# ha7ilm/csdr

Measured on AMD Instinct MI355X. Metric: complex MS/s in->out, WFM demod chain @2.4 MS/s x N streams, higher is better.
Workload: dtype f32

## Files before the change

### csdr_amd/__init__.py

```python
import ctypes as C
import os
import sys
import subprocess
import numpy as np

HERE = os.path.dirname(os.path.abspath(__file__))
LIB_PATH = os.environ.get("CSDR_AMD_LIB") or os.path.join(HERE, "libcsdr_amd.so")
ROOT = os.path.dirname(HERE)

c64 = np.complex64
f32 = np.float32

SHIFT = {"addition": 0, "math": 1, "table": 2, "unroll": 3, "addfast": 4}
WINDOWS = {"BOXCAR": 0, "BLACKMAN": 1, "HAMMING": 2}


class CsdrAmdError(RuntimeError):
    pass


def build(verbose=False):
    r = subprocess.run(["make", "-C", os.path.join(HERE, "csrc"), "-j8"], capture_output=True, text=True)
    if r.returncode != 0:
        raise CsdrAmdError("libcsdr_amd build failed:\n" + r.stdout[-4000:] + r.stderr[-4000:])
# ... 151 lines not shown
    L.csdr_amd_costas_params.argtypes = [fl, fl, i, vp]
    L.csdr_amd_pll_params_p.argtypes = [fl, vp]
    L.csdr_amd_pll_params_pi.argtypes = [fl, fl, fl, fl, vp]
    L.csdr_amd_carrier_create.restype = vp; L.csdr_amd_carrier_create.argtypes = [vp, vp, i]
    L.csdr_amd_carrier_process.argtypes = [vp, vp, ll, sz, vp, vp, vp, vp, sz]
    L.csdr_amd_carrier_reset.argtypes = [vp]
    L.csdr_amd_carrier_reset_channel.argtypes = [vp, i]
    L.csdr_amd_carrier_get_channel.argtypes = [vp, i, vp]
    L.csdr_amd_carrier_set_channel.argtypes = [vp, i, vp]
    L.csdr_amd_carrier_set_lanes.argtypes = [vp, i]
    L.csdr_amd_carrier_lanes.argtypes = [vp]
    L.csdr_amd_carrier_force_generic.argtypes = [vp, i]
    L.csdr_amd_carrier_kernel_name.restype = C.c_char_p; L.csdr_amd_carrier_kernel_name.argtypes = [vp]
    L.csdr_amd_carrier_destroy.argtypes = [vp]; L.csdr_amd_carrier_destroy.restype = None
    L.csdr_amd_debug_carrier_walk.restype = ll; L.csdr_amd_debug_carrier_walk.argtypes = [vp, vp, ll, vp, i, vp, vp, vp, vp, vp]
    L.csdr_amd_amssb_params_default.argtypes = [vp, i]
    L.csdr_amd_amssb_create_cf32.restype = vp; L.csdr_amd_amssb_create_cf32.argtypes = [vp, vp, i, vp, i, i, sz]
    L.csdr_amd_amssb_create.restype = vp; L.csdr_amd_amssb_create.argtypes = [vp, vp, i, fl, i, vp, i, vp, i, i, sz]
    L.csdr_amd_amssb_create_rates.restype = vp; L.csdr_amd_amssb_create_rates.argtypes = [vp, vp, i, vp, i, vp, i, vp, i, i, sz]
    L.csdr_amd_amssb_process.restype = ll; L.csdr_amd_amssb_process.argtypes = [vp, vp, sz, ll, vp, vp, sz]
    L.csdr_amd_amssb_max_out.restype = ll; L.csdr_amd_amssb_max_out.argtypes = [vp, ll]
    L.csdr_amd_amssb_set_rate.argtypes = [vp, i, fl]
    L.csdr_amd_amssb_get_rate.restype = fl; L.csdr_amd_amssb_get_rate.argtypes = [vp, i]
    L.csdr_amd_amssb_front_end.restype = vp; L.csdr_amd_amssb_front_end.argtypes = [vp]
    if hasattr(L, "csdr_amd_amssb_set_passband"):
        L.csdr_amd_amssb_set_passband.argtypes = [vp, i, fl, fl, i]
        L.csdr_amd_amssb_set_channel_taps.argtypes = [vp, i, vp, i]
        L.csdr_amd_amssb_get_passband.argtypes = [vp, i, vp, vp]
    L.csdr_amd_amssb_reset.argtypes = [vp]
    L.csdr_amd_amssb_reset_channel.argtypes = [vp, i]
    L.csdr_amd_amssb_get_channel.argtypes = [vp, i, vp]
    L.csdr_amd_amssb_set_channel.argtypes = [vp, i, vp]
    L.csdr_amd_amssb_set_lanes.argtypes = [vp, i]
    L.csdr_amd_amssb_lanes.argtypes = [vp]
    L.csdr_amd_amssb_force_generic.argtypes = [vp, i]
    L.csdr_amd_amssb_kernel_name.restype = C.c_char_p; L.csdr_amd_amssb_kernel_name.argtypes = [vp]
    L.csdr_amd_amssb_destroy.argtypes = [vp]; L.csdr_amd_amssb_destroy.restype = None
    L.csdr_amd_debug_amssb_walk.restype = ll; L.csdr_amd_debug_amssb_walk.argtypes = [vp, vp, i, vp, vp, vp]
    L.csdr_amd_fmmod_fc.argtypes = [vp, vp, vp, i, sz, sz, sz, vp]
    L.csdr_amd_dsb_fc.argtypes = [vp, vp, vp, sz, fl]
    L.csdr_amd_add_dcoffset_cc.argtypes = [vp, vp, vp, sz]
    L.csdr_amd_fixed_amplitude_cc.argtypes = [vp, vp, vp, sz, fl]
    L.csdr_amd_convert_f_samplerf.argtypes = [vp, vp, vp, sz, C.c_uint]
    L.csdr_amd_debug_fmmod_walk.restype = ll; L.csdr_amd_debug_fmmod_walk.argtypes = [vp, ll, vp, i, vp, vp, vp]
    L.csdr_amd_txbank_create.restype = vp; L.csdr_amd_txbank_create.argtypes = [vp, i, i, fl, fl, i, vp, i, vp, i, sz]
    L.csdr_amd_txbank_process.argtypes = [vp, vp, sz, ll, vp, sz, C.POINTER(ll)]
    L.csdr_amd_txbank_set_rate.argtypes = [vp, i, fl]
    L.csdr_amd_txbank_get_rate.restype = fl; L.csdr_amd_txbank_get_rate.argtypes = [vp, i]
    L.csdr_amd_txbank_reset.argtypes = [vp]
    L.csdr_amd_txbank_max_out.restype = ll; L.csdr_amd_txbank_max_out.argtypes = [vp, ll]
    L.csdr_amd_txbank_force_generic.argtypes = [vp, i]
    L.csdr_amd_txbank_kernel_name.restype = C.c_char_p; L.csdr_amd_txbank_kernel_name.argtypes = [vp]
    L.csdr_amd_txbank_destroy.argtypes = [vp]; L.csdr_amd_txbank_destroy.restype = None
    L.csdr_amd_rational_resampler_get_lowpass_f.restype = None; L.csdr_amd_rational_resampler_get_lowpass_f.argtypes = [vp, i, i, i, i]
    L.csdr_amd_debug_resampler_schedule.argtypes = [i, i, i, i, i, vp]
    L.csdr_amd_logaveragepower_cf.argtypes = [vp, vp, vp, i, i, i, fl]
    L.csdr_amd_fft_exchange_sides_ff.argtypes = [vp, vp, vp, i, i]
    L.csdr_amd_accumulate_power_cf.argtypes = [vp, vp, vp, sz]
    L.csdr_amd_log_ff.argtypes = [vp, vp, vp, sz, fl]
    L.csdr_amd_timer_start.argtypes = [vp]
    L.csdr_amd_timer_stop_ms.argtypes = [vp, C.POINTER(fl)]
    L.csdr_amd_firdes_filter_len.argtypes = [fl]
    L.csdr_amd_firdes_lowpass_f.argtypes = [vp, i, fl, i]
    L.csdr_amd_firdes_bandpass_c.argtypes = [vp, i, fl, fl, i]
    L.csdr_amd_nfm_deemph_taps.argtypes = [i, C.POINTER(vp)]
    L.csdr_amd_shift_addition_init.argtypes = [fl, vp]
    for nm in ("u8_f", "s8_f", "s16_f", "f_u8", "f_s8", "f_s16"):
        getattr(L, "csdr_amd_convert_" + nm).argtypes = [vp, vp, vp, sz]
    L.csdr_amd_convert_f_s24.argtypes = [vp, vp, vp, sz, i]
    L.csdr_amd_convert_s24_f.argtypes = [vp, vp, vp, sz, i]
    L.csdr_amd_rotator_generate.argtypes = [vp, i, fl, C.POINTER(fl), vp, sz, i, i]
    L.csdr_amd_mix_cc.argtypes = [vp, vp, vp, vp, i, sz, sz, sz]
    L.csdr_amd_mix_fc.argtypes = [vp, vp, vp, vp, i, sz, sz, sz]
    L.csdr_amd_shift_cc.argtypes = [vp, i, fl, C.POINTER(fl), vp, vp, i, sz, sz, sz, i, i]
    L.csdr_amd_decimating_shift_addition_cc.argtypes = [vp, vp, vp, i, i, sz, sz, vp, i, vp]
    L.csdr_amd_fir_decimate_cc.argtypes = [vp, vp, vp, i, i, sz, sz, i, vp, i]
    L.csdr_amd_fir_last_kernel.restype = C.c_char_p; L.csdr_amd_fir_last_kernel.argtypes = []
    L.csdr_amd_fir_last_instance.restype = C.c_char_p; L.csdr_amd_fir_last_instance.argtypes = []
    L.csdr_amd_audio_last_path.restype = C.c_char_p; L.csdr_amd_audio_last_path.argtypes = []
    L.csdr_amd_fir_ff_last_instance.restype = C.c_char_p; L.csdr_amd_fir_ff_last_instance.argtypes = []
    L.csdr_amd_fir_ff.argtypes = [vp, vp, vp, i, i, sz, sz, vp, i]
    L.csdr_amd_fmdemod_quadri_cf.argtypes = [vp, vp, vp, i, sz, sz, sz, vp]
    L.csdr_amd_limit_ff.argtypes = [vp, vp, vp, sz, fl]
    L.csdr_amd_gain_ff.argtypes = [vp, vp, vp, sz, fl]
    L.csdr_amd_deemphasis_wfm_ff.argtypes = [vp, vp, vp, i, sz, sz, sz, fl, i, vp]
    L.csdr_amd_fastagc_ff.argtypes = [vp, vp, vp, i, i, i, sz, sz, fl, vp]
    L.csdr_amd_fracdec_create.restype = vp; L.csdr_amd_fracdec_create.argtypes = [fl, i, vp, i]
    L.csdr_amd_fracdec_destroy.argtypes = [vp]
    L.csdr_amd_fractional_decimator_ff.argtypes = [vp, vp, vp, vp, i, i, sz, sz, C.POINTER(i)]
    L.csdr_amd_fracdec_set_cli_bufsize.restype = None; L.csdr_amd_fracdec_set_cli_bufsize.argtypes = [vp, i]
    L.csdr_amd_fracdec_set_where.restype = None; L.csdr_amd_fracdec_set_where.argtypes = [vp, fl]
    L.csdr_amd_fracdec_get_where.restype = fl; L.csdr_amd_fracdec_get_where.argtypes = [vp]
    L.csdr_amd_fftfilt_create.restype = vp; L.csdr_amd_fftfilt_create.argtypes = [vp, i, vp, i, i, i]
    L.csdr_amd_fftfilt_set_taps.argtypes = [vp, vp, i]
    if hasattr(L, "csdr_amd_fftfilt_create_per_stream"):
        L.csdr_amd_fftfilt_create_per_stream.restype = vp; L.csdr_amd_fftfilt_create_per_stream.argtypes = [vp, i, vp, i, i, i]
        L.csdr_amd_fftfilt_set_stream_taps.argtypes = [vp, i, vp, i]
        L.csdr_amd_fftfilt_per_stream.argtypes = [vp]
    L.csdr_amd_fftfilt_destroy.argtypes = [vp]
    L.csdr_amd_fftfilt_input_size.argtypes = [vp]
    L.csdr_amd_fftfilt_reset.argtypes = [vp]
    L.csdr_amd_fftfilt_kernel_name.restype = C.c_char_p; L.csdr_amd_fftfilt_kernel_name.argtypes = [vp]
    L.csdr_amd_fftfilt_window.argtypes = [vp]
    L.csdr_amd_fftfilt_process.argtypes = [vp, vp, vp, i, sz, sz]
    L.csdr_amd_fft_c2c.argtypes = [vp, vp, vp, i, i]
    L.csdr_amd_fastddc_init.argtypes = [vp, fl, i, fl]
    L.csdr_amd_fastddc_fwd_create.restype = vp; L.csdr_amd_fastddc_fwd_create.argtypes = [vp, vp, i]
    L.csdr_amd_fastddc_fwd_destroy.argtypes = [vp]
    L.csdr_amd_fastddc_fwd_process.argtypes = [vp, vp, vp, i]
    L.csdr_amd_fastddc_inv_create.restype = vp; L.csdr_amd_fastddc_inv_create.argtypes = [vp, fl, i, vp, i, i, i]
    L.csdr_amd_fastddc_inv_destroy.argtypes = [vp]
    L.csdr_amd_fastddc_inv_geometry.argtypes = [vp, i, vp]
    L.csdr_amd_fastddc_inv_max_output.argtypes = [vp, i]
    L.csdr_amd_fastddc_inv_process.argtypes = [vp, vp, i, vp, sz, vp]
    L.csdr_amd_fastddc_bank_create.restype = vp; L.csdr_amd_fastddc_bank_create.argtypes = [vp, fl, i, vp, i, i, i]
    L.csdr_amd_fastddc_bank_destroy.argtypes = [vp]; L.csdr_amd_fastddc_bank_destroy.restype = None
    L.csdr_amd_fastddc_bank_set_rate.argtypes = [vp, i, fl]
    L.csdr_amd_fastddc_bank_input_size.argtypes = [vp]
    L.csdr_amd_fastddc_bank_max_output.argtypes = [vp, i]
    L.csdr_amd_fastddc_bank_process.argtypes = [vp, vp, i, vp, sz, vp]
    L.csdr_amd_fastddc_bank_inverse.restype = vp; L.csdr_amd_fastddc_bank_inverse.argtypes = [vp]
    L.csdr_amd_fastddc_bank_submit.argtypes = [vp, vp, i]
    L.csdr_amd_fastddc_bank_collect.argtypes = [vp, vp, sz, vp]
    L.csdr_amd_comm_unique_id.argtypes = [vp]
    L.csdr_amd_comm_create.restype = vp; L.csdr_amd_comm_create.argtypes = [vp, vp, i, i]
    L.csdr_amd_comm_destroy.argtypes = [vp]; L.csdr_amd_comm_destroy.restype = None
    L.csdr_amd_comm_rank.argtypes = [vp]; L.csdr_amd_comm_world.argtypes = [vp]
    L.csdr_amd_comm_broadcast.argtypes = [vp, vp, sz, i]
    L.csdr_amd_comm_dup.restype = vp; L.csdr_amd_comm_dup.argtypes = [vp]
    L.csdr_amd_comm_selftest.argtypes = [vp, sz, C.c_char_p, sz]
    L.csdr_amd_fastddc_bank_create_sharded.restype = vp; L.csdr_amd_fastddc_bank_create_sharded.argtypes = [vp, fl, i, vp, i, i, i, vp]
    L.csdr_amd_fastddc_bank_channel_slice.argtypes = [vp, C.POINTER(i), C.POINTER(i)]
    L.csdr_amd_fastddc_bank_create_sharded_by.restype = vp; L.csdr_amd_fastddc_bank_create_sharded_by.argtypes = [vp, fl, i, vp, i, i, i, vp, i]
    L.csdr_amd_fastddc_bank_shard_mode.argtypes = [vp]
    L.csdr_amd_fastddc_bank_default_shard_mode.argtypes = [i]
    L.csdr_amd_fastddc_bank_local_blocks.argtypes = [vp, i, C.POINTER(i), C.POINTER(i)]
    L.csdr_amd_fastddc_bank_overlap.argtypes = [vp]
    L.csdr_amd_fastddc_bank_submit_local.argtypes = [vp, vp, i]
    if hasattr(L, "csdr_amd_fastddc_bank_process_s16"):
        for nm in ("s16", "u8"):
            getattr(L, "csdr_amd_fastddc_bank_process_" + nm).argtypes = [vp, vp, i, vp, sz, vp]
            getattr(L, "csdr_amd_fastddc_bank_submit_" + nm).argtypes = [vp, vp, i]
            getattr(L, "csdr_amd_fastddc_bank_submit_local_" + nm).argtypes = [vp, vp, i]
    L.csdr_amd_fastddc_bank_finish.argtypes = [vp, vp]
    L.csdr_amd_fastddc_bank_set_rate_global.argtypes = [vp, i, fl]
    L.csdr_amd_loopback_create.restype = vp; L.csdr_amd_loopback_create.argtypes = [i]
    L.csdr_amd_loopback_destroy.argtypes = [vp]; L.csdr_amd_loopback_destroy.restype = None
    L.csdr_amd_loopback_abort.argtypes = [vp]; L.csdr_amd_loopback_abort.restype = None
    L.csdr_amd_comm_create_loopback.restype = vp; L.csdr_amd_comm_create_loopback.argtypes = [vp, vp, i]
    L.csdr_amd_comm_create_null.restype = vp; L.csdr_amd_comm_create_null.argtypes = [vp, i, i]
    L.csdr_amd_comm_create_ipc.restype = vp; L.csdr_amd_comm_create_ipc.argtypes = [vp, C.c_char_p, i, i]
    L.csdr_amd_fastddc_inv_kernel_name.restype = C.c_char_p; L.csdr_amd_fastddc_inv_kernel_name.argtypes = [vp]
    L.csdr_amd_fastddc_inv_kernels.restype = C.c_char_p; L.csdr_amd_fastddc_inv_kernels.argtypes = [vp]
    L.csdr_amd_fastddc_inv_set_profiling.argtypes = [vp, i]
    L.csdr_amd_fastddc_inv_kernel_time.argtypes = [vp, C.POINTER(C.c_double), C.POINTER(C.c_long)]
    L.csdr_amd_fastddc_inv_stage_time.argtypes = [vp, i, C.POINTER(C.c_double), C.POINTER(C.c_long)]
    L.csdr_amd_wfm_create.restype = vp; L.csdr_amd_wfm_create.argtypes = [vp, i, fl, i, vp, i, i, fl, i, sz]
    L.csdr_amd_wfm_destroy.argtypes = [vp]
    L.csdr_amd_wfm_reset.argtypes = [vp]
    L.csdr_amd_wfm_process.restype = C.c_long; L.csdr_amd_wfm_process.argtypes = [vp, vp, sz, sz, vp, vp, sz]
    L.csdr_amd_wfm_kernel_name.restype = C.c_char_p; L.csdr_amd_wfm_kernel_name.argtypes = [vp]
    ll = C.c_longlong; db = C.c_double
    L.csdr_amd_wfm_ring_create.restype = vp; L.csdr_amd_wfm_ring_create.argtypes = [vp, i, fl, i, vp, i, i, fl, i, sz, i]
    L.csdr_amd_wfm_ring_destroy.argtypes = [vp]; L.csdr_amd_wfm_ring_destroy.restype = None
    L.csdr_amd_wfm_ring_reset.argtypes = [vp]
    L.csdr_amd_wfm_ring_acquire.argtypes = [vp, ll, db]
    L.csdr_amd_wfm_ring_input.restype = vp; L.csdr_amd_wfm_ring_input.argtypes = [vp, ll, C.POINTER(sz)]
    L.csdr_amd_wfm_ring_submit.restype = ll; L.csdr_amd_wfm_ring_submit.argtypes = [vp]
    L.csdr_amd_wfm_ring_wait.restype = C.c_long; L.csdr_amd_wfm_ring_wait.argtypes = [vp, ll, db]
    L.csdr_amd_wfm_ring_output.restype = vp; L.csdr_amd_wfm_ring_output.argtypes = [vp, ll, C.POINTER(sz)]
    L.csdr_amd_wfm_ring_set_rate.argtypes = [vp, fl]
    L.csdr_amd_wfm_ring_get_rate.restype = fl; L.csdr_amd_wfm_ring_get_rate.argtypes = [vp]
    L.csdr_amd_wfm_ring_set_timeouts.argtypes = [vp, db, db]
    L.csdr_amd_wfm_ring_resident.argtypes = [vp]
    L.csdr_amd_wfm_ring_stop.argtypes = [vp]
    L.csdr_amd_wfm_ring_slots.argtypes = [vp]
    L.csdr_amd_wfm_ring_grid.argtypes = [vp]
    L.csdr_amd_wfm_ring_launches.restype = C.c_long; L.csdr_amd_wfm_ring_launches.argtypes = [vp]
    L.csdr_amd_wfm_ring_submitted.restype = ll; L.csdr_amd_wfm_ring_submitted.argtypes = [vp]
    L.csdr_amd_wfm_ring_block_times.argtypes = [vp, ll, C.POINTER(db), C.POINTER(db)]
    L.csdr_amd_wfm_ring_replay.argtypes = [vp, C.c_long, vp, vp]
    L.csdr_amd_wfm_ring_stats.argtypes = [vp, vp]
    L.csdr_amd_wfm_set_profiling.argtypes = [vp, i]
    L.csdr_amd_wfm_kernel_time.argtypes = [vp, C.POINTER(C.c_double), C.POINTER(C.c_long)]
    L.csdr_amd_ddc_create.restype = vp; L.csdr_amd_ddc_create.argtypes = [vp, i, fl, i, vp, i, sz]
    if hasattr(L, "csdr_amd_ddc_create_rates"):
        L.csdr_amd_ddc_create_rates.restype = vp; L.csdr_amd_ddc_create_rates.argtypes = [vp, i, vp, i, vp, i, sz]
        L.csdr_amd_ddc_set_rate.argtypes = [vp, i, fl]
        L.csdr_amd_ddc_get_rate.restype = fl; L.csdr_amd_ddc_get_rate.argtypes = [vp, i]
        L.csdr_amd_ddc_fallback.argtypes = [vp]
        L.csdr_amd_wfm_fallback.argtypes = [vp]
        L.csdr_amd_wfm_create_rates.restype = vp; L.csdr_amd_wfm_create_rates.argtypes = [vp, i, vp, i, vp, i, i, fl, i, sz]
        L.csdr_amd_wfm_set_rate.argtypes = [vp, i, fl]
        L.csdr_amd_wfm_get_rate.restype = fl; L.csdr_amd_wfm_get_rate.argtypes = [vp, i]
        L.csdr_amd_nfm_create_rates.restype = vp; L.csdr_amd_nfm_create_rates.argtypes = [vp, i, vp, i, vp, i, i, i, fl, fl, sz]
        L.csdr_amd_nfm_set_rate.argtypes = [vp, i, fl]
    L.csdr_amd_ddc_destroy.argtypes = [vp]
    L.csdr_amd_ddc_reset.argtypes = [vp]
    L.csdr_amd_ddc_process.restype = C.c_long; L.csdr_amd_ddc_process.argtypes = [vp, vp, sz, sz, vp, sz]
    L.csdr_amd_ddc_kernel_name.restype = C.c_char_p; L.csdr_amd_ddc_kernel_name.argtypes = [vp]
    L.csdr_amd_ddc_set_profiling.argtypes = [vp, i]
    L.csdr_amd_ddc_kernel_time.argtypes = [vp, C.POINTER(C.c_double), C.POINTER(C.c_long)]
    L.csdr_amd_nfm_create.restype = vp; L.csdr_amd_nfm_create.argtypes = [vp, i, fl, i, vp, i, i, i, fl, fl, sz]
    L.csdr_amd_nfm_destroy.argtypes = [vp]
    L.csdr_amd_nfm_reset.argtypes = [vp]
    L.csdr_amd_nfm_process.restype = C.c_long; L.csdr_amd_nfm_process.argtypes = [vp, vp, sz, sz, vp, vp, sz]
    L.csdr_amd_nfm_front_end.restype = vp; L.csdr_amd_nfm_front_end.argtypes = [vp]
    _lib = L
    return L


def _hp(a):
    return a.ctypes.data_as(C.c_void_p)


class DevBuf:

    def __init__(self, ctx, nbytes):
        self.ctx, self.nbytes = ctx, int(nbytes)
        self.ptr = lib().csdr_amd_malloc(ctx.h, max(self.nbytes, 16))
        if not self.ptr:
            raise CsdrAmdError(ctx.err())

    def free(self):
        if self.ptr and self.ctx.h:
            lib().csdr_amd_free(self.ctx.h, self.ptr)
        self.ptr = None

    def __del__(self):
        try:
            self.free()
        except Exception:
            pass

    def at(self, byte_offset):
        return C.c_void_p(self.ptr + int(byte_offset))


class _Handle:
    h = None

    def __init__(self, ctx, pre, h):
        self.ctx, self._pre, self._L = ctx, pre, ctx.L if ctx is not None else lib()
        if not h:
            raise CsdrAmdError(ctx.err() if ctx is not None else self._L.csdr_amd_last_error().decode())
        self.h = h

    def _fn(self, name):
        return getattr(self._L, "csdr_amd_%s_%s" % (self._pre, name))

    def _call(self, name, *args):
        return self.ctx.check(self._fn(name)(self.h, *args), "%s_%s" % (self._pre, name))

    def reset(self):
        self._call("reset")

    def force_generic(self, on=True):
        self._call("force_generic", int(on))

    def kernel_name(self):
        return self._fn("kernel_name")(self.h).decode()

    def close(self):
        h, self.h = self.h, None
        if h and (self.ctx is None or self.ctx.h):
            self._fn("destroy")(h)

    def __del__(self):
        try:
            self.close()
        except Exception:
            pass

    def __enter__(self):
        return self

    def __exit__(self, *exc):
        self.close()


class _MaxOut:

    def max_out(self, n_in):
        return int(self._fn("max_out")(self.h, int(n_in)))


class _PerChannel:

    def reset_channel(self, ch):
        self._call("reset_channel", int(ch))


class _ChannelState(_PerChannel):

    def get_channel(self, ch):
        st = self._chan()
        self._call("get_channel", int(ch), C.byref(st))
        return st

    def set_channel(self, ch, st):
        self._call("set_channel", int(ch), C.byref(st))


class _Lanes:

    def set_lanes(self, lanes):
# ... 1195 lines not shown
        di = self.upload(x) if n else self.alloc(256)
        do = self.alloc(max(m, 1) * s + 256)
        self.check(self.L.csdr_amd_duplicate_samples_ntimes_u8_u8(self.h, di.ptr, do.ptr, s, n, max(n, 1), max(m, 1), sample_size_bytes, ntimes),
                   "duplicate_samples_ntimes_u8_u8")
        y = self.download(do, np.uint8, max(m, 1) * s).reshape(s, max(m, 1))[:, :m]
        return y[0].copy() if squeeze else y.copy()

    def rtty(self, params=None, n_channels=1, first="bfsk", last="baudot"):
        return Rtty(self, params, n_channels, first, last)

    def bfsk_demod_cf(self, x, mark, space, force_generic=False):
        x = np.ascontiguousarray(x, c64)
        squeeze = x.ndim == 1
        if squeeze:
            x = x[None]
        s, n = x.shape
        mark = np.ascontiguousarray(mark, c64); space = np.ascontiguousarray(space, c64)
        L = mark.size
        no = max(n - L + 1, 0)
        di = self.upload(x); dt = self.upload(np.concatenate([mark, space]))
        do = self.alloc(4 * max(no, 1) * s + 256)
        self.check(self.L.csdr_amd_bfsk_demod_cf(self.h, di.ptr, do.ptr, s, n, n, max(no, 1), dt.ptr, dt.at(8 * L), L, int(force_generic)), "bfsk_demod_cf")
        y = self.download(do, f32, max(no, 1) * s).reshape(s, max(no, 1))[:, :no].copy()
        self.last_bfsk_kernel = self.L.csdr_amd_bfsk_last_kernel().decode()
        return y[0] if squeeze else y

    def squelch(self, n_channels=1, block_size=1024, use_every_nth=1, levels=None, max_samples_per_call=1 << 22):
        return Squelch(self, n_channels, block_size, use_every_nth, levels, max_samples_per_call)

    def am_bank(self, n_channels=1, block=1024, agc=None, limit_max=None, **kw):
        return AmSsb(self, amssb_params("am", block, agc, limit_max), n_channels, **kw)

    def ssb_bank(self, n_channels=1, block=1024, taps=None, fft_size=0, agc=None, limit_max=None, **kw):
        if kw.get("passbands") is not None:
            kw["passbands"] = _passband_list(kw["passbands"], n_channels)
            if taps is None:
                raise ValueError("passbands need taps: their length is the passbands' length")
        return AmSsb(self, amssb_params("ssb", block, agc, limit_max), n_channels, taps=taps, fft_size=fft_size, **kw)

    def carrier(self, params, n_channels=1):
        return Carrier(self, params, n_channels)

    def txbank(self, n_streams, mode, interpolation, taps, rates, **kw):
        return TxBank(self, n_streams, mode, interpolation, taps, rates, **kw)

    def _get_power(self, x, block_size, decimation, dt, fn):
        x = np.ascontiguousarray(x, dt)
        squeeze = x.ndim == 1
        if squeeze:
            x = x[None]
        s, n = x.shape
        B = n if block_size is None else int(block_size)
        nb = n // B if B > 0 else 0
        di = self.upload(x); do = self.alloc(4 * max(nb, 1) * s + 256)
        self.check(fn(self.h, di.ptr, s, nb, B, int(decimation), n, do.ptr), "get_power")
        y = self.download(do, f32, nb * s).reshape(s, nb)
        return y[0].copy() if squeeze else y.copy()

    def get_power_c(self, x, block_size=None, decimation=1):
        return self._get_power(x, block_size, decimation, c64, self.L.csdr_amd_get_power_c)

    def get_power_f(self, x, block_size=None, decimation=1):
        return self._get_power(x, block_size, decimation, f32, self.L.csdr_amd_get_power_f)

    def binary_slicer_f_u8(self, x):
        x = np.ascontiguousarray(x, f32)
        squeeze = x.ndim == 1
        if squeeze:
            x = x[None]
        s, n = x.shape
        di = self.upload(x); do = self.alloc(max(n, 1) * s + 256)
        self.check(self.L.csdr_amd_binary_slicer_f_u8(self.h, di.ptr, do.ptr, s, n, n, n), "binary_slicer_f_u8")
        y = self.download(do, np.uint8, n * s).reshape(s, n)
        return y[0].copy() if squeeze else y.copy()

    def rtty_line_decoder_u8_u8(self, x, calls=None):
        x = np.ascontiguousarray(x, np.uint8)
        squeeze = x.ndim == 1
        if squeeze:
            x = x[None]
        s, n = x.shape
        calls = [n] if calls is None else list(calls)
        di = self.upload(x)
        mx = max(max(calls) if calls else 0, 1)
        do = self.alloc(mx * s + 256); dc = self.alloc(4 * s + 256)
        dst = self.upload(np.zeros(5 * s, np.int32))
        outs = [[] for _ in range(s)]
        at = 0
        for k in calls:
            self.check(self.L.csdr_amd_rtty_line_decoder_u8_u8(self.h, di.at(at), do.ptr, s, k, n, mx, dst.ptr, dc.ptr), "rtty_line_decoder_u8_u8")
            cnt = self.download(dc, np.int32, s)
            y = self.download(do, np.uint8, mx * s).reshape(s, mx)
            for c in range(s):
                outs[c].append(y[c, :cnt[c]].copy())
            at += k
        res = [np.concatenate(o) for o in outs]
        return res[0] if squeeze else res

    def interpolator(self, interpolation, taps=None, n_streams=1, transition_bw=0.05, window="HAMMING", bufsize=None):
        if taps is None:
            taps = fir_interpolate_lowpass_f(self.firdes_filter_len(transition_bw), interpolation, window)
        return Interpolator(self, interpolation, taps, n_streams, bufsize)

    def rational_resampler_ff(self, x, interpolation, decimation, taps=None, transition_bw=0.05, window="HAMMING", bufsize=None, calls=None):
        x2 = np.ascontiguousarray(x, f32)
        r = self.resampler(interpolation, decimation, taps, 1 if x2.ndim == 1 else x2.shape[0], transition_bw, window, bufsize)
        try:
            return r.process(x2, calls)
        finally:
            r.close()

    def fir_interpolate_cc(self, x, interpolation, taps=None, transition_bw=0.05, window="HAMMING", bufsize=None, calls=None):
        x2 = np.ascontiguousarray(x, c64)
        p = self.interpolator(interpolation, taps, 1 if x2.ndim == 1 else x2.shape[0], transition_bw, window, bufsize)
        try:
            return p.process(x2, calls)
        finally:
            p.close()

    def fft_c2c(self, x, forward=True):
        x = np.ascontiguousarray(x, c64); di = self.upload(x); do = self.alloc(x.nbytes + 64)
        self.check(self.L.csdr_amd_fft_c2c(self.h, di.ptr, do.ptr, x.size, int(forward)), "fft"); return self.download(do, c64, x.size)

    def fftfilt(self, fft_size, taps, n_streams=1, max_blocks=1):
        return FftFilt(self, fft_size, taps, n_streams, max_blocks)

    def bandpass_fir_fft_cc(self, x, taps, fft_size, blocks_per_call=None):
        x2, squeeze = self._2d(x, c64)
        s, n = x2.shape
        taps = _fftfilt_taps(taps, s)
        inp = fft_size - taps.shape[-1] + 1; nb = n // inp
        per = nb if not blocks_per_call else blocks_per_call
        with FftFilt(self, fft_size, taps, s, max(per, 1)) as f:
            y = f.process(x2, [per] * (nb // per) + ([nb % per] if nb % per else [])) if nb else np.zeros((s, 0), c64)
        return y[0].copy() if squeeze else y

    def fastddc_init(self, tbw, decimation, shift_rate):
        d = FastDDC(); err = self.L.csdr_amd_fastddc_init(C.byref(d), tbw, decimation, shift_rate); return d, err

    def fastddc_fwd_cc(self, x, ddc, blocks_per_call=None):
        x = np.ascontiguousarray(x, c64); nb = x.size // ddc.input_size
        per = nb if not blocks_per_call else blocks_per_call
        with _Handle(self, "fastddc_fwd", self.L.csdr_amd_fastddc_fwd_create(self.h, C.byref(ddc), max(per, 1))) as f:
            di = self.upload(x); do = self.alloc(8 * nb * ddc.fft_size + 64)
            b = 0
            while b < nb:
                k = min(per, nb - b)
                self.check(f._fn("process")(f.h, di.at(8 * b * ddc.input_size), do.at(8 * b * ddc.fft_size), k), "fastddc_fwd")
                b += k
            return self.download(do, c64, nb * ddc.fft_size).reshape(nb, ddc.fft_size)

    def _note_ddc_call(self, inv, counts):
        self.last_ddc_kernels = self.L.csdr_amd_fastddc_inv_kernels(inv).decode()
        self.ddc_kernels_seen.add(self.last_ddc_kernels)
        self.ddc_call_kernels.append(self.last_ddc_kernels); self.ddc_call_counts.append(counts.copy())

    def fastddc_inv_cc(self, spectra, tbw, decimation, shift_rates, window="HAMMING", blocks_per_call=None):
        self.ddc_call_kernels = []; self.ddc_call_counts = []
        spectra = np.ascontiguousarray(spectra, c64); nb = spectra.shape[0]
        rates = np.ascontiguousarray(shift_rates, f32); nc = rates.size
        per = nb if not blocks_per_call else blocks_per_call
        with _Handle(self, "fastddc_inv", self.L.csdr_amd_fastddc_inv_create(self.h, tbw, decimation, _hp(rates), nc, WINDOWS[window], max(per, 1))) as f:
            fft = spectra.shape[1]
            di = self.upload(spectra)
            outs = [[] for _ in range(nc)]
            b = 0
            while b < nb:
                k = min(per, nb - b)
                pitch = f._fn("max_output")(f.h, k) + 8
                do = self.alloc(8 * nc * pitch)
                counts = np.zeros(nc, np.int32)
                self.check(f._fn("process")(f.h, di.at(8 * b * fft), k, do.ptr, pitch, _hp(counts)), "fastddc_inv")
                self._note_ddc_call(f.h, counts)
                y = self.download(do, c64, nc * pitch).reshape(nc, pitch)
                for c in range(nc):
                    outs[c].append(y[c, :counts[c]].copy())
                b += k
        return [np.concatenate(o) for o in outs]

    def fastddc_bank(self, x, tbw, decimation, shift_rates, window="HAMMING", blocks_per_call=None, retune=None, schedule=None, retunes=None):
        x, sfx, es = _bank_input(x)
        self.ddc_call_kernels = []; self.ddc_call_counts = []
        rates = np.ascontiguousarray(shift_rates, f32); nc = rates.size
        ddc, _ = self.fastddc_init(tbw, decimation, 0.0)
        nb = (x.size if es == 8 else x.size // 2) // ddc.input_size
        process = getattr(self.L, "csdr_amd_fastddc_bank_process" + sfx)
        per = nb if not blocks_per_call else blocks_per_call
        if schedule:
            per = max(schedule)
        with _Handle(self, "fastddc_bank", self.L.csdr_amd_fastddc_bank_create(self.h, tbw, decimation, _hp(rates), nc, WINDOWS[window], max(per, 1))) as bk:
            di = self.upload(x)
            outs = [[] for _ in range(nc)]
            b = 0; call = 0
            while b < nb:
                k = min(per, nb - b) if not schedule else min(schedule[call % len(schedule)], nb - b)
                if retune and retune[0] == call:
                    self.check(bk._fn("set_rate")(bk.h, retune[1], retune[2]), "bank_set_rate")
                for ch, rt in (retunes or {}).get(call, []):
                    self.check(bk._fn("set_rate")(bk.h, ch, rt), "bank_set_rate")
                pitch = bk._fn("max_output")(bk.h, k) + 8
                do = self.alloc(8 * nc * pitch)
                counts = np.zeros(nc, np.int32)
                self.check(process(bk.h, di.at(es * b * ddc.input_size), k, do.ptr, pitch, _hp(counts)), "fastddc_bank")
                self._note_ddc_call(bk._fn("inverse")(bk.h), counts)
                y = self.download(do, c64, nc * pitch).reshape(nc, pitch)
                for c in range(nc):
                    outs[c].append(y[c, :counts[c]].copy())
                b += k; call += 1
            self.last_ddc_kernel = self.L.csdr_amd_fastddc_inv_kernel_name(bk._fn("inverse")(bk.h)).decode()
        return [np.concatenate(o) for o in outs]


    def wfm_chain(self, iq_u8, shift_rate, decimation, taps, frac_rate=5, tau=50e-6, audio_rate=48000, block=None, pitch_pad=0, retunes=None, want_float=True,
                  out_per_call=False):
        x2, squeeze = self._2d(iq_u8, np.uint8)
        s, nbytes = x2.shape; n = nbytes // 2
        pitch = (nbytes + 15) // 16 * 16 + pitch_pad
        xx = np.zeros((s, pitch), np.uint8); xx[:, :nbytes] = x2
        taps = np.ascontiguousarray(taps, f32)
        sched = list(block) if isinstance(block, (list, tuple)) else None
        block = n if block is None else (max(sched) if sched else block)
        if np.ndim(shift_rate) == 0:
            w = self.L.csdr_amd_wfm_create(self.h, s, shift_rate, decimation, _hp(taps), taps.size, frac_rate, tau, audio_rate, max(block, 1024))
        else:
            rates = np.ascontiguousarray(shift_rate, f32); assert rates.size == s
            w = self.L.csdr_amd_wfm_create_rates(self.h, s, _hp(rates), decimation, _hp(taps), taps.size, frac_rate, tau, audio_rate, max(block, 1024))
        with _Handle(self, "wfm", w) as w:
            di = self.upload(xx)
            apitch = (n // (decimation * frac_rate) + 64 + 63) // 64 * 64
            ds = self.alloc(2 * s * apitch); df = self.alloc(4 * s * apitch) if want_float else None
            pos = 0; na = 0; call = 0; parts_s = []; parts_f = []
            while pos < n:
                for st, r in (retunes or {}).get(call, []):
                    w._call("set_rate", st, r)
                k = min(sched[call] if (sched and call < len(sched)) else block, n - pos); call += 1
                if out_per_call:
                    got = w._call("process", di.at(2 * pos), pitch, k, ds.ptr, df.ptr if want_float else None, apitch)
                    parts_s.append(self.download(ds, np.int16, s * apitch).reshape(s, apitch)[:, :got].copy())
                    if want_float: parts_f.append(self.download(df, f32, s * apitch).reshape(s, apitch)[:, :got].copy())
                else:
                    got = w._call("process", di.at(2 * pos), pitch, k, ds.at(2 * na), df.at(4 * na) if want_float else None, apitch)
                pos += k; na += got
            if out_per_call:
                s16 = np.concatenate(parts_s, axis=1) if parts_s else np.zeros((s, 0), np.int16)
                af = np.concatenate(parts_f, axis=1) if parts_f else np.zeros((s, 0), f32)
            else:
                s16 = self.download(ds, np.int16, s * apitch).reshape(s, apitch)[:, :na]
                af = self.download(df, f32, s * apitch).reshape(s, apitch)[:, :na] if want_float else np.zeros((s, 0), f32)
            self.last_wfm_kernel = w.kernel_name()
        return (s16[0].copy(), af[0].copy()) if squeeze else (s16.copy(), af.copy())

    def ddc_u8(self, iq_u8, shift_rate, decimation, taps, block=None, pitch_pad=0, retunes=None):
        x2, squeeze = self._2d(iq_u8, np.uint8)
        s, nbytes = x2.shape; n = nbytes // 2
        pitch = (nbytes + 127) // 128 * 128 + pitch_pad
        xx = np.full((s, pitch), 0x80, np.uint8); xx[:, :nbytes] = x2
        taps = np.ascontiguousarray(taps, f32)
        sched = list(block) if isinstance(block, (list, tuple)) else None
        block = n if block is None else (max(sched) if sched else block)
        if np.ndim(shift_rate) == 0:
            d = self.L.csdr_amd_ddc_create(self.h, s, shift_rate, decimation, _hp(taps), taps.size, max(block, 1024))
        else:
            rates = np.ascontiguousarray(shift_rate, f32); assert rates.size == s
            d = self.L.csdr_amd_ddc_create_rates(self.h, s, _hp(rates), decimation, _hp(taps), taps.size, max(block, 1024))
        with _Handle(self, "ddc", d) as d:
            di = self.upload(xx)
            opitch = n // decimation + 64
            do = self.alloc(8 * s * opitch)
            pos = 0; no = 0; self.ddc_kernels = set(); call = 0
            while pos < n:
                for st, r in (retunes or {}).get(call, []):
                    d._call("set_rate", st, r)
                k = min(sched[call] if (sched and call < len(sched)) else block, n - pos); call += 1
                got = d._call("process", di.at(2 * pos), pitch, k, do.at(8 * no), opitch)
                self.ddc_kernels.add(d.kernel_name())
                pos += k; no += got
            y = self.download(do, c64, s * opitch).reshape(s, opitch)[:, :no]
            self.last_ddc_kernel = d.kernel_name()
        return y[0].copy() if squeeze else y.copy()

    def wfm_ring_chain(self, iq_u8, shift_rate, decimation, taps, block=16384, n_slots=8, frac_rate=5, tau=50e-6, audio_rate=48000, retunes=None, in_flight=None,
                       idle_us=None, life_ms=None, pause_every=None, pause_s=0.0):
        import time
        x2, squeeze = self._2d(iq_u8, np.uint8)
        s, nbytes = x2.shape; n = nbytes // 2
        assert n % block == 0
        nb = n // block
        taps = np.ascontiguousarray(taps, f32)
        with _Handle(self, "wfm_ring", self.L.csdr_amd_wfm_ring_create(self.h, s, shift_rate, decimation, _hp(taps), taps.size, frac_rate, tau, audio_rate, block,
                                                                       n_slots)) as ring:
            r = ring.h
            if idle_us is not None or life_ms is not None:
                self.check(self.L.csdr_amd_wfm_ring_set_timeouts(r, 200.0 if idle_us is None else idle_us, 250.0 if life_ms is None else life_ms), "ring_set_timeouts")
            depth = (n_slots - 2) if in_flight is None else in_flight
            outs = []; pitch = C.c_size_t(0); opitch = C.c_size_t(0)

            def collect(k):
                na = self.check(self.L.csdr_amd_wfm_ring_wait(r, k, 0.0), "ring_wait")
                po = self.L.csdr_amd_wfm_ring_output(r, k, C.byref(opitch))
                buf = np.empty((s, opitch.value), np.int16)
                self.check(self.L.csdr_amd_d2h(self.h, _hp(buf), po, buf.nbytes), "d2h")
                outs.append(buf[:, :na].copy())
            for k in range(nb):
                if retunes and k in retunes:
                    while len(outs) < k:
                        collect(len(outs))
# ... 183 lines not shown
```

### csdr_amd/csrc/fastddc.hpp

```cpp
#pragma once
#include "common.hpp"

namespace csdr_amd {

struct ChanGeom { int offsetbin; float sindelta, cosdelta, rate2; };
struct DdcChanState { int remain; float phase; };

struct DdcMfma;

struct DdcComm {
    int rank, world; void *impl;
    int (*group_start)(const DdcComm *c);
    int (*group_end)(const DdcComm *c);
    int (*send)(const DdcComm *c, const void *dev_buf, size_t n_floats, int peer, hipStream_t st);
    int (*recv)(const DdcComm *c, void *dev_buf, size_t n_floats, int peer, hipStream_t st);
    int (*all_gather)(const DdcComm *c, void *dev_buf_all, size_t n_floats_per_rank, hipStream_t st);
};

DdcMfma *ddc_mfma_create(csdr_amd_ctx *ctx, int fft, int inv, int pre, int n_channels, int max_blocks, int scrap, int post_in, int post_dec, int input_size, int overlap,
                         const DdcComm *comm);
void ddc_mfma_destroy(DdcMfma *m);
int ddc_mfma_quiesce(DdcMfma *m);
int ddc_mfma_set_taps(DdcMfma *m, hipStream_t st, const cf32 *d_H, int c_first, int c_count);
bool ddc_mfma_can_forward(const DdcMfma *m);
enum { DDC_IN_CF32 = 0, DDC_IN_S16 = 1, DDC_IN_U8 = 2 };
static inline size_t ddc_in_bytes(int fmt) { return fmt == DDC_IN_S16 ? 4 : fmt == DDC_IN_U8 ? 2 : 8; }
int ddc_mfma_submit(DdcMfma *m, const void *in, const cf32 *spectra, int n_blocks, DdcChanState *d_state, const ChanGeom *d_geom, bool inline_call, const cf32 *ext_tail = nullptr,
                    int fmt = DDC_IN_CF32, bool tail_in_front = false);
int ddc_mfma_convert_samples(hipStream_t st, const void *in, int fmt, long long first, int n, cf32 *out);
int ddc_mfma_set_segment(DdcMfma *m, int nbl, int first, int total, int world, int *pref_cur, int *pref_next);
int ddc_mfma_pending_blocks(const DdcMfma *m);
int ddc_mfma_skip_batch(DdcMfma *m, DdcChanState *d_state, const ChanGeom *d_geom);
int ddc_mfma_collect(DdcMfma *m, const ChanGeom *d_geom, cf32 *out, size_t out_pitch, const int **d_counts, hipEvent_t after_inverse = nullptr);
int ddc_mfma_set_profiling(DdcMfma *m, int on);
int ddc_mfma_kernel_time(DdcMfma *m, double *total_ms, long *launches);
int ddc_mfma_stage_time(DdcMfma *m, int stage, double *total_ms, long *launches);
const char *ddc_mfma_kernel_name(const DdcMfma *m);
const char *ddc_mfma_kernels(const DdcMfma *m);

}
```

### csdr_amd/csrc/fastddc_mfma.hip

```cpp
#include "fastddc.hpp"
#include "convert_dev.hpp"
#include <hip/hip_ext.h>
#include "fft_butterflies.hpp"
#include <math.h>
#include <stddef.h>
#include <stdlib.h>
#include <string.h>
#include <string>
#include <vector>

namespace csdr_amd {

typedef float f32x16 __attribute__((ext_vector_type(16)));

struct DdcMfma {
    csdr_amd_ctx *ctx;
    Stream side;
    int fft, inv, pre, G, C, Cpad, nbp, scrap, post_in, post_dec, kmax, rpitch, max_blocks;
    DevBuf<float> d_Ht; DevBuf<cf32> d_Ct; DevBuf<float2> d_tw;
    int rank, world, nbl; const DdcComm *comm; DevBuf<cf32> d_in_local;
    int seg_nbl = 0, seg_first = 0, seg_total = 0, seg_world = 0, spec_seg_first = 0, spec_seg_total = 0; int *seg_cur = nullptr, *seg_next = nullptr;
    DevBuf<cf32> d_Xt[2]; DevBuf<float2> d_R[2]; DevBuf<int> d_blk_remain[2], d_blk_off[2], d_counts[2]; DevBuf<float> d_blk_phase[2];
    int pending_blocks[2]; int fill, drain;
    bool inline_set[2], chains_on_side[2];
    bool gemm_three = false, gemm_narrow = false;
    const char *front[2] = {"", ""}, *front2[2] = {"", ""}; std::string kernels;
    bool y_holds[2] = {false, false};
    DevBuf<DdcChanState> d_state_spec; DdcChanState *last_state = nullptr; bool spec_valid = false, ahead_ok = false; int spec_set = 0, spec_blocks = 0;
    Event ev_ready[2], ev_free[2], ev_fork; bool free_recorded[2];
    DevBuf<cf32> d_Y, d_tail[2]; DevBuf<float2> d_twb; int flip, input_size, overlap;
    struct Opt { bool fwd_off, riders_off, spec_off, pass2_own; } opt;
    bool profiling = false; double prof_ms = 0; long prof_launches = 0; KernelTimer timer;
    bool profile_stages = false;
    struct StageProf { double ms = 0; long launches = 0; KernelTimer timer; } stage[2];
    bool stages_timed() const { return profiling && profile_stages; }
};

namespace {

__global__ __launch_bounds__(256) void k_ddc_ht(const float2 *__restrict__ H, float *__restrict__ Ht, int fft, int inv, int G, int Cpad, int c_first)
{
    const int r = blockIdx.x * 256 + threadIdx.x;
    if (r >= inv) return;
    const int q = blockIdx.y, c = c_first + blockIdx.z;
    const float2 v = H[(size_t)c * fft + r + (size_t)q * inv];
    *reinterpret_cast<float2 *>(Ht + (((size_t)r * G + (q >> 2)) * Cpad + c) * 8 + 2 * (q & 3)) = v;
}

__global__ __launch_bounds__(256) void k_ddc_xt(const float2 *__restrict__ X, float2 *__restrict__ Xt, int fft, int inv, int pre, int nbp)
{
    __shared__ float2 tile[32][33];
    const int tx = threadIdx.x & 31, ty = threadIdx.x >> 5;
    const int r0 = blockIdx.x * 32, qp0 = blockIdx.y * 32; const size_t b = blockIdx.z;
#pragma unroll
    for (int j = 0; j < 4; j++) {
        const int qp = qp0 + ty + 8 * j, r = r0 + tx;
        if (qp < pre && r < inv) tile[ty + 8 * j][tx] = X[b * fft + (size_t)qp * inv + r];
    }
    __syncthreads();
#pragma unroll
    for (int j = 0; j < 4; j++) {
        const int r = r0 + ty + 8 * j, qp = qp0 + tx;
        if (qp < pre && r < inv) Xt[((size_t)r * nbp + b) * pre + ((qp - pre / 2) & (pre - 1))] = tile[tx][ty + 8 * j];
    }
}


template <int NBT, bool PERSIST>
__global__ __launch_bounds__(512, PERSIST ? 2 : 4) void k_ddc_gemm(const float *__restrict__ Ht, const float2 *__restrict__ Xt, float2 *__restrict__ Ct,
                                                  const ChanGeom *__restrict__ geom, int inv, int pre, int Cpad, int n_channels, int nbp, int nbl, int n_blocks, float scale)
{
    extern __shared__ float4 xs_all[];
    constexpr int NX = 4 * NBT;
    const int wave = threadIdx.x >> 6, lane = threadIdx.x & 63;
    const int c_base = blockIdx.y * 256 + wave * 32, b_base = blockIdx.z * 32 * NBT;
    const int G = pre >> 2, P4 = (pre >> 1) + 1, rows = 32 * NBT, row4 = pre >> 1, BUF = rows * P4;
    const int i = lane & 31, hi = lane >> 5;
    const size_t gstride = (size_t)Cpad * 2;
    const bool active = c_base < Cpad;
    auto xt_row = [&](int r, int b) { return reinterpret_cast<const float4 *>(Xt + (((size_t)(b / nbl) * inv + r) * nbl + (b % nbl)) * pre); };
    {
        for (int idx = threadIdx.x; idx < rows * row4; idx += 512) {
            const int row = idx / row4, col = idx - row * row4, b = b_base + row;
            xs_all[row * P4 + col] = (b < n_blocks) ? xt_row(blockIdx.x, b)[col] : make_float4(0.f, 0.f, 0.f, 0.f);
        }
    }
    __syncthreads();
    int cur = 0;
    for (int r = blockIdx.x; r < inv; r += gridDim.x) {
        const int rn = r + gridDim.x;
        float4 nx[NX];
        if (PERSIST && rn < inv) {
#pragma unroll
            for (int k = 0; k < NX; k++) {
                const int idx = threadIdx.x + 512 * k, row = idx / row4, col = idx - row * row4, b = b_base + row;
                nx[k] = (idx < rows * row4 && b < n_blocks) ? xt_row(rn, b)[col] : make_float4(0.f, 0.f, 0.f, 0.f);
            }
        }
        if (active) {
            const float4 *xs = xs_all + cur * BUF;
            const float4 *ap = reinterpret_cast<const float4 *>(Ht) + ((size_t)r * G * Cpad + c_base + i) * 2 + hi;
            f32x16 acc[NBT][2];
#pragma unroll
            for (int bt = 0; bt < NBT; bt++)
#pragma unroll
                for (int p = 0; p < 2; p++)
#pragma unroll
                    for (int e = 0; e < 16; e++) acc[bt][p][e] = 0.f;
            float4 a0 = ap[0], a1 = ap[(size_t)min(1, G - 1) * gstride], a2 = ap[(size_t)min(2, G - 1) * gstride], a3 = ap[(size_t)min(3, G - 1) * gstride];
            const float4 *xrow = xs + i * P4 + hi;
#define DDC_STEP(AV, GG)                                                                                                   \
            {                                                                                                              \
                _Pragma("unroll") for (int bt = 0; bt < NBT; bt++) {                                                       \
                    const float4 xv = xrow[bt * 32 * P4 + 2 * (GG)];                                                       \
                    acc[bt][0] = __builtin_amdgcn_mfma_f32_32x32x2f32((AV).x, xv.x, acc[bt][0], 0, 0, 0);                  \
                    acc[bt][1] = __builtin_amdgcn_mfma_f32_32x32x2f32((AV).x, xv.y, acc[bt][1], 0, 0, 0);                  \
                    acc[bt][0] = __builtin_amdgcn_mfma_f32_32x32x2f32((AV).y, -xv.y, acc[bt][0], 0, 0, 0);                 \
                    acc[bt][1] = __builtin_amdgcn_mfma_f32_32x32x2f32((AV).y, xv.x, acc[bt][1], 0, 0, 0);                  \
                    acc[bt][0] = __builtin_amdgcn_mfma_f32_32x32x2f32((AV).z, xv.z, acc[bt][0], 0, 0, 0);                  \
                    acc[bt][1] = __builtin_amdgcn_mfma_f32_32x32x2f32((AV).z, xv.w, acc[bt][1], 0, 0, 0);                  \
                    acc[bt][0] = __builtin_amdgcn_mfma_f32_32x32x2f32((AV).w, -xv.w, acc[bt][0], 0, 0, 0);                 \
                    acc[bt][1] = __builtin_amdgcn_mfma_f32_32x32x2f32((AV).w, xv.z, acc[bt][1], 0, 0, 0);                  \
                }                                                                                                          \
            }
            int g = 0;
            for (; g + 4 <= G; g += 4) {
                { const float4 av = a0; a0 = ap[(size_t)min(g + 4, G - 1) * gstride]; DDC_STEP(av, g); }
                { const float4 av = a1; a1 = ap[(size_t)min(g + 5, G - 1) * gstride]; DDC_STEP(av, g + 1); }
                { const float4 av = a2; a2 = ap[(size_t)min(g + 6, G - 1) * gstride]; DDC_STEP(av, g + 2); }
                { const float4 av = a3; a3 = ap[(size_t)min(g + 7, G - 1) * gstride]; DDC_STEP(av, g + 3); }
            }
            if (g < G) { DDC_STEP(a0, g); }
            if (g + 1 < G) { DDC_STEP(a1, g + 1); }
            if (g + 2 < G) { DDC_STEP(a2, g + 2); }
#undef DDC_STEP
#pragma unroll
            for (int e = 0; e < 16; e++) {
                const int c = c_base + (e & 3) + 8 * (e >> 2) + 4 * hi;
                if (c >= n_channels) continue;
                int m = (r - geom[c].offsetbin) % inv; if (m < 0) m += inv;
                float2 *dst = Ct + ((size_t)m * Cpad + c) * nbp + b_base + i;
#pragma unroll
                for (int bt = 0; bt < NBT; bt++)
                    if (b_base + bt * 32 + i < n_blocks) dst[bt * 32] = make_float2(acc[bt][0][e] * scale, acc[bt][1][e] * scale);
            }
        }
        if (PERSIST && rn < inv) {
            float4 *nxt = xs_all + (cur ^ 1) * BUF;
#pragma unroll
            for (int k = 0; k < NX; k++) {
                const int idx = threadIdx.x + 512 * k, row = idx / row4, col = idx - row * row4;
                if (idx < rows * row4) nxt[row * P4 + col] = nx[k];
            }
            __builtin_amdgcn_fence(__ATOMIC_RELEASE, "workgroup", "local");
            __builtin_amdgcn_s_barrier();
            __builtin_amdgcn_fence(__ATOMIC_ACQUIRE, "workgroup", "local");
            cur ^= 1;
        }
    }
}

template <int NBT, bool FWD>
__global__ __launch_bounds__(512, 2) void k_ddc_gemm3(const float *__restrict__ Ht, const float2 *__restrict__ Xt, float2 *__restrict__ Ct,
                                                       const ChanGeom *__restrict__ geom, int inv, int Cpad, int n_channels, int nbp, int nbl, int n_blocks, float scale,
                                                       const float2 *__restrict__ g_tw)
{
    extern __shared__ float4 xs_all[];
    constexpr int PRE = 128, G = PRE / 4, P4 = PRE / 2 + 1, ROWS = 32 * NBT, BUF = ROWS * P4, RPW = ROWS / 8;
    constexpr int AD = FWD ? 4 : 8;
    const int wave = __builtin_amdgcn_readfirstlane(threadIdx.x >> 6), lane = threadIdx.x & 63;
    const int c_base = blockIdx.y * 256 + wave * 32, b_base = blockIdx.z * ROWS;
    const int i = lane & 31, hi = lane >> 5;
    const size_t gstride = (size_t)Cpad * 2;
    const bool active = c_base < Cpad;
    const uint32_t lds_base = (uint32_t)(size_t)(__attribute__((address_space(3))) uint8_t *)xs_all;
    auto dma_rows = [&](int r, int buf) {
#pragma unroll
        for (int k = 0; k < RPW; k++) {
            const int row = wave * RPW + k, b = min(b_base + row, n_blocks - 1);
            const float2 *src = (FWD ? Xt + ((size_t)b * 512 + r) * PRE
                                     : Xt + (((size_t)(b / nbl) * inv + r) * nbl + (b % nbl)) * PRE) + 2 * lane;
            const uint32_t la = __builtin_amdgcn_readfirstlane((int)(lds_base + ((uint32_t)buf * BUF + (uint32_t)row * P4) * 16u));
            uint32_t keep;
            asm volatile("s_mov_b32 %0, m0\n\ts_mov_b32 m0, %2\n\ts_nop 0\n\tglobal_load_lds_dwordx4 %1, off\n\ts_mov_b32 m0, %0" : "=&s"(keep) : "v"(src), "s"(la) : "memory");
        }
    };
    typedef float g3_v4f __attribute__((ext_vector_type(4)));
    auto taps_fetch = [&](g3_v4f &dst, const float4 *p) { asm volatile("global_load_dwordx4 %0, %1, off" : "=v"(dst) : "v"(p) : "memory"); };
#define G3_TAPS_READY(V, K) asm volatile("s_waitcnt vmcnt(%1)" : "+v"(V) : "n"(K))
    const int tr = wave * RPW + (lane >> 3), fc = lane & 7;
    const bool frow = (lane >> 3) < RPW;
    auto fft_rows = [&](int buf) {
        if (!frow) return;
        float2 *rowp = reinterpret_cast<float2 *>(xs_all + (size_t)buf * BUF + (size_t)tr * P4);
        float2 v[16];
#pragma unroll
        for (int a16 = 0; a16 < 16; a16++) v[a16] = rowp[8 * a16 + fc];
        dft16<false>(v);
        __builtin_amdgcn_wave_barrier();
#pragma unroll
        for (int ka = 0; ka < 16; ka++) rowp[fc * 16 + ka] = cmul(v[ka], g_tw[(4 * fc * ka) & 511]);
        __builtin_amdgcn_wave_barrier();
        float2 e[8], o[8];
#pragma unroll
        for (int cc = 0; cc < 8; cc++) {
            const float4 two = *reinterpret_cast<const float4 *>(&rowp[cc * 16 + 2 * fc]);
            e[cc] = make_float2(two.x, two.y); o[cc] = make_float2(two.z, two.w);
        }
        dft8<false>(e); dft8<false>(o);
        __builtin_amdgcn_wave_barrier();
#pragma unroll
        for (int kc = 0; kc < 8; kc++) {
            const int q = (2 * fc + 16 * kc + 64) & 127;
            *reinterpret_cast<float4 *>(&rowp[q]) = make_float4(e[kc].x, e[kc].y, o[kc].x, o[kc].y);
        }
    };
    int r = blockIdx.x;
    if (r >= inv) return;
    dma_rows(r, 0);
    asm volatile("s_waitcnt vmcnt(0)" ::: "memory");
    const int c_eff = min(c_base, Cpad - 32);
    f32x16 acc[NBT][3];
    auto store_bins = [&](int rr) {
        if (!active) return;
        int mm[16];
#pragma unroll
        for (int e = 0; e < 16; e++) {
            const int c = min(c_base + (e & 3) + 8 * (e >> 2) + 4 * hi, n_channels - 1);
            mm[e] = (rr - geom[c].offsetbin) & (inv - 1);
        }
#pragma unroll
        for (int e = 0; e < 16; e++) {
            const int c = c_base + (e & 3) + 8 * (e >> 2) + 4 * hi;
            if (c >= n_channels) continue;
            float2 *dst = Ct + ((size_t)mm[e] * Cpad + c) * nbp + b_base + i;
#pragma unroll
            for (int bt = 0; bt < NBT; bt++)
                if (b_base + bt * 32 + i < n_blocks) {
                    const float p1 = acc[bt][0][e], p2 = acc[bt][1][e], p3 = acc[bt][2][e];
                    dst[bt * 32] = make_float2((p1 - p2) * scale, (p3 - p1 - p2) * scale);
                }
        }
    };
    int cur = 0, r_prev = -1;
    for (;;) {
        const int rn = r + gridDim.x;
        const float4 *ap = reinterpret_cast<const float4 *>(Ht) + ((size_t)r * G * Cpad + c_eff + i) * 2 + hi;
        g3_v4f a[AD];
#pragma unroll
        for (int d = 0; d < AD; d++) taps_fetch(a[d], ap + (size_t)d * gstride);
        if (r_prev >= 0) store_bins(r_prev);
        if (FWD) fft_rows(cur);
        __builtin_amdgcn_fence(__ATOMIC_RELEASE, "workgroup", "local");
        __builtin_amdgcn_s_barrier();
        __builtin_amdgcn_fence(__ATOMIC_ACQUIRE, "workgroup", "local");
#pragma unroll
        for (int bt = 0; bt < NBT; bt++)
#pragma unroll
            for (int p = 0; p < 3; p++)
#pragma unroll
                for (int e = 0; e < 16; e++) acc[bt][p][e] = 0.f;
        const float4 *xrow = xs_all + cur * BUF + i * P4 + hi;
        float4 xn[NBT];
#pragma unroll
        for (int bt = 0; bt < NBT; bt++) xn[bt] = xrow[bt * 32 * P4];
#define DDC_STEP3(AV, GG)                                                                                                  \
        {                                                                                                                  \
            const float hs0 = (AV).x + (AV).y, hs1 = (AV).z + (AV).w;                                                      \
            float4 xc[NBT];                                                                                                \
            _Pragma("unroll") for (int bt = 0; bt < NBT; bt++) { xc[bt] = xn[bt]; xn[bt] = xrow[bt * 32 * P4 + 2 * min((GG) + 1, G - 1)]; }  \
            _Pragma("unroll") for (int bt = 0; bt < NBT; bt++) {                                                           \
                const float4 xv = xc[bt];                                                                                  \
                const float xs0 = xv.x + xv.y, xs1 = xv.z + xv.w;                                                          \
                acc[bt][0] = __builtin_amdgcn_mfma_f32_32x32x2f32((AV).x, xv.x, acc[bt][0], 0, 0, 0);                      \
                acc[bt][1] = __builtin_amdgcn_mfma_f32_32x32x2f32((AV).y, xv.y, acc[bt][1], 0, 0, 0);                      \
                acc[bt][2] = __builtin_amdgcn_mfma_f32_32x32x2f32(hs0, xs0, acc[bt][2], 0, 0, 0);                          \
                acc[bt][0] = __builtin_amdgcn_mfma_f32_32x32x2f32((AV).z, xv.z, acc[bt][0], 0, 0, 0);                      \
                acc[bt][1] = __builtin_amdgcn_mfma_f32_32x32x2f32((AV).w, xv.w, acc[bt][1], 0, 0, 0);                      \
                acc[bt][2] = __builtin_amdgcn_mfma_f32_32x32x2f32(hs1, xs1, acc[bt][2], 0, 0, 0);                          \
            }                                                                                                              \
        }
        static_assert(G % AD == 0 && G >= 2 * AD, "k loop");
#pragma unroll
        for (int d = 0; d < AD; d++) { G3_TAPS_READY(a[d], AD - 1); const g3_v4f av = a[d]; taps_fetch(a[d], ap + (size_t)(AD + d) * gstride); DDC_STEP3(av, d); }
        if (rn < inv) dma_rows(rn, cur ^ 1);
#pragma unroll
        for (int g = AD; g < G - AD; g += AD) {
#pragma unroll
            for (int d = 0; d < AD; d++) { G3_TAPS_READY(a[d], AD - 1); const g3_v4f av = a[d]; taps_fetch(a[d], ap + (size_t)(g + AD + d) * gstride); DDC_STEP3(av, g + d); }
        }
#define G3_LAST(D) { G3_TAPS_READY(a[D], AD - 1 - (D)); const g3_v4f av = a[D]; DDC_STEP3(av, G - AD + (D)); }
        G3_LAST(0) G3_LAST(1) G3_LAST(2) G3_LAST(3)
        if constexpr (AD == 8) { G3_LAST(4) G3_LAST(5) G3_LAST(6) G3_LAST(7) }
#undef G3_LAST
#undef DDC_STEP3
        r_prev = r;
        if (rn >= inv) break;
        r = rn; cur ^= 1;
    }
    store_bins(r_prev);
}

template <int NW>
__global__ __launch_bounds__(64 * NW) void k_ddc_gemm3n(const float *__restrict__ Ht, const float2 *__restrict__ Xt, float2 *__restrict__ Ct,
                                                        const ChanGeom *__restrict__ geom, int inv, int Cpad, int n_channels, int nbp, int nbl, int n_blocks, float scale)
{
    extern __shared__ float4 xs_all[];
    constexpr int PRE = 128, G = PRE / 4, P4 = PRE / 2 + 1, ROWS = 32, RPW = ROWS / NW, AD = 8;
    const int wave = __builtin_amdgcn_readfirstlane(threadIdx.x >> 6), lane = threadIdx.x & 63;
    const int r = blockIdx.x;
    const int c_base = ((int)blockIdx.y * NW + wave) * 32, b_base = blockIdx.z * ROWS;
    const int i = lane & 31, hi = lane >> 5;
    const size_t gstride = (size_t)Cpad * 2;
    const bool active = c_base < Cpad;
    const int c_eff = min(c_base, Cpad - 32);
    const uint32_t lds_base = (uint32_t)(size_t)(__attribute__((address_space(3))) uint8_t *)xs_all;
    typedef float g3_v4f __attribute__((ext_vector_type(4)));
    auto taps_fetch = [&](g3_v4f &dst, const float4 *p) { asm volatile("global_load_dwordx4 %0, %1, off" : "=v"(dst) : "v"(p) : "memory"); };
    const float4 *ap = reinterpret_cast<const float4 *>(Ht) + ((size_t)r * G * Cpad + c_eff + i) * 2 + hi;
    g3_v4f a[AD];
#pragma unroll
    for (int d = 0; d < AD; d++) taps_fetch(a[d], ap + (size_t)d * gstride);
#pragma unroll
    for (int k = 0; k < RPW; k++) {
        const int row = wave * RPW + k, b = min(b_base + row, n_blocks - 1);
        const float2 *src = Xt + (((size_t)(b / nbl) * inv + r) * nbl + (b % nbl)) * PRE + 2 * lane;
        const uint32_t la = __builtin_amdgcn_readfirstlane((int)(lds_base + (uint32_t)row * P4 * 16u));
        uint32_t keep;
        asm volatile("s_mov_b32 %0, m0\n\ts_mov_b32 m0, %2\n\ts_nop 0\n\tglobal_load_lds_dwordx4 %1, off\n\ts_mov_b32 m0, %0" : "=&s"(keep) : "v"(src), "s"(la) : "memory");
    }
    asm volatile("s_waitcnt vmcnt(0)" ::: "memory");
    __builtin_amdgcn_fence(__ATOMIC_RELEASE, "workgroup", "local");
    if (NW > 1) __builtin_amdgcn_s_barrier();
    __builtin_amdgcn_fence(__ATOMIC_ACQUIRE, "workgroup", "local");
    f32x16 acc[3];
#pragma unroll
    for (int p = 0; p < 3; p++)
#pragma unroll
        for (int e = 0; e < 16; e++) acc[p][e] = 0.f;
    const float4 *xrow = xs_all + i * P4 + hi;
    float4 xn = xrow[0];
#define DDC_STEP3N(AV, GG)                                                                                                 \
    {                                                                                                                      \
        const float hs0 = (AV).x + (AV).y, hs1 = (AV).z + (AV).w;                                                          \
        const float4 xv = xn; xn = xrow[2 * min((GG) + 1, G - 1)];                                                         \
        const float xs0 = xv.x + xv.y, xs1 = xv.z + xv.w;                                                                  \
        acc[0] = __builtin_amdgcn_mfma_f32_32x32x2f32((AV).x, xv.x, acc[0], 0, 0, 0);                                      \
        acc[1] = __builtin_amdgcn_mfma_f32_32x32x2f32((AV).y, xv.y, acc[1], 0, 0, 0);                                      \
        acc[2] = __builtin_amdgcn_mfma_f32_32x32x2f32(hs0, xs0, acc[2], 0, 0, 0);                                          \
        acc[0] = __builtin_amdgcn_mfma_f32_32x32x2f32((AV).z, xv.z, acc[0], 0, 0, 0);                                      \
        acc[1] = __builtin_amdgcn_mfma_f32_32x32x2f32((AV).w, xv.w, acc[1], 0, 0, 0);                                      \
        acc[2] = __builtin_amdgcn_mfma_f32_32x32x2f32(hs1, xs1, acc[2], 0, 0, 0);                                          \
    }
    static_assert(G % AD == 0 && G >= 2 * AD, "k loop");
#pragma unroll
    for (int g = 0; g < G - AD; g += AD) {
#pragma unroll
        for (int d = 0; d < AD; d++) { G3_TAPS_READY(a[d], AD - 1); const g3_v4f av = a[d]; taps_fetch(a[d], ap + (size_t)(g + AD + d) * gstride); DDC_STEP3N(av, g + d); }
    }
#define G3N_LAST(D) { G3_TAPS_READY(a[D], AD - 1 - (D)); const g3_v4f av = a[D]; DDC_STEP3N(av, G - AD + (D)); }
    G3N_LAST(0) G3N_LAST(1) G3N_LAST(2) G3N_LAST(3) G3N_LAST(4) G3N_LAST(5) G3N_LAST(6) G3N_LAST(7)
#undef G3N_LAST
#undef DDC_STEP3N
    if (!active) return;
    int mm[16];
#pragma unroll
    for (int e = 0; e < 16; e++) {
        const int c = min(c_base + (e & 3) + 8 * (e >> 2) + 4 * hi, n_channels - 1);
        mm[e] = (r - geom[c].offsetbin) & (inv - 1);
    }
    if (b_base + i >= n_blocks) return;
#pragma unroll
    for (int e = 0; e < 16; e++) {
        const int c = c_base + (e & 3) + 8 * (e >> 2) + 4 * hi;
        if (c >= n_channels) continue;
        const float p1 = acc[0][e], p2 = acc[1][e], p3 = acc[2][e];
        Ct[((size_t)mm[e] * Cpad + c) * nbp + b_base + i] = make_float2((p1 - p2) * scale, (p3 - p1 - p2) * scale);
    }
}
#undef G3_TAPS_READY

struct DdcChainJob {
    DdcChanState *state, *state_out; const ChanGeom *geom; int n_channels, n_blocks, post_in, post_dec, kmax;
    int mode;
    int *blk_remain; float *blk_phase; int *blk_off; int *counts; float2 *R;
    int seg_nbl, seg_first, seg_total, seg_world; int *seg_pref;
};
__host__ __device__ __forceinline__ int ddc_chain_step(DdcChanState &s, float r, int post_in, int post_dec, int sh)
{
    int k = 0, pos = s.remain;
    if (pos < post_in) { k = (sh >= 0 ? (post_in - 1 - pos) >> sh : (post_in - 1 - pos) / post_dec) + 1; pos += k * post_dec; }
    s.remain = pos - post_in;
    float p = s.phase + r * PI_F * (float)k;
    while (p > PI_F) p -= 2 * PI_F;
    while (p < -PI_F) p += 2 * PI_F;
    s.phase = p;
    return k;
}
struct DdcChainFast { bool ok, big; int k; float d; };
__host__ __device__ __forceinline__ DdcChainFast ddc_chain_fast(const DdcChanState &s, float r, int post_in, int post_dec)
{
    DdcChainFast f;
    f.k = post_in / post_dec; f.d = r * PI_F * (float)f.k;
    f.ok = post_in % post_dec == 0 && s.remain >= 0 && s.remain < post_dec;
    f.big = !(fabsf(f.d) < 6.0f);
    return f;
}
__host__ __device__ __forceinline__ float ddc_phase_step(float p, float d, bool big = false)
{
    p = p + d;
    if (big) { while (p > PI_F) p -= 2 * PI_F; while (p < -PI_F) p += 2 * PI_F; return p; }
    const float lo = p - 2 * PI_F; p = p > PI_F ? lo : p;
    const float hi = p + 2 * PI_F; p = p < -PI_F ? hi : p;
    return p;
}
__device__ __forceinline__ void ddc_chain_body_seg(const DdcChainJob &j, int c)
{
    if (c >= j.n_channels) return;
    DdcChanState s = j.state[c];
    const float r = j.geom[c].rate2;
    const int post_in = j.post_in, post_dec = j.post_dec, n_channels = j.n_channels;
    const int sh = (post_dec & (post_dec - 1)) == 0 ? __ffs(post_dec) - 1 : -1;
    const DdcChainFast f = ddc_chain_fast(s, r, post_in, post_dec);
    int total = 0;
    for (int g = 0; g < j.seg_world; g++) {
        const int b0 = min(g * j.seg_nbl, j.seg_total), b1 = min(b0 + j.seg_nbl, j.seg_total);
        const bool mine = b0 == j.seg_first && j.n_blocks > 0;
        int cnt = 0;
        if (f.ok) {
            float p = s.phase;
            if (mine) for (int b = b0; b < b1; b++) {
                const size_t id = (size_t)(b - b0) * n_channels + c;
                j.blk_remain[id] = s.remain; j.blk_phase[id] = p; j.blk_off[id] = (b - b0) * f.k;
                p = ddc_phase_step(p, f.d, f.big);
            } else for (int b = b0; b < b1; b++) p = ddc_phase_step(p, f.d, f.big);
            s.phase = p; cnt = (b1 - b0) * f.k;
        } else if (mine) {
            for (int b = b0; b < b1; b++) {
                const size_t id = (size_t)(b - b0) * n_channels + c;
                j.blk_remain[id] = s.remain; j.blk_phase[id] = s.phase; j.blk_off[id] = cnt;
                cnt += ddc_chain_step(s, r, post_in, post_dec, sh);
            }
        } else for (int b = b0; b < b1; b++) cnt += ddc_chain_step(s, r, post_in, post_dec, sh);
        if (mine) j.counts[c] = cnt;
        j.seg_pref[(size_t)g * n_channels + c] = total; total += cnt;
    }
    j.seg_pref[(size_t)j.seg_world * n_channels + c] = total;
    if (j.n_blocks <= 0) j.counts[c] = 0;
    j.state_out[c] = s;
}
__device__ __forceinline__ void ddc_chain_body(const DdcChainJob &j, int c)
{
    if (j.seg_nbl) { ddc_chain_body_seg(j, c); return; }
    if (c >= j.n_channels) return;
    DdcChanState s = j.state[c];
    const float r = j.geom[c].rate2;
    const int post_in = j.post_in, post_dec = j.post_dec, n_channels = j.n_channels;
    const int sh = (post_dec & (post_dec - 1)) == 0 ? __ffs(post_dec) - 1 : -1;
    const DdcChainFast f = ddc_chain_fast(s, r, post_in, post_dec);
    if (f.ok) {
        float p = s.phase;
        for (int b = 0; b < j.n_blocks; b++) {
            const size_t id = (size_t)b * n_channels + c;
            j.blk_remain[id] = s.remain; j.blk_phase[id] = p; j.blk_off[id] = b * f.k;
            p = ddc_phase_step(p, f.d, f.big);
        }
        s.phase = p;
        j.state_out[c] = s; j.counts[c] = j.n_blocks * f.k;
        return;
    }
    int off = 0;
    for (int b = 0; b < j.n_blocks; b++) {
        const size_t id = (size_t)b * n_channels + c;
        j.blk_remain[id] = s.remain; j.blk_phase[id] = s.phase; j.blk_off[id] = off;
        off += ddc_chain_step(s, r, post_in, post_dec, sh);
    }
    j.state_out[c] = s; j.counts[c] = off;
}
__global__ __launch_bounds__(64) void k_ddc_chain_t(DdcChainJob j) { ddc_chain_body(j, blockIdx.x * 64 + threadIdx.x); }
constexpr int ROT_CK = 16;
__device__ __forceinline__ void ddc_rot_body(const DdcChainJob &j, int id)
{
    const int n_chains = j.n_channels * j.n_blocks;
    if (id >= n_chains) return;
    const ChanGeom g = j.geom[id % j.n_channels];
    const float cd = g.cosdelta, sd = g.sindelta, ph = j.blk_phase[id];
    float co = (float)cos((double)ph), sn = (float)sin((double)ph);
    for (int k0 = 0; k0 < j.kmax; k0 += ROT_CK) {
        j.R[(size_t)(k0 / ROT_CK) * n_chains + id] = make_float2(co, sn);
#pragma unroll
        for (int kk = 0; kk < ROT_CK; kk++) { const float c1 = co * cd - sn * sd, s1 = sn * cd + co * sd; co = c1; sn = s1; }
    }
}
__global__ __launch_bounds__(64) void k_ddc_rot(DdcChainJob j) { ddc_rot_body(j, blockIdx.x * 64 + threadIdx.x); }

__device__ __forceinline__ int pad8(int idx) { return idx + (idx >> 3); }
template <int NT> struct I512 { static constexpr int pitch = NT == 16 ? 580 : 578; static constexpr int tw_n = NT == 16 ? 512 : 448; };

template <bool INV>
__device__ __forceinline__ void fft512_stage1_store(float2 (&v)[8], float2 *row, int tp, const float2 *tw)
{
    dft8<INV>(v);
#pragma unroll
    for (int k1 = 0; k1 < 8; k1++) { float2 w = tw[(k1 * tp) & 511]; if (INV) w.y = -w.y; row[pad8(64 * k1 + tp)] = cmul(v[k1], w); }
}
template <bool INV, int NT>
__device__ __forceinline__ void fft512_stages23(float2 *data, int t, const float2 *tw)
{
    const int wave = t >> 6, lane = t & 63, hi3 = lane >> 3, lo3 = lane & 7;
    for (int round = 0; round < NT / 4; round++) {
        float2 *row = data + (4 * round + wave) * I512<NT>::pitch;
        float2 v[8];
#pragma unroll
        for (int n2 = 0; n2 < 8; n2++) v[n2] = row[pad8(64 * hi3 + 8 * n2 + lo3)];
        dft8<INV>(v);
#pragma unroll
        for (int k2 = 0; k2 < 8; k2++) { float2 w = tw[(8 * k2 * lo3) & 511]; if (INV) w.y = -w.y; row[pad8(64 * hi3 + 8 * k2 + lo3)] = cmul(v[k2], w); }
        __syncthreads();
#pragma unroll
        for (int n3 = 0; n3 < 8; n3++) v[n3] = row[pad8(64 * hi3 + 8 * lo3 + n3)];
        dft8<INV>(v);
        __syncthreads();
#pragma unroll
        for (int k3 = 0; k3 < 8; k3++) row[pad8(hi3 + 8 * lo3 + 64 * k3)] = v[k3];
    }
    __syncthreads();
}

template <int FMT> __device__ __forceinline__ float2 ddc_in_sample(const void *in, long long pos)
{
// ... 101 lines not shown
        for (int a = 0; a < 8; a++) v[s][a] = src[(size_t)(64 * a + i + IW * s) * mstride];
    __syncthreads();
#pragma unroll
    for (int s = 0; s < NS; s++) {
        if (!ok) {
#pragma unroll
            for (int a = 0; a < 8; a++) v[s][a] = make_float2(0.f, 0.f);
        }
        fft512_stage1_store<true>(v[s], data + j * PITCH, i + IW * s, tw);
    }
    __syncthreads();
    fft512_stages23<true, NT>(data, t, tw);
    const float inv_n = 1.0f / 512.0f;
    const float cd = geom[c].cosdelta, sd = geom[c].sindelta;
    const size_t n_chains = (size_t)n_blocks * n_channels;
    for (int bl = 0; bl < NT; bl++) {
        const int b = b0 + bl;
        if (b >= n_blocks) break;
        const size_t id = (size_t)b * n_channels + c;
        const int rem = blk_remain[id];
        const int cnt = rem < post_in ? (post_in - 1 - rem) / post_dec + 1 : 0;
        float2 *dst = out + (size_t)c * out_pitch + blk_off[id];
        for (int k = t; k < cnt; k += 256) {
            const float2 x = data[bl * PITCH + pad8(scrap + rem + post_dec * k)];
            const float vi = x.x * inv_n, vq = x.y * inv_n;
            float2 w = R[(size_t)(k / ROT_CK) * n_chains + id];
            const int steps = k % ROT_CK;
#pragma unroll
            for (int s2 = 0; s2 < ROT_CK - 1; s2++)
                if (s2 < steps) { const float c1 = w.x * cd - w.y * sd, s1 = w.y * cd + w.x * sd; w.x = c1; w.y = s1; }
            dst[k] = make_float2(w.x * vi - w.y * vq, w.y * vi + w.x * vq);
        }
    }
}

template <int NT> struct I256 { static constexpr int pitch = NT == 16 ? 292 : 290; };

template <int NT>
__global__ __launch_bounds__(256) void k_ddc_ifft256d_post(const float2 *__restrict__ Ct, float2 *__restrict__ out, size_t out_pitch, const float2 *__restrict__ R,
                                                           const float2 *__restrict__ g_tw, const int *__restrict__ blk_remain, const int *__restrict__ blk_off,
                                                           const ChanGeom *__restrict__ geom, int Cpad, int nbp, int n_blocks, int n_channels, int scrap, int post_in,
                                                           DdcChainJob ahead, int n_riders)
{
    if ((int)blockIdx.x < n_riders) { ddc_chain_body(ahead, (int)blockIdx.x * 256 + (int)threadIdx.x); return; }
    const int bx = (int)blockIdx.x - n_riders;
    extern __shared__ float4 lds_raw[];
    constexpr int PITCH = I256<NT>::pitch, NS = NT / 4, IW = 256 / NT;
    float2 *data = reinterpret_cast<float2 *>(lds_raw), *tw = data + NT * PITCH;
    const int t = threadIdx.x, j = t & (NT - 1), i = t / NT;
    int c, b0;
    if (NT == 16) { c = blockIdx.y; b0 = blockIdx.x * 16; }
    else {
        const int L = bx, h = (L >> 3) & 1, P = (L >> 4) * 8 + (L & 7), nl = (n_blocks + 15) / 16;
        c = P / nl; b0 = (P - c * nl) * 16 + 8 * h;
        if (c >= n_channels) return;
    }
    tw[t] = g_tw[t]; tw[t + 256] = g_tw[t + 256];
    const bool ok = b0 + j < n_blocks;
    const size_t idj = (size_t)(ok ? b0 + j : 0) * n_channels + c;
    const int remj = blk_remain[idj], rho = (scrap + remj) & 1;
    const float2 *src = Ct + (size_t)c * nbp + b0 + (ok ? j : 0);
    const size_t mstride = (size_t)Cpad * nbp;
    float2 v[NS][8];
#pragma unroll
    for (int s = 0; s < NS; s++)
#pragma unroll
        for (int a = 0; a < 8; a++) v[s][a] = src[(size_t)(64 * a + i + IW * s) * mstride];
    __syncthreads();
    float2 *row = data + j * PITCH;
#pragma unroll
    for (int s = 0; s < NS; s++) {
        const int tp = i + IW * s;
        float2 z[4];
#pragma unroll
        for (int a = 0; a < 4; a++) {
            float2 lo = v[s][a], hi = v[s][a + 4];
            if (!ok) { lo = make_float2(0.f, 0.f); hi = lo; }
            float2 sum = rho ? csub(lo, hi) : cadd(lo, hi);
            if (rho) { float2 w = tw[64 * a + tp]; w.y = -w.y; sum = cmul(sum, w); }
            z[a] = sum;
        }
        dft4<true>(z[0], z[1], z[2], z[3]);
#pragma unroll
        for (int k1 = 0; k1 < 4; k1++) { float2 w = tw[(2 * k1 * tp) & 511]; w.y = -w.y; row[pad8(64 * k1 + tp)] = cmul(z[k1], w); }
    }
    __syncthreads();
    {
        const int wave = t >> 6, lane = t & 63, half = lane >> 5, l5 = lane & 31, k1 = l5 >> 3, lo3 = l5 & 7;
        for (int round = 0; round < NT / 8; round++) {
            float2 *rw = data + (8 * round + 2 * wave + half) * PITCH;
            float2 u[8];
#pragma unroll
            for (int n2 = 0; n2 < 8; n2++) u[n2] = rw[pad8(64 * k1 + 8 * n2 + lo3)];
            dft8<true>(u);
#pragma unroll
            for (int k2 = 0; k2 < 8; k2++) { float2 w = tw[(8 * k2 * lo3) & 511]; w.y = -w.y; rw[pad8(64 * k1 + 8 * k2 + lo3)] = cmul(u[k2], w); }
            __syncthreads();
#pragma unroll
            for (int n3 = 0; n3 < 8; n3++) u[n3] = rw[pad8(64 * k1 + 8 * lo3 + n3)];
            dft8<true>(u);
            __syncthreads();
#pragma unroll
            for (int k3 = 0; k3 < 8; k3++) rw[pad8(k1 + 4 * lo3 + 32 * k3)] = u[k3];
        }
        __syncthreads();
    }
    const float inv_n = 1.0f / 512.0f;
    const float cd = geom[c].cosdelta, sd = geom[c].sindelta;
    const size_t n_chains = (size_t)n_blocks * n_channels;
    for (int bl = 0; bl < NT; bl++) {
        const int b = b0 + bl;
        if (b >= n_blocks) break;
        const size_t id = (size_t)b * n_channels + c;
        const int rem = blk_remain[id];
        const int cnt = rem < post_in ? (post_in - 1 - rem) / 2 + 1 : 0;
        const int kbase = (scrap + rem) >> 1;
        float2 *dst = out + (size_t)c * out_pitch + blk_off[id];
        for (int k = t; k < cnt; k += 256) {
            const float2 x = data[bl * PITCH + pad8(kbase + k)];
            const float vi = x.x * inv_n, vq = x.y * inv_n;
            float2 w = R[(size_t)(k / ROT_CK) * n_chains + id];
            const int steps = k % ROT_CK;
#pragma unroll
            for (int s2 = 0; s2 < ROT_CK - 1; s2++)
                if (s2 < steps) { const float c1 = w.x * cd - w.y * sd, s1 = w.y * cd + w.x * sd; w.x = c1; w.y = s1; }
            dst[k] = make_float2(w.x * vi - w.y * vq, w.y * vi + w.x * vq);
        }
    }
}

}

static constexpr size_t DDC_LDS_MAX = 160 * 1024;
static size_t ddc_fold_lds(int pre, int nbt) { return (size_t)32 * nbt * (pre / 2 + 1) * sizeof(float4); }
static int ddc_fold_tiles(int pre, int n_blocks) { return n_blocks > 32 && ddc_fold_lds(pre, 2) <= DDC_LDS_MAX ? 2 : 1; }

DdcMfma *ddc_mfma_create(csdr_amd_ctx *ctx, int fft, int inv, int pre, int n_channels, int max_blocks, int scrap, int post_in, int post_dec, int input_size, int overlap,
                         const DdcComm *comm)
{
    if (getenv("CSDR_AMD_DDC_MFMA_OFF")) return nullptr;
    if (inv != 512 || pre < 8 || (pre & (pre - 1)) || fft != inv * pre || post_dec < 1 || scrap + post_in > inv) return nullptr;
    if (ddc_fold_lds(pre, 1) > DDC_LDS_MAX) return nullptr;
    Owned<DdcMfma, ddc_mfma_destroy> m(new DdcMfma());
    m->ctx = ctx; m->fft = fft; m->inv = inv; m->pre = pre; m->G = pre / 4; m->C = n_channels; m->Cpad = (n_channels + 31) / 32 * 32;
    m->max_blocks = max_blocks; m->nbp = (max_blocks + 31) / 32 * 32; m->scrap = scrap; m->post_in = post_in; m->post_dec = post_dec;
    m->kmax = (post_in - 1) / post_dec + 1; m->rpitch = (m->kmax + ROT_CK - 1) / ROT_CK;
    m->input_size = input_size; m->overlap = overlap;
    m->comm = comm; m->rank = comm ? comm->rank : 0; m->world = comm ? comm->world : 1;
    {
        DdcMfma::Opt &o = m->opt;
        o.fwd_off = getenv("CSDR_AMD_DDC_FWD_OFF") != nullptr;
        o.riders_off = getenv("CSDR_AMD_DDC_RIDERS_OFF") != nullptr; o.spec_off = getenv("CSDR_AMD_DDC_SPEC_OFF") != nullptr;
        o.pass2_own = getenv("CSDR_AMD_DDC_PASS2") != nullptr;
    }
    m->nbl = m->world > 1 ? (max_blocks + m->world - 1) / m->world : m->nbp;
    const size_t xt_elems = (size_t)m->world * inv * m->nbl * pre;
    hipError_t e = dev_alloc(m->d_Ht, sizeof(float) * 2 * (size_t)m->Cpad * fft);
    if (e == hipSuccess) e = dev_alloc(m->d_Ct, sizeof(cf32) * (size_t)inv * m->Cpad * m->nbp);
    if (e == hipSuccess) e = dev_alloc(m->d_tw, sizeof(float2) * 512);
    if (e == hipSuccess) e = dev_alloc(m->d_twb, sizeof(float2) * 128);
    for (int k = 0; k < 2 && e == hipSuccess; k++) {
        const size_t n_tab = (size_t)n_channels * max_blocks;
        e = dev_alloc(m->d_Xt[k], sizeof(cf32) * xt_elems);
        if (e == hipSuccess) e = dev_alloc(m->d_R[k], sizeof(float2) * n_tab * m->rpitch);
        if (e == hipSuccess) e = dev_alloc(m->d_blk_remain[k], sizeof(int) * n_tab);
        if (e == hipSuccess) e = dev_alloc(m->d_blk_off[k], sizeof(int) * n_tab);
        if (e == hipSuccess) e = dev_alloc(m->d_blk_phase[k], sizeof(float) * n_tab);
        if (e == hipSuccess) e = dev_alloc(m->d_counts[k], sizeof(int) * n_channels);
        if (e == hipSuccess) e = event_create(m->ev_ready[k], hipEventDisableTiming);
        if (e == hipSuccess) e = event_create(m->ev_free[k], hipEventDisableTiming);
    }
    if (e == hipSuccess) e = event_create(m->ev_fork, hipEventDisableTiming);
    if (e == hipSuccess) e = dev_alloc(m->d_state_spec, sizeof(DdcChanState) * (size_t)n_channels);
    if (e == hipSuccess) e = stream_create(m->side);
    if (e == hipSuccess) e = hipMemsetAsync(m->d_Ht.get(), 0, sizeof(float) * 2 * (size_t)m->Cpad * fft, ctx->stream);
    m->input_size = input_size; m->overlap = overlap;
    if (e == hipSuccess && fft == 65536 && pre == 128) {
        const int y_blocks = m->world > 1 ? m->nbl : m->max_blocks;
        e = dev_alloc(m->d_Y, sizeof(cf32) * (size_t)y_blocks * fft);
        for (int t = 0; t < 2 && e == hipSuccess; t++) {
            e = dev_alloc(m->d_tail[t], sizeof(cf32) * (size_t)(overlap + 1));
            if (e == hipSuccess) e = hipMemsetAsync(m->d_tail[t].get(), 0, sizeof(cf32) * (size_t)(overlap + 1), ctx->stream);
        }
        if (e == hipSuccess && m->world > 1) e = dev_alloc(m->d_in_local, sizeof(cf32) * ((size_t)m->nbl * input_size + overlap));
    }
    if (e != hipSuccess) { fail(e, "hipMalloc(fastddc matrix-core path)", __FILE__, __LINE__); return nullptr; }
    std::vector<float2> tw(512), twb(128);
    for (int k = 0; k < 512; k++) { const double a = -2.0 * M_PI * k / 512.0; tw[k] = make_float2((float)cos(a), (float)sin(a)); }
    for (int k = 0; k < 128; k++) { const double a = -2.0 * M_PI * k / 65536.0; twb[k] = make_float2((float)cos(a), (float)sin(a)); }
    if (hipMemcpy(m->d_tw.get(), tw.data(), sizeof(float2) * 512, hipMemcpyHostToDevice) != hipSuccess ||
        hipMemcpy(m->d_twb.get(), twb.data(), sizeof(float2) * 128, hipMemcpyHostToDevice) != hipSuccess) return nullptr;
    return m.release();
}

void ddc_mfma_destroy(DdcMfma *m)
{
    if (!m) return;
    if (m->side) (void)hipStreamSynchronize(m->side.get());
    delete m;
}

int ddc_mfma_quiesce(DdcMfma *m)
{
    CSDR_HIP(hipStreamSynchronize(m->side.get())); CSDR_HIP(hipStreamSynchronize(m->ctx->stream));
    m->spec_valid = false;
    return 0;
}

int ddc_mfma_set_taps(DdcMfma *m, hipStream_t st, const cf32 *d_H, int c_first, int c_count)
{
    if (c_count <= 0) return 0;
    hipLaunchKernelGGL(k_ddc_ht, dim3(cdiv(m->inv, 256), m->pre, c_count), dim3(256), 0, st, reinterpret_cast<const float2 *>(d_H), m->d_Ht.get(), m->fft, m->inv, m->G, m->Cpad, c_first);
    CSDR_LAUNCH_CHECK();
    return 0;
}

bool ddc_mfma_can_forward(const DdcMfma *m) { return m && m->fft == 65536 && m->pre == 128 && !m->opt.fwd_off; }

static DdcChainJob mfma_chain_job(DdcMfma *m, int k, int n_blocks, DdcChanState *d_state, const ChanGeom *d_geom)
{
    DdcChainJob j;
    j.state = d_state; j.state_out = d_state; j.mode = 1; j.geom = d_geom; j.n_channels = m->C; j.n_blocks = n_blocks; j.post_in = m->post_in; j.post_dec = m->post_dec; j.kmax = m->kmax;
    j.blk_remain = m->d_blk_remain[k].get(); j.blk_phase = m->d_blk_phase[k].get(); j.blk_off = m->d_blk_off[k].get(); j.counts = m->d_counts[k].get(); j.R = m->d_R[k].get();
    j.seg_nbl = m->seg_nbl; j.seg_first = m->seg_first; j.seg_total = m->seg_total; j.seg_world = m->seg_world; j.seg_pref = m->seg_cur;
    return j;
}

int ddc_mfma_set_segment(DdcMfma *m, int nbl, int first, int total, int world, int *pref_cur, int *pref_next)
{
    m->seg_nbl = nbl; m->seg_first = first; m->seg_total = total; m->seg_world = world; m->seg_cur = pref_cur; m->seg_next = pref_next;
    return 0;
}
int ddc_mfma_pending_blocks(const DdcMfma *m) { return m->pending_blocks[m->drain]; }
int ddc_mfma_skip_batch(DdcMfma *m, DdcChanState *d_state, const ChanGeom *d_geom)
{
    if (!m->seg_nbl) return fail_msg(-3, "fastddc: skip_batch outside a time-sliced bank");
    DdcChainJob j = mfma_chain_job(m, m->fill, 0, d_state, d_geom);
    hipLaunchKernelGGL(k_ddc_chain_t, dim3(cdiv(m->C, 64)), dim3(64), 0, m->ctx->stream, j);
    CSDR_LAUNCH_CHECK();
    m->spec_valid = false;
    return 0;
}
static int mfma_chains(DdcMfma *m, hipStream_t st, int k, int n_blocks, DdcChanState *d_state, const ChanGeom *d_geom)
{
    const DdcChainJob j = mfma_chain_job(m, k, n_blocks, d_state, d_geom);
    hipLaunchKernelGGL(k_ddc_chain_t, dim3(cdiv(m->C, 64)), dim3(64), 0, st, j);
    CSDR_LAUNCH_CHECK();
    hipLaunchKernelGGL(k_ddc_rot, dim3(cdiv((size_t)m->C * n_blocks, 64)), dim3(64), 0, st, j);
    CSDR_LAUNCH_CHECK();
    return 0;
}

template <int FMT> __global__ __launch_bounds__(256) void k_ddc_cvt_tail(const void *__restrict__ in, long long first, int n, float2 *__restrict__ out)
{
    const int i = blockIdx.x * 256 + threadIdx.x;
    if (i < n) out[i] = ddc_in_sample<FMT>(in, first + i);
}
int ddc_mfma_convert_samples(hipStream_t st, const void *in, int fmt, long long first, int n, cf32 *out)
{
    if (fmt == 1) hipLaunchKernelGGL(k_ddc_cvt_tail<1>, dim3(cdiv(n, 256)), dim3(256), 0, st, in, first, n, reinterpret_cast<float2 *>(out));
    else if (fmt == 2) hipLaunchKernelGGL(k_ddc_cvt_tail<2>, dim3(cdiv(n, 256)), dim3(256), 0, st, in, first, n, reinterpret_cast<float2 *>(out));
    else CSDR_HIP(hipMemcpyAsync(out, reinterpret_cast<const cf32 *>(in) + first, sizeof(cf32) * (size_t)n, hipMemcpyDeviceToDevice, st));
    CSDR_LAUNCH_CHECK();
    return 0;
}

static int mfma_forward(DdcMfma *m, hipStream_t st, const void *in, int fmt, const cf32 *tail, cf32 *tail_out, int n_loc, cf32 *xt, const DdcChainJob *riders, bool skip_pass2 = false)
{
    if (n_loc <= 0) return 0;
    DdcChainJob cj; memset(&cj, 0, sizeof cj);
    if (riders) cj = *riders;
    const size_t rider_lanes = riders ? (cj.mode == 2 ? (size_t)cj.n_channels * cj.n_blocks : (size_t)cj.n_channels) : 0;
#define DDC_FWD_ARGS in, reinterpret_cast<const float2 *>(tail), reinterpret_cast<float2 *>(tail_out), \
                     reinterpret_cast<float2 *>(m->d_Y.get()), m->d_tw.get(), m->d_twb.get(), m->input_size, m->overlap, n_loc, cj
    if (m->stages_timed()) { if (const int rc = m->stage[0].timer.begin(st)) return rc; }
    {
        const size_t lds = (size_t)(16 * I512<16>::pitch + 512 + 128) * sizeof(float2);
        const dim3 grid(8, n_loc + (riders ? cdiv(rider_lanes, 8 * 256) : 0));
#define DDC_FWD_LAUNCH(F) do { const int rc = lds_attr_once((const void *)k_ddc_fwd512<16, F>, lds); if (rc) return rc; \
                               hipLaunchKernelGGL((k_ddc_fwd512<16, F>), grid, dim3(256), lds, st, DDC_FWD_ARGS); } while (0)
        if (fmt == 1) DDC_FWD_LAUNCH(1); else if (fmt == 2) DDC_FWD_LAUNCH(2); else DDC_FWD_LAUNCH(0);
#undef DDC_FWD_LAUNCH
    }
#undef DDC_FWD_ARGS
    CSDR_LAUNCH_CHECK();
    if (m->stages_timed()) { if (const int rc = m->stage[0].timer.end(st)) return rc; }
    const bool rot_rides = !skip_pass2 && riders && cj.mode == 1 && (size_t)cj.n_channels * cj.n_blocks <= 512u * 256u;
    if (!rot_rides) cj.R = nullptr;
    if (!skip_pass2)
    hipLaunchKernelGGL(k_ddc_fwd128, dim3(512, cdiv(n_loc, 32) + (rot_rides ? 1 : 0)), dim3(256), 0, st, reinterpret_cast<const float2 *>(m->d_Y.get()), reinterpret_cast<float2 *>(xt),
                       m->d_tw.get(), m->nbl, n_loc, cj);
    CSDR_LAUNCH_CHECK();
    if (riders && cj.mode == 1 && !rot_rides) {
        hipLaunchKernelGGL(k_ddc_rot, dim3(cdiv((size_t)m->C * cj.n_blocks, 64)), dim3(64), 0, st, *riders);
        CSDR_LAUNCH_CHECK();
    }
    return 0;
}

static bool ddc_folds_with_gemm3(const DdcMfma *m, int n_blocks)
{
    const int nbt = ddc_fold_tiles(m->pre, n_blocks);
    const size_t lds = ddc_fold_lds(m->pre, nbt);
    const int per_res = (int)(cdiv(m->Cpad, 256) * cdiv(n_blocks, 32 * nbt));
    int slots = current_device_cu_count() / per_res; if (slots < 1) slots = 1; if (slots > m->inv) slots = m->inv;
    bool persist = m->pre <= 128 && 2 * lds <= DDC_LDS_MAX - 512 && slots * 2 <= m->inv;
    return persist && m->pre == 128;
}

static bool ddc_fold_is_narrow(const DdcMfma *m, int n_blocks)
{
    static const bool off = getenv("CSDR_AMD_DDC_NARROW") && atoi(getenv("CSDR_AMD_DDC_NARROW")) == 0;
    return !off && m->Cpad <= 128 && (m->inv & (m->inv - 1)) == 0 && ddc_folds_with_gemm3(m, n_blocks);
}

int ddc_mfma_submit(DdcMfma *m, const void *in_v, const cf32 *spectra, int n_blocks, DdcChanState *d_state, const ChanGeom *d_geom, bool inline_call, const cf32 *ext_tail,
                    int fmt, bool tail_in_front)
{
    if (fmt < 0 || fmt > 2) return fail_msg(-3, "fastddc: unknown input format %d", fmt);
    const size_t es = ddc_in_bytes(fmt);
    const uint8_t *in = reinterpret_cast<const uint8_t *>(in_v);
    if (n_blocks <= 0) return fail_msg(-3, "fastddc: nothing to submit");
    if (n_blocks > m->max_blocks) return fail_msg(-3, "fastddc: %d blocks exceed max_blocks %d", n_blocks, m->max_blocks);
    const int k = m->fill;
    if (m->pending_blocks[k]) return fail_msg(-3, "fastddc: two calls are already staged; collect one first");
    hipStream_t mainst = m->ctx->stream;
    const bool inl = inline_call && m->world == 1 && !m->pending_blocks[k ^ 1];
    const int chains_side = 0;
    hipStream_t st = inl ? mainst : m->side.get();
    int rc = 0;
    const bool riders_off = m->opt.riders_off, spec_off = m->opt.spec_off;
    const bool fused_fwd = inl && !chains_side && !spectra && ddc_mfma_can_forward(m);
    const bool spec_hit = fused_fwd && m->spec_valid && m->spec_set == k && m->spec_blocks == n_blocks && m->spec_seg_first == m->seg_first && m->spec_seg_total == m->seg_total;
    m->spec_valid = false;
    const bool ride = fused_fwd && !riders_off;
    m->last_state = d_state; m->ahead_ok = fused_fwd && !spec_off && !riders_off;
    m->y_holds[k] = false;
    m->front[k] = spectra ? "k_ddc_xt+" : fmt == 1 ? "k_ddc_fwd512<16,1>+" : fmt == 2 ? "k_ddc_fwd512<16,2>+" : "k_ddc_fwd512<16,0>+";
    m->front2[k] = spectra ? "" : "k_ddc_fwd128+";
    if (ride) {
    } else if (inl && !chains_side) {
        rc = mfma_chains(m, mainst, k, n_blocks, d_state, d_geom); if (rc) return rc;
    } else {
        CSDR_HIP(hipEventRecord(m->ev_fork.get(), mainst));
        CSDR_HIP(hipStreamWaitEvent(m->side.get(), m->ev_fork.get(), 0));
        rc = mfma_chains(m, m->side.get(), k, n_blocks, d_state, d_geom); if (rc) return rc;
    }
    if (spectra) {
        if (m->world > 1) return fail_msg(-3, "fastddc: natural-order spectra cannot feed a sharded bank");
        hipLaunchKernelGGL(k_ddc_xt, dim3(cdiv(m->inv, 32), cdiv(m->pre, 32), n_blocks), dim3(256), 0, st, reinterpret_cast<const float2 *>(spectra),
                           reinterpret_cast<float2 *>(m->d_Xt[k].get()), m->fft, m->inv, m->pre, m->nbl);
        CSDR_LAUNCH_CHECK();
    } else {
        if (!ddc_mfma_can_forward(m)) return fail_msg(-3, "fastddc: the fused forward transform covers fft_size 65536 / pre_decimation 128 only");
        const int inp = m->input_size, ovl = m->overlap;
        if (!m->d_Y) return fail_msg(-3, "fastddc: forward buffers missing");
        if (m->world == 1) {
            DdcChainJob job = mfma_chain_job(m, k, n_blocks, d_state, d_geom);
            if (spec_hit) { job.mode = 2; job.state_out = m->d_state_spec.get(); }
            const bool fuse2_off = m->opt.pass2_own;
            const bool skip2 = inl && !fuse2_off && ddc_folds_with_gemm3(m, n_blocks) && !ddc_fold_is_narrow(m, n_blocks);
            if (tail_in_front) rc = mfma_forward(m, st, in, fmt, nullptr, nullptr, n_blocks, m->d_Xt[k].get(), ride ? &job : nullptr, skip2);
            else if (ext_tail) rc = mfma_forward(m, st, in, fmt, ext_tail, nullptr, n_blocks, m->d_Xt[k].get(), ride ? &job : nullptr, skip2);
            else { rc = mfma_forward(m, st, in, fmt, m->d_tail[m->flip].get(), m->d_tail[m->flip ^ 1].get(), n_blocks, m->d_Xt[k].get(), ride ? &job : nullptr, skip2); m->flip ^= 1; }
            if (rc) return rc;
            m->y_holds[k] = skip2;
            if (skip2) m->front2[k] = "";
        } else {
            const DdcComm *cm = m->comm;
            auto first_of = [&](int g) { return g * m->nbl < n_blocks ? g * m->nbl : n_blocks; };
            const int b0 = first_of(m->rank), b1 = first_of(m->rank + 1), n_loc = b1 - b0;
            rc = cm->group_start(cm); if (rc) return rc;
            if (m->rank == 0) {
                for (int g = 1; g < m->world; g++) {
                    const int g0 = first_of(g), g1 = first_of(g + 1);
                    if (g1 > g0) { rc = cm->send(cm, in + ((size_t)g0 * inp - ovl) * es, ((size_t)(g1 - g0) * inp + ovl) * es / 4, g, st); if (rc) return rc; }
                }
            } else if (n_loc > 0) { rc = cm->recv(cm, m->d_in_local.get(), ((size_t)n_loc * inp + ovl) * es / 4, 0, st); if (rc) return rc; }
            rc = cm->group_end(cm); if (rc) return rc;
            cf32 *chunk = m->d_Xt[k].get() + (size_t)m->rank * m->inv * m->nbl * m->pre;
            if (m->rank == 0) {
                rc = mfma_forward(m, st, in, fmt, m->d_tail[m->flip].get(), nullptr, n_loc, chunk, nullptr); if (rc) return rc;
                rc = ddc_mfma_convert_samples(st, in, fmt, (long long)n_blocks * inp - ovl, ovl, m->d_tail[m->flip ^ 1].get()); if (rc) return rc;
                m->flip ^= 1;
            } else { rc = mfma_forward(m, st, reinterpret_cast<const uint8_t *>(m->d_in_local.get()) + (size_t)ovl * es, fmt, nullptr, nullptr, n_loc, chunk, nullptr); if (rc) return rc; }
            rc = cm->all_gather(cm, m->d_Xt[k].get(), 2 * (size_t)m->inv * m->nbl * m->pre, st); if (rc) return rc;
        }
    }
    if (!(inl && !chains_side)) CSDR_HIP(hipEventRecord(m->ev_ready[k].get(), m->side.get()));
    m->inline_set[k] = inl; m->chains_on_side[k] = !(inl && !chains_side);
    m->pending_blocks[k] = n_blocks; m->fill ^= 1;
    return 0;
}

const char *ddc_mfma_kernel_name(const DdcMfma *m) { return m->gemm_three ? (m->gemm_narrow ? "k_ddc_gemm3n" : "k_ddc_gemm3") : "k_ddc_gemm"; }
const char *ddc_mfma_kernels(const DdcMfma *m) { return m->kernels.c_str(); }
static void mfma_note_kernels(DdcMfma *m, int k, const char *fold, const char *inverse) { m->kernels.clear(); m->kernels.append(m->front[k]).append(m->front2[k]).append(fold).append("+").append(inverse); }
int ddc_mfma_set_profiling(DdcMfma *m, int on)
{
    m->profiling = on != 0; m->timer.reset(); m->prof_ms = 0; m->prof_launches = 0;
    m->profile_stages = on == 2;
    for (auto &p : m->stage) { p.timer.reset(); p.ms = 0; p.launches = 0; }
    return 0;
}
int ddc_mfma_stage_time(DdcMfma *m, int stage, double *total_ms, long *launches)
{
    if (stage < 1 || stage > 2) return -3;
    DdcMfma::StageProf &p = m->stage[stage - 1];
    if (const int rc = p.timer.resolve(&p.ms, &p.launches)) return rc;
    *total_ms = p.ms; *launches = p.launches;
    return 0;
}
int ddc_mfma_kernel_time(DdcMfma *m, double *total_ms, long *launches)
{
    if (const int rc = m->timer.resolve(&m->prof_ms, &m->prof_launches)) return rc;
    *total_ms = m->prof_ms; *launches = m->prof_launches;
    return 0;
}

int ddc_mfma_collect(DdcMfma *m, const ChanGeom *d_geom, cf32 *out, size_t out_pitch, const int **d_counts, hipEvent_t after_inverse)
{
    const int k = m->drain, n_blocks = m->pending_blocks[k];
    if (!n_blocks) return fail_msg(-3, "fastddc: nothing staged to collect");
    hipStream_t st = m->ctx->stream;
    if (m->chains_on_side[k]) CSDR_HIP(hipStreamWaitEvent(st, m->ev_ready[k].get(), 0));
    const float scale = 1.0f / (float)m->pre;
    const int nbt = ddc_fold_tiles(m->pre, n_blocks);
    const size_t lds = ddc_fold_lds(m->pre, nbt);
    const dim3 grid(m->inv, cdiv(m->Cpad, 256), cdiv(n_blocks, 32 * nbt));
    if (m->profiling) { if (const int rc = m->timer.begin(st)) return rc; }
    const int n_cu = current_device_cu_count();
    const int per_res = (int)(grid.y * grid.z);
    int slots = n_cu / per_res; if (slots < 1) slots = 1; if (slots > m->inv) slots = m->inv;
    bool persist = m->pre <= 128 && 2 * lds <= DDC_LDS_MAX - 512 && slots * 2 <= m->inv;
    const size_t lds_use = persist ? 2 * lds : lds;
    const dim3 grid_use(persist ? (unsigned)slots : grid.x, grid.y, grid.z);
#define DDC_GEMM_LAUNCH(NBTV, PV) do {                                                                                                               \
        if (lds_use > 64 * 1024) { const int rc = lds_attr_once((const void *)k_ddc_gemm<NBTV, PV>, lds_use); if (rc) return rc; }                    \
        hipLaunchKernelGGL((k_ddc_gemm<NBTV, PV>), grid_use, dim3(512), lds_use, st, m->d_Ht.get(), reinterpret_cast<const float2 *>(m->d_Xt[k].get()),           \
                           reinterpret_cast<float2 *>(m->d_Ct.get()), d_geom, m->inv, m->pre, m->Cpad, m->C, m->nbp, m->nbl, n_blocks, scale); } while (0)
    const bool three = ddc_folds_with_gemm3(m, n_blocks);
    m->gemm_three = three; m->gemm_narrow = false;
    const char *fold = "";
    if (three) {
        const bool fwd = m->y_holds[k];
        const float2 *src = fwd ? reinterpret_cast<const float2 *>(m->d_Y.get()) : reinterpret_cast<const float2 *>(m->d_Xt[k].get());
#define DDC_GEMM3_LAUNCH(NBTV, FV) do { const int rc = lds_attr_once((const void *)k_ddc_gemm3<NBTV, FV>, lds_use); if (rc) return rc;                     \
        hipLaunchKernelGGL((k_ddc_gemm3<NBTV, FV>), grid_use, dim3(512), lds_use, st, m->d_Ht.get(), src, reinterpret_cast<float2 *>(m->d_Ct.get()), d_geom, m->inv, m->Cpad, m->C,  \
                           m->nbp, m->nbl, n_blocks, scale, m->d_tw.get()); } while (0)
        m->gemm_narrow = !fwd && ddc_fold_is_narrow(m, n_blocks);
        if (m->gemm_narrow) {
            const dim3 gn(m->inv, 1, cdiv(n_blocks, 32));
            const size_t ldsn = (size_t)32 * (m->pre / 2 + 1) * sizeof(float4);
#define DDC_GEMM3N_LAUNCH(NWV) hipLaunchKernelGGL((k_ddc_gemm3n<NWV>), gn, dim3(64 * NWV), ldsn, st, m->d_Ht.get(), src, reinterpret_cast<float2 *>(m->d_Ct.get()), d_geom, m->inv, m->Cpad, m->C, \
                                                  m->nbp, m->nbl, n_blocks, scale)
            if (m->Cpad <= 32) DDC_GEMM3N_LAUNCH(1); else if (m->Cpad <= 64) DDC_GEMM3N_LAUNCH(2); else DDC_GEMM3N_LAUNCH(4);
            fold = m->Cpad <= 32 ? "k_ddc_gemm3n<1>" : m->Cpad <= 64 ? "k_ddc_gemm3n<2>" : "k_ddc_gemm3n<4>";
#undef DDC_GEMM3N_LAUNCH
        }
        else if (nbt == 2) { if (fwd) DDC_GEMM3_LAUNCH(2, true); else DDC_GEMM3_LAUNCH(2, false); }
        else          { if (fwd) DDC_GEMM3_LAUNCH(1, true); else DDC_GEMM3_LAUNCH(1, false); }
#undef DDC_GEMM3_LAUNCH
        if (!m->gemm_narrow) fold = nbt == 2 ? (fwd ? "k_ddc_gemm3<2,true>" : "k_ddc_gemm3<2,false>") : (fwd ? "k_ddc_gemm3<1,true>" : "k_ddc_gemm3<1,false>");
    }
    else if (nbt == 2) { if (persist) DDC_GEMM_LAUNCH(2, true); else DDC_GEMM_LAUNCH(2, false); }
    else               { if (persist) DDC_GEMM_LAUNCH(1, true); else DDC_GEMM_LAUNCH(1, false); }
#undef DDC_GEMM_LAUNCH
    if (!three) fold = nbt == 2 ? (persist ? "k_ddc_gemm<2,true>" : "k_ddc_gemm<2,false>") : (persist ? "k_ddc_gemm<1,true>" : "k_ddc_gemm<1,false>");
    mfma_note_kernels(m, k, fold, m->post_dec != 2 ? "k_ddc_ifft512_post<8>" : "k_ddc_ifft256d_post<8>");
    CSDR_LAUNCH_CHECK();
    if (m->profiling) { if (const int rc = m->timer.end(st)) return rc; }
    const bool full = m->post_dec != 2;
    const int pairs = m->C * cdiv(n_blocks, 16);
    const dim3 g8(cdiv(pairs, 8) * 16);
    if (m->stages_timed()) { if (const int rc = m->stage[1].timer.begin(st)) return rc; }
#define DDC_IFFT_ARGS reinterpret_cast<const float2 *>(m->d_Ct.get()), reinterpret_cast<float2 *>(out), out_pitch, m->d_R[k].get(), m->d_tw.get(), m->d_blk_remain[k].get(), m->d_blk_off[k].get(), d_geom, m->Cpad, m->nbp, n_blocks, m->C, m->scrap, m->post_in
    DdcChainJob ahead; memset(&ahead, 0, sizeof ahead);
    if (full) {
        hipLaunchKernelGGL(k_ddc_ifft512_post<8>, g8, dim3(256), (size_t)(8 * I512<8>::pitch + I512<8>::tw_n) * sizeof(float2), st, DDC_IFFT_ARGS, m->post_dec);
    } else {
        int n_riders = 0;
        if (m->ahead_ok && m->inline_set[k] && m->last_state && m->C <= 16 * 256) {
            ahead = mfma_chain_job(m, k ^ 1, n_blocks, m->last_state, d_geom);
            ahead.state_out = m->d_state_spec.get(); ahead.seg_pref = m->seg_next;
            n_riders = 16;
            m->spec_valid = true; m->spec_set = k ^ 1; m->spec_blocks = n_blocks; m->spec_seg_first = m->seg_first; m->spec_seg_total = m->seg_total;
        }
        if (after_inverse) hipExtLaunchKernelGGL(k_ddc_ifft256d_post<8>, dim3(g8.x + n_riders), dim3(256), (size_t)(8 * I256<8>::pitch + 512) * sizeof(float2), st, nullptr, after_inverse, 0, DDC_IFFT_ARGS, ahead, n_riders);
        else
        hipLaunchKernelGGL(k_ddc_ifft256d_post<8>, dim3(g8.x + n_riders), dim3(256), (size_t)(8 * I256<8>::pitch + 512) * sizeof(float2), st, DDC_IFFT_ARGS, ahead, n_riders);
        after_inverse = nullptr;
    }
#undef DDC_IFFT_ARGS
    CSDR_LAUNCH_CHECK();
    if (m->stages_timed()) { if (const int rc = m->stage[1].timer.end(st)) return rc; }
    if (after_inverse) CSDR_HIP(hipEventRecord(after_inverse, st));
    if (d_counts) *d_counts = m->d_counts[k].get();
    m->pending_blocks[k] = 0; m->drain ^= 1;
    return n_blocks;
}

}

extern "C" int csdr_amd_debug_ddc_chain(int mode, float rate2, int post_in, int post_dec, int n_blocks, int *remain_io, float *phase_io, float *phases_out, int *count_out)
{
    using namespace csdr_amd;
    DdcChanState s{*remain_io, *phase_io};
    const int sh = (post_dec & (post_dec - 1)) == 0 ? __builtin_ctz(post_dec) : -1;
    int total = 0;
    if (mode == 1) {
        const DdcChainFast f = ddc_chain_fast(s, rate2, post_in, post_dec);
        if (!f.ok) return -1;
        float p = s.phase;
        for (int b = 0; b < n_blocks; b++) { phases_out[b] = p; p = ddc_phase_step(p, f.d, f.big); total += f.k; }
        s.phase = p;
    } else {
        for (int b = 0; b < n_blocks; b++) { phases_out[b] = s.phase; total += ddc_chain_step(s, rate2, post_in, post_dec, sh); }
    }
    *remain_io = s.remain; *phase_io = s.phase; *count_out = total;
    return 0;
}

extern "C" int csdr_amd_debug_ddc_fold_plan(int pre, int n_blocks, int *tiles, long *lds_bytes)
{
    using namespace csdr_amd;
    if (ddc_fold_lds(pre, 1) > DDC_LDS_MAX) return -1;
    *tiles = ddc_fold_tiles(pre, n_blocks); *lds_bytes = (long)ddc_fold_lds(pre, *tiles);
    return 0;
}

extern "C" void csdr_amd_debug_dft8(const float *in16, float *out16, int inverse)
{
    float2 v[8];
    for (int k = 0; k < 8; k++) v[k] = make_float2(in16[2 * k], in16[2 * k + 1]);
    if (inverse) dft8<true>(v); else dft8<false>(v);
    for (int k = 0; k < 8; k++) { out16[2 * k] = v[k].x; out16[2 * k + 1] = v[k].y; }
}
```

### csdr_amd/csrc/fftpath.hip

```cpp
#include "common.hpp"
#include "fastddc.hpp"
#include <hipfft/hipfft.h>

struct csdr_amd_comm;
namespace csdr_amd { const DdcComm *csdr_amd_comm_ddc(csdr_amd_comm *c); }
#include <math.h>
#include <vector>
#include <map>
#include <tuple>
#include <mutex>
#include <string.h>
using namespace csdr_amd;

#define CSDR_FFT(expr) do { hipfftResult r__ = (expr); if (r__ != HIPFFT_SUCCESS) return ::csdr_amd::fail_msg(-5, "hipFFT error %d at %s:%d: %s", (int)r__, __FILE__, __LINE__, #expr); } while (0)

namespace {

__global__ __launch_bounds__(256) void k_oa_frame(const cf32 *__restrict__ in, size_t in_pitch, cf32 *__restrict__ padded,
                                                  int fft, int inp, int n_blocks)
{
    const int k = blockIdx.x * 256 + threadIdx.x;
    if (k >= fft) return;
    const size_t s = blockIdx.z, b = blockIdx.y;
    cf32 v = cf32{0.f, 0.f};
// ... 441 lines not shown
    if (e == hipSuccess) e = dev_alloc(f->d_tail[0], sizeof(cf32) * (size_t)(ddc->overlap_length + 1));
    if (e == hipSuccess) e = dev_alloc(f->d_tail[1], sizeof(cf32) * (size_t)(ddc->overlap_length + 1));
    if (e != hipSuccess) { fail(e, "hipMalloc(fastddc_fwd)", __FILE__, __LINE__); return nullptr; }
    (void)hipMemsetAsync(f->d_tail[0].get(), 0, sizeof(cf32) * (size_t)(ddc->overlap_length + 1), ctx->stream);
    (void)hipMemsetAsync(f->d_tail[1].get(), 0, sizeof(cf32) * (size_t)(ddc->overlap_length + 1), ctx->stream);
    return f.release();
}

void csdr_amd_fastddc_fwd_destroy(csdr_amd_fastddc_fwd *f)
{
    if (!f) return;
    (void)hipStreamSynchronize(f->ctx->stream);
    delete f;
}

int csdr_amd_fastddc_fwd_process(csdr_amd_fastddc_fwd *f, const csdr_complexf *in, csdr_complexf *spectra, int n_blocks)
{
    if (n_blocks <= 0) return 0;
    if (n_blocks > f->max_blocks) return fail_msg(-3, "fastddc_fwd: %d blocks exceed max_blocks %d", n_blocks, f->max_blocks);
    hipStream_t st = f->ctx->stream;
    const int fft = f->ddc.fft_size, inp = f->ddc.input_size, ovl = f->ddc.overlap_length;
    if (!f->plans.count(n_blocks)) {
        hipfftHandle h; int n[1] = {fft};
        CSDR_FFT(hipfftPlanMany(&h, 1, n, nullptr, 1, fft, nullptr, 1, fft, HIPFFT_C2C, n_blocks));
        FftPlan owned(h);
        CSDR_FFT(hipfftSetStream(h, st));
        f->plans[n_blocks] = std::move(owned);
    }
    hipLaunchKernelGGL(k_os_frame, dim3(cdiv(fft, 256), n_blocks), dim3(256), 0, st, in, f->d_tail[f->flip].get(), f->d_win.get(), fft, inp, ovl); CSDR_LAUNCH_CHECK();
    CSDR_FFT(hipfftExecC2C(f->plans[n_blocks].get(), (hipfftComplex *)f->d_win.get(), (hipfftComplex *)spectra, HIPFFT_FORWARD));
    hipLaunchKernelGGL(k_os_tail, dim3(cdiv(ovl, 256)), dim3(256), 0, st, in, f->d_tail[f->flip].get(), f->d_tail[f->flip ^ 1].get(), inp, ovl, n_blocks); CSDR_LAUNCH_CHECK();
    f->flip ^= 1;
    return 0;
}

}

struct csdr_amd_fastddc_inv {
    csdr_amd_ctx *ctx; int n_channels, max_blocks;
    float tbw; int decimation, window;
    std::vector<csdr_fastddc_t> geom;
    DevBuf<cf32> d_H, d_inv_in, d_td;
    DevBuf<ChanGeom> d_geom; DevBuf<DdcChanState> d_state;
    DevBuf<int> d_blk_remain, d_blk_off, d_counts; DevBuf<float> d_blk_phase;
    Owned<DdcMfma, ddc_mfma_destroy> mf;
    std::map<int, FftPlan> plans;
    bool fold_old;
    const char *kernels = "";
};

extern "C" {

static csdr_amd_fastddc_inv *fastddc_inv_create_comm(csdr_amd_ctx *ctx, float transition_bw, int decimation, const float *shift_rates,
                                                     int n_channels, int window, int max_blocks, const DdcComm *comm);
csdr_amd_fastddc_inv *csdr_amd_fastddc_inv_create(csdr_amd_ctx *ctx, float transition_bw, int decimation, const float *shift_rates,
                                                  int n_channels, int window, int max_blocks)
{
    return fastddc_inv_create_comm(ctx, transition_bw, decimation, shift_rates, n_channels, window, max_blocks, nullptr);
}
static csdr_amd_fastddc_inv *fastddc_inv_create_comm(csdr_amd_ctx *ctx, float transition_bw, int decimation, const float *shift_rates,
                                                     int n_channels, int window, int max_blocks, const DdcComm *comm)
{
    if (n_channels < 1 || max_blocks < 1) { fail_msg(-3, "fastddc_inv: bad sizes"); return nullptr; }
    Owned<csdr_amd_fastddc_inv, csdr_amd_fastddc_inv_destroy> f(new csdr_amd_fastddc_inv());
    f->ctx = ctx; f->n_channels = n_channels; f->max_blocks = max_blocks; f->fold_old = getenv("CSDR_AMD_DDC_FOLD_OLD") != nullptr;
    f->tbw = transition_bw; f->decimation = decimation; f->window = window;
    f->geom.resize(n_channels);
    std::vector<ChanGeom> cg(n_channels);
    for (int c = 0; c < n_channels; c++) {
        if (csdr_amd_fastddc_init(&f->geom[c], transition_bw, decimation, shift_rates[c])) { fail_msg(-3, "fastddc_init failed (fft_size <= 2)"); return nullptr; }
        cg[c].offsetbin = f->geom[c].offsetbin; cg[c].sindelta = f->geom[c].dsadata.sindelta; cg[c].cosdelta = f->geom[c].dsadata.cosdelta; cg[c].rate2 = f->geom[c].dsadata.rate;
    }
    const csdr_fastddc_t &g = f->geom[0];
    const int fft = g.fft_size, inv = g.fft_inv_size;
    f->mf.reset(ddc_mfma_create(ctx, fft, inv, g.pre_decimation, n_channels, max_blocks, g.scrap, g.post_input_size, g.post_decimation, g.input_size, g.overlap_length, comm));
    hipError_t e = dev_alloc(f->d_H, sizeof(cf32) * (size_t)n_channels * fft);
    if (!f->mf) {
        if (e == hipSuccess) e = dev_alloc(f->d_inv_in, sizeof(cf32) * (size_t)n_channels * max_blocks * inv);
        if (e == hipSuccess) e = dev_alloc(f->d_td, sizeof(cf32) * (size_t)n_channels * max_blocks * inv);
    }
    if (e == hipSuccess) e = dev_alloc(f->d_geom, sizeof(ChanGeom) * n_channels);
    if (e == hipSuccess) e = dev_alloc(f->d_state, sizeof(DdcChanState) * n_channels);
    if (e == hipSuccess) e = dev_alloc(f->d_blk_remain, sizeof(int) * (size_t)n_channels * max_blocks);
    if (e == hipSuccess) e = dev_alloc(f->d_blk_off, sizeof(int) * (size_t)n_channels * max_blocks);
    if (e == hipSuccess) e = dev_alloc(f->d_blk_phase, sizeof(float) * (size_t)n_channels * max_blocks);
    if (e == hipSuccess) e = dev_alloc(f->d_counts, sizeof(int) * n_channels);
    if (e != hipSuccess) { fail(e, "hipMalloc(fastddc_inv)", __FILE__, __LINE__); return nullptr; }
    (void)hipMemcpy(f->d_geom.get(), cg.data(), sizeof(ChanGeom) * n_channels, hipMemcpyHostToDevice);
    (void)hipMemset(f->d_state.get(), 0, sizeof(DdcChanState) * n_channels);
    {
        std::vector<cf32> taps((size_t)n_channels * fft, cf32{0.f, 0.f});
        std::vector<cf32> one(g.taps_length);
        const float half_bw = 0.5f / (float)decimation;
        for (int c = 0; c < n_channels; c++) {
            csdr_amd_firdes_bandpass_c(one.data(), g.taps_length, (-shift_rates[c]) - half_bw, (-shift_rates[c]) + half_bw, window);
            for (int k = 0; k < g.taps_length; k++) taps[(size_t)c * fft + k] = one[k];
        }
        (void)hipMemcpy(f->d_H.get(), taps.data(), sizeof(cf32) * taps.size(), hipMemcpyHostToDevice);
        static std::map<std::tuple<int, int, int>, hipfftHandle> taps_plans;
        static std::mutex taps_mu;
        std::lock_guard<std::mutex> lk(taps_mu);
        (void)hipSetDevice(ctx->device);
        const auto key = std::make_tuple(ctx->device, fft, n_channels);
        if (!taps_plans.count(key)) {
            hipfftHandle h; int n[1] = {fft};
            if (hipfftPlanMany(&h, 1, n, nullptr, 1, fft, nullptr, 1, fft, HIPFFT_C2C, n_channels) != HIPFFT_SUCCESS) { fail_msg(-5, "hipfftPlanMany(taps) failed"); return nullptr; }
            taps_plans[key] = h;
        }
        hipfftHandle h = taps_plans[key];
        hipfftSetStream(h, ctx->stream);
        hipfftExecC2C(h, (hipfftComplex *)f->d_H.get(), (hipfftComplex *)f->d_H.get(), HIPFFT_FORWARD);
        const size_t total = (size_t)n_channels * fft;
        hipLaunchKernelGGL(k_swap_halves, dim3(cdiv(total / 2, 256)), dim3(256), 0, ctx->stream, f->d_H.get(), fft, total);
        if (f->mf && ddc_mfma_set_taps(f->mf.get(), ctx->stream, f->d_H.get(), 0, n_channels)) return nullptr;
        (void)hipStreamSynchronize(ctx->stream);
    }
    return f.release();
}

int csdr_amd_fastddc_inv_set_rate(csdr_amd_fastddc_inv *f, int channel, float shift_rate)
{
    if (!f || channel < 0 || channel >= f->n_channels) return fail_msg(-3, "fastddc_inv_set_rate: bad channel");
    csdr_amd_ctx *ctx = f->ctx;
    csdr_fastddc_t g;
    if (csdr_amd_fastddc_init(&g, f->tbw, f->decimation, shift_rate)) return fail_msg(-3, "fastddc_init failed");
    f->geom[channel] = g;
    ChanGeom cg; cg.offsetbin = g.offsetbin; cg.sindelta = g.dsadata.sindelta; cg.cosdelta = g.dsadata.cosdelta; cg.rate2 = g.dsadata.rate;
    const int fft = g.fft_size;
    std::vector<cf32> taps((size_t)fft, cf32{0.f, 0.f});
    const float half_bw = 0.5f / (float)f->decimation;
    csdr_amd_firdes_bandpass_c((csdr_complexf *)taps.data(), g.taps_length, (-shift_rate) - half_bw, (-shift_rate) + half_bw, f->window);
    if (f->mf) { const int qrc = ddc_mfma_quiesce(f->mf.get()); if (qrc) return qrc; }
    CSDR_HIP(hipStreamSynchronize(ctx->stream));
    CSDR_HIP(hipMemcpy(f->d_geom.get() + channel, &cg, sizeof(ChanGeom), hipMemcpyHostToDevice));
    CSDR_HIP(hipMemset(f->d_state.get() + channel, 0, sizeof(DdcChanState)));
    cf32 *row = f->d_H.get() + (size_t)channel * fft;
    CSDR_HIP(hipMemcpy(row, taps.data(), sizeof(cf32) * (size_t)fft, hipMemcpyHostToDevice));
    int rc = csdr_amd_fft_c2c(ctx, (const csdr_complexf *)row, (csdr_complexf *)row, fft, 1); if (rc) return rc;
    hipLaunchKernelGGL(k_swap_halves, dim3(cdiv((size_t)fft / 2, 256)), dim3(256), 0, ctx->stream, row, fft, (size_t)fft);
    CSDR_LAUNCH_CHECK();
    if (f->mf) { rc = ddc_mfma_set_taps(f->mf.get(), ctx->stream, f->d_H.get(), channel, 1); if (rc) return rc; }
    CSDR_HIP(hipStreamSynchronize(ctx->stream));
    return 0;
}

void csdr_amd_fastddc_inv_destroy(csdr_amd_fastddc_inv *f)
{
    if (!f) return;
    (void)hipStreamSynchronize(f->ctx->stream);
    delete f;
}

const char *csdr_amd_fastddc_inv_kernel_name(const csdr_amd_fastddc_inv *f) { return f->mf ? ddc_mfma_kernel_name(f->mf.get()) : "k_ddc_fold_ct"; }
const char *csdr_amd_fastddc_inv_kernels(const csdr_amd_fastddc_inv *f) { return f->mf ? ddc_mfma_kernels(f->mf.get()) : f->kernels; }
int csdr_amd_fastddc_inv_set_profiling(csdr_amd_fastddc_inv *f, int on) { return f->mf ? ddc_mfma_set_profiling(f->mf.get(), on) : 0; }
int csdr_amd_fastddc_inv_kernel_time(csdr_amd_fastddc_inv *f, double *total_ms, long *launches)
{
    *total_ms = 0; *launches = 0;
    return f->mf ? ddc_mfma_kernel_time(f->mf.get(), total_ms, launches) : 0;
}
int csdr_amd_fastddc_inv_stage_time(csdr_amd_fastddc_inv *f, int stage, double *total_ms, long *launches)
{
    *total_ms = 0; *launches = 0;
    return f->mf ? ddc_mfma_stage_time(f->mf.get(), stage, total_ms, launches) : 0;
}

int csdr_amd_fastddc_inv_geometry(const csdr_amd_fastddc_inv *f, int channel, csdr_fastddc_t *ddc)
{
    if (channel < 0 || channel >= f->n_channels) return fail_msg(-3, "fastddc_inv: channel out of range");
    *ddc = f->geom[channel]; return 0;
}

int csdr_amd_fastddc_inv_max_output(const csdr_amd_fastddc_inv *f, int n_blocks)
{
    const csdr_fastddc_t &g = f->geom[0];
    return n_blocks * (g.post_input_size / g.post_decimation + 1);
}

int csdr_amd_fastddc_inv_process(csdr_amd_fastddc_inv *f, const csdr_complexf *spectra, int n_blocks, csdr_complexf *out, size_t out_pitch, int *out_counts)
{
    if (n_blocks <= 0) return 0;
    if (n_blocks > f->max_blocks) return fail_msg(-3, "fastddc_inv: %d blocks exceed max_blocks %d", n_blocks, f->max_blocks);
    hipStream_t st = f->ctx->stream;
    const csdr_fastddc_t &g = f->geom[0];
    const int fft = g.fft_size, inv = g.fft_inv_size, pre = g.pre_decimation;
    if ((size_t)csdr_amd_fastddc_inv_max_output(f, n_blocks) > out_pitch) return fail_msg(-3, "fastddc_inv: out_pitch too small");
    if (f->mf) {
        int rc = ddc_mfma_submit(f->mf.get(), nullptr, spectra, n_blocks, f->d_state.get(), f->d_geom.get(), true); if (rc) return rc;
        const int *d_cnt = nullptr;
        rc = ddc_mfma_collect(f->mf.get(), f->d_geom.get(), out, out_pitch, &d_cnt); if (rc < 0) return rc;
        if (out_counts) {
            CSDR_HIP(hipMemcpyAsync(out_counts, d_cnt, sizeof(int) * f->n_channels, hipMemcpyDeviceToHost, st));
            CSDR_HIP(hipStreamSynchronize(st));
        }
        return 0;
    }
    const int batch = f->n_channels * n_blocks;
    if (!f->plans.count(batch)) {
        hipfftHandle h; int n[1] = {inv};
        CSDR_FFT(hipfftPlanMany(&h, 1, n, nullptr, 1, inv, nullptr, 1, inv, HIPFFT_C2C, batch));
        FftPlan owned(h);
        CSDR_FFT(hipfftSetStream(h, st));
        f->plans[batch] = std::move(owned);
    }
    const bool ct_ok = f->n_channels >= 4 && pre >= 2 && (pre & (pre - 1)) == 0 && !f->fold_old;
#define FOLD_CT(CTV, BTV) hipLaunchKernelGGL((k_ddc_fold_ct<CTV, BTV>), dim3(cdiv(inv, 256), cdiv(n_blocks, BTV), cdiv(f->n_channels, CTV)), dim3(256), 0, st, spectra, f->d_H.get(), f->d_inv_in.get(), f->d_geom.get(), fft, inv, pre, n_blocks, f->n_channels)
    if (ct_ok && f->n_channels >= 8) { FOLD_CT(8, 4); f->kernels = "k_ddc_fold_ct<8,4>+hipfft+k_ddc_post"; }
    else if (ct_ok) { FOLD_CT(4, 4); f->kernels = "k_ddc_fold_ct<4,4>+hipfft+k_ddc_post"; }
#undef FOLD_CT
    else if (n_blocks >= 16) {
        f->kernels = "k_ddc_fold<16>+hipfft+k_ddc_post";
        hipLaunchKernelGGL((k_ddc_fold<16>), dim3(cdiv(inv, 256), cdiv(n_blocks, 16), f->n_channels), dim3(256), 0, st, spectra, f->d_H.get(), f->d_inv_in.get(), f->d_geom.get(), fft, inv, pre, n_blocks);
    } else {
        f->kernels = "k_ddc_fold<4>+hipfft+k_ddc_post";
        hipLaunchKernelGGL((k_ddc_fold<4>), dim3(cdiv(inv, 256), cdiv(n_blocks, 4), f->n_channels), dim3(256), 0, st, spectra, f->d_H.get(), f->d_inv_in.get(), f->d_geom.get(), fft, inv, pre, n_blocks);
    }
    CSDR_LAUNCH_CHECK();
    CSDR_FFT(hipfftExecC2C(f->plans[batch].get(), (hipfftComplex *)f->d_inv_in.get(), (hipfftComplex *)f->d_td.get(), HIPFFT_BACKWARD));
    hipLaunchKernelGGL(k_ddc_chain, dim3(cdiv(f->n_channels, 64)), dim3(64), 0, st, f->d_state.get(), f->d_geom.get(), f->n_channels, n_blocks, g.post_input_size, g.post_decimation,
                       f->d_blk_remain.get(), f->d_blk_phase.get(), f->d_blk_off.get(), f->d_counts.get()); CSDR_LAUNCH_CHECK();
    hipLaunchKernelGGL(k_ddc_post, dim3(cdiv((size_t)batch, 64)), dim3(64), 0, st, f->d_td.get(), out, out_pitch, f->d_geom.get(), f->n_channels, n_blocks, inv, g.scrap,
                       g.post_input_size, g.post_decimation, f->d_blk_remain.get(), f->d_blk_phase.get(), f->d_blk_off.get()); CSDR_LAUNCH_CHECK();
    if (out_counts) {
        CSDR_HIP(hipMemcpyAsync(out_counts, f->d_counts.get(), sizeof(int) * f->n_channels, hipMemcpyDeviceToHost, st));
        CSDR_HIP(hipStreamSynchronize(st));
    }
    return 0;
}

}

struct csdr_amd_fastddc_bank {
    csdr_amd_ctx *ctx; int max_blocks; bool fused;
    csdr_amd_comm *comm; int first_channel, n_channels_total; int staged[2], n_staged;
    const int *last_counts = nullptr; int last_count_n = 0;
    int shard_mode = CSDR_AMD_SHARD_CHANNELS; const DdcComm *dc = nullptr; int world = 1, rank = 0, nbl = 0, out_count = 0;
    csdr_amd_comm *comm_out = nullptr; const DdcComm *dc_out = nullptr;
    size_t pitch_loc = 0;
    Event ev_fork, ev_in_ready[2], ev_in_free[2], ev_out_ready[2], ev_done[2];
    DevBuf<cf32> d_in_loc[2], d_out_loc[2], d_recv[2], d_tail_root[2];
    DevBuf<int> d_pref[3]; int tail_flip = 0, pref_at = 0;
    DevBuf<cf32> d_spec;
    Owned<csdr_amd_fastddc_inv, csdr_amd_fastddc_inv_destroy> inv;
    Owned<csdr_amd_fastddc_fwd, csdr_amd_fastddc_fwd_destroy> fwd;
    Stream xin, xout;
    bool in_free_rec[2] = {false, false}, done_rec[2] = {false, false};
    struct Batch { int n_glob; const uint8_t *in; bool local; int fmt; } batch[2]; int fill = 0, drain = 0, n_batches = 0, last_slot = -1;
    struct Retune { long first_batch; int channel; float rate; }; std::vector<Retune> deferred; long seq_submit = 0, seq_collect = 0;
};

static void shard_slice(int n, int world, int rank, int *first, int *count)
{
    const int base = n / world, extra = n % world;
    *count = base + (rank < extra ? 1 : 0); *first = rank * base + (rank < extra ? rank : extra);
}

__global__ __launch_bounds__(256) void k_bank_stitch(const float2 *__restrict__ own, const float2 *__restrict__ recv, const int *__restrict__ pref, float2 *__restrict__ out,
                                                     size_t pitch_loc, size_t out_pitch, int n_total, int first, int count, int me)
{
    const int cc = blockIdx.x, g = blockIdx.y;
    const int at = pref[(size_t)g * n_total + first + cc], cnt = pref[(size_t)(g + 1) * n_total + first + cc] - at;
    const float2 *src = g == me ? own + (size_t)(first + cc) * pitch_loc : recv + ((size_t)g * count + cc) * pitch_loc;
    float2 *dst = out + (size_t)cc * out_pitch + at;
    const int per = (cnt + (int)gridDim.z - 1) / (int)gridDim.z, t0 = (int)blockIdx.z * per, t1 = min(t0 + per, cnt);
    for (int t = t0 + (int)threadIdx.x; t < t1; t += 256) dst[t] = src[t];
}
__global__ __launch_bounds__(64) void k_bank_counts(const int *__restrict__ pref, int *__restrict__ counts, int n_total, int first, int count, int world)
{
    const int cc = blockIdx.x * 64 + threadIdx.x;
    if (cc < count) counts[cc] = pref[(size_t)world * n_total + first + cc];
}

static csdr_amd_fastddc_bank *bank_create(csdr_amd_ctx *ctx, float transition_bw, int decimation, const float *host_shift_rates, int n_channels,
                                          int window, int max_blocks, csdr_amd_comm *comm, int shard_mode)
{
    Owned<csdr_amd_fastddc_bank, csdr_amd_fastddc_bank_destroy> b(new csdr_amd_fastddc_bank());
    b->ctx = ctx; b->max_blocks = max_blocks; b->comm = comm; b->n_staged = 0;
    b->first_channel = 0; b->n_channels_total = n_channels;
    int count = n_channels;
    const DdcComm *dc = comm ? csdr_amd_comm_ddc(comm) : nullptr;
    const bool multi = dc && dc->world > 1;
    if (multi) {
        shard_slice(n_channels, dc->world, dc->rank, &b->first_channel, &count);
        if (count < 1) { fail_msg(-3, "fastddc_bank: fewer channels than ranks"); return nullptr; }
        b->dc = dc; b->world = dc->world; b->rank = dc->rank; b->out_count = count;
    }
    b->shard_mode = multi ? shard_mode : CSDR_AMD_SHARD_CHANNELS;
    if (b->shard_mode == CSDR_AMD_SHARD_BLOCKS) {
        b->nbl = (max_blocks + b->world - 1) / b->world;
        b->comm_out = csdr_amd_comm_dup(comm);
        if (!b->comm_out) return nullptr;
        b->dc_out = csdr_amd_comm_ddc(b->comm_out);
        b->inv.reset(fastddc_inv_create_comm(ctx, transition_bw, decimation, host_shift_rates, n_channels, window, b->nbl, nullptr));
    } else
        b->inv.reset(fastddc_inv_create_comm(ctx, transition_bw, decimation, host_shift_rates + b->first_channel, count, window, max_blocks, multi ? dc : nullptr));
    if (!b->inv) return nullptr;
    b->fused = ddc_mfma_can_forward(b->inv->mf.get());
    if (multi && !b->fused) { fail_msg(-3, "fastddc_bank: sharding needs the geometry of the matrix-core path (fft_size 65536, fft_inv_size 512)"); return nullptr; }
    const csdr_fastddc_t g = b->inv->geom[0];
    if (multi && g.input_size < g.overlap_length) { fail_msg(-3, "fastddc_bank: sharding needs input_size >= overlap_length"); return nullptr; }
    if (!b->fused) {
        b->fwd.reset(csdr_amd_fastddc_fwd_create(ctx, &g, max_blocks));
        if (!b->fwd || dev_alloc(b->d_spec, sizeof(cf32) * (size_t)max_blocks * g.fft_size) != hipSuccess) {
            fail_msg(-2, "fastddc_bank: cannot allocate the spectrum buffer"); return nullptr; }
    }
    if (b->shard_mode == CSDR_AMD_SHARD_BLOCKS) {
// ... 291 lines not shown
```

### include/csdr_amd.h

```cpp
#ifndef CSDR_AMD_H
#define CSDR_AMD_H
#include <stddef.h>
#include <stdint.h>

#ifdef __cplusplus
extern "C" {
#endif

typedef struct csdr_complexf_s { float i, q; } csdr_complexf;

typedef enum { CSDR_WINDOW_BOXCAR = 0, CSDR_WINDOW_BLACKMAN = 1, CSDR_WINDOW_HAMMING = 2 } csdr_window_t;

typedef struct csdr_amd_ctx csdr_amd_ctx;

csdr_amd_ctx *csdr_amd_ctx_create(int device, void *hip_stream);
void          csdr_amd_ctx_destroy(csdr_amd_ctx *ctx);
int           csdr_amd_ctx_sync(csdr_amd_ctx *ctx);
void         *csdr_amd_ctx_stream(csdr_amd_ctx *ctx);
const char   *csdr_amd_last_error(void);
int           csdr_amd_device_count(void);
const char   *csdr_amd_device_arch(csdr_amd_ctx *ctx);

void *csdr_amd_malloc(csdr_amd_ctx *ctx, size_t bytes);
void  csdr_amd_free(csdr_amd_ctx *ctx, void *dptr);
// ... 186 lines not shown
char csdr_amd_rtty_baudot_decoder_push(csdr_amd_rtty_push_state *s, unsigned char symbol);
void csdr_amd_firdes_add_peak_c(csdr_complexf *output, int length, float rate, int window, int add, int normalize);
void csdr_amd_firdes_peak_c(csdr_complexf *taps, int length, float rate, int window);
long long csdr_amd_debug_rtty_walk(const csdr_amd_rtty_params *params, int first_stage, int last_stage, const void *in, long long n, const long long *cuts,
                                   int n_cuts, void *out);

typedef struct csdr_amd_squelch csdr_amd_squelch;
csdr_amd_squelch *csdr_amd_squelch_create(csdr_amd_ctx *ctx, int n_channels, int block_size, int use_every_nth, const float *levels, long long max_samples_per_call);
int  csdr_amd_squelch_process(csdr_amd_squelch *s, const csdr_complexf *in, long long n_in, size_t in_pitch, csdr_complexf *out, size_t out_pitch, float *power,
                              size_t power_pitch, uint8_t *open_flags, int *n_blocks_out);
int  csdr_amd_squelch_set_level(csdr_amd_squelch *s, int channel, float level);
float csdr_amd_squelch_get_level(const csdr_amd_squelch *s, int channel);
long long csdr_amd_squelch_block_index(const csdr_amd_squelch *s, int channel);
int  csdr_amd_squelch_max_blocks(const csdr_amd_squelch *s);
int  csdr_amd_squelch_reset(csdr_amd_squelch *s);
int  csdr_amd_squelch_reset_channel(csdr_amd_squelch *s, int channel);
int  csdr_amd_squelch_force_generic(csdr_amd_squelch *s, int on);
const char *csdr_amd_squelch_kernel_name(const csdr_amd_squelch *s);
void csdr_amd_squelch_destroy(csdr_amd_squelch *s);
int  csdr_amd_get_power_c(csdr_amd_ctx *ctx, const csdr_complexf *in, int n_streams, int n_blocks, int block_size, int decimation, size_t in_pitch, float *power_out);
int  csdr_amd_get_power_f(csdr_amd_ctx *ctx, const float *in, int n_streams, int n_blocks, int block_size, int decimation, size_t in_pitch, float *power_out);
int  csdr_amd_squelch_report_due(int report_every_nth, long long block_index);
int  csdr_amd_squelch_gate_open(float power, float level);
float csdr_amd_debug_squelch_power(const float *in, int block_size, int decimation, int is_complex);

enum { CSDR_AMD_CARRIER_COSTAS = 0, CSDR_AMD_CARRIER_COSTAS_DD = 1, CSDR_AMD_CARRIER_PLL_P = 2, CSDR_AMD_CARRIER_PLL_PI = 3 };
typedef struct csdr_amd_carrier_params { int mode; float alpha, beta, dphase_max; int dphase_max_reset_to_zero; } csdr_amd_carrier_params;
typedef struct csdr_amd_carrier_chan { float phase, dphase, freq; } csdr_amd_carrier_chan;
typedef struct csdr_amd_carrier csdr_amd_carrier;
int  csdr_amd_costas_params(float bandwidth, float damping, int decision_directed, csdr_amd_carrier_params *p);
int  csdr_amd_pll_params_p(float alpha, csdr_amd_carrier_params *p);
int  csdr_amd_pll_params_pi(float bandwidth, float ko, float kd, float damping, csdr_amd_carrier_params *p);
csdr_amd_carrier *csdr_amd_carrier_create(csdr_amd_ctx *ctx, const csdr_amd_carrier_params *params, int n_channels);
int  csdr_amd_carrier_process(csdr_amd_carrier *p, const csdr_complexf *in, long long n, size_t in_pitch, csdr_complexf *out, float *error, float *dphase,
                              csdr_complexf *nco, size_t out_pitch);
int  csdr_amd_carrier_reset(csdr_amd_carrier *p);
int  csdr_amd_carrier_reset_channel(csdr_amd_carrier *p, int channel);
int  csdr_amd_carrier_get_channel(csdr_amd_carrier *p, int channel, csdr_amd_carrier_chan *out);
int  csdr_amd_carrier_set_channel(csdr_amd_carrier *p, int channel, const csdr_amd_carrier_chan *state);
int  csdr_amd_carrier_set_lanes(csdr_amd_carrier *p, int lanes);
int  csdr_amd_carrier_lanes(const csdr_amd_carrier *p);
int  csdr_amd_carrier_force_generic(csdr_amd_carrier *p, int on);
const char *csdr_amd_carrier_kernel_name(const csdr_amd_carrier *p);
void csdr_amd_carrier_destroy(csdr_amd_carrier *p);
long long csdr_amd_debug_carrier_walk(const csdr_amd_carrier_params *params, const csdr_complexf *in, long long n, const long long *cuts, int n_cuts,
                                      csdr_complexf *out, float *error, float *dphase, csdr_complexf *nco, csdr_amd_carrier_chan *state_io);

int csdr_amd_fmmod_fc(csdr_amd_ctx *ctx, const float *in, csdr_complexf *out, int n_streams, size_t n, size_t in_pitch, size_t out_pitch, float *phase_io);
int csdr_amd_dsb_fc(csdr_amd_ctx *ctx, const float *in, csdr_complexf *out, size_t n, float q_value);
int csdr_amd_add_dcoffset_cc(csdr_amd_ctx *ctx, const csdr_complexf *in, csdr_complexf *out, size_t n);
int csdr_amd_fixed_amplitude_cc(csdr_amd_ctx *ctx, const csdr_complexf *in, csdr_complexf *out, size_t n, float new_amplitude);
int csdr_amd_convert_f_samplerf(csdr_amd_ctx *ctx, const float *in, void *out, size_t n, unsigned wait_for_this_sample);
long long csdr_amd_debug_fmmod_walk(const float *in, long long n, const long long *cuts, int n_cuts, float *phases, csdr_complexf *out, float *state_io);

enum { CSDR_TX_FM = 0, CSDR_TX_AM = 1, CSDR_TX_DSB = 2 };
enum { CSDR_TX_OUT_CF32 = 0, CSDR_TX_OUT_U8 = 1 };
typedef struct csdr_amd_txbank csdr_amd_txbank;
csdr_amd_txbank *csdr_amd_txbank_create(csdr_amd_ctx *ctx, int n_streams, int mode, float gain, float q_value, int interpolation, const float *host_taps,
                                        int taps_length, const float *shift_rates, int out_format, size_t max_in_samples);
int  csdr_amd_txbank_process(csdr_amd_txbank *p, const int16_t *in_s16, size_t in_pitch, long long n_in, void *out, size_t out_pitch, long long *n_out);
int  csdr_amd_txbank_set_rate(csdr_amd_txbank *p, int stream, float rate);
float csdr_amd_txbank_get_rate(const csdr_amd_txbank *p, int stream);
int  csdr_amd_txbank_reset(csdr_amd_txbank *p);
long long csdr_amd_txbank_max_out(const csdr_amd_txbank *p, long long n_in);
int  csdr_amd_txbank_force_generic(csdr_amd_txbank *p, int on);
const char *csdr_amd_txbank_kernel_name(const csdr_amd_txbank *p);
void csdr_amd_txbank_destroy(csdr_amd_txbank *p);

int csdr_amd_amdemod_cf(csdr_amd_ctx *ctx, const csdr_complexf *in, float *out, size_t n);
int csdr_amd_amdemod_estimator_cf(csdr_amd_ctx *ctx, const csdr_complexf *in, float *out, size_t n, float alpha, float beta);
int csdr_amd_realpart_cf(csdr_amd_ctx *ctx, const csdr_complexf *in, float *out, size_t n);
int csdr_amd_logpower_cf(csdr_amd_ctx *ctx, const csdr_complexf *in, float *out, size_t n, float add_db);
int csdr_amd_fmdemod_atan_cf(csdr_amd_ctx *ctx, const csdr_complexf *in, float *out, int n_streams, size_t n,
                             size_t in_pitch, size_t out_pitch, float *last_phase_io);
int csdr_amd_dcblock_ff(csdr_amd_ctx *ctx, const float *in, float *out, int n_streams, size_t n, size_t in_pitch, size_t out_pitch,
                        float a, float *state_io);
int csdr_amd_fastdcblock_ff(csdr_amd_ctx *ctx, const float *in, float *out, int n_streams, int n_blocks, int block,
                            size_t in_pitch, size_t out_pitch, float *last_dc_io);
int csdr_amd_agc_ff(csdr_amd_ctx *ctx, const float *in, float *out, int n_streams, size_t n, int block, size_t in_pitch, size_t out_pitch,
                    float reference, float attack_rate, float decay_rate, float max_gain, short hang_time, short attack_wait_time,
                    float gain_filter_alpha, float *last_gain_io);
void csdr_amd_precalculate_window(float *host_windowt, int size, int window);
typedef struct csdr_amd_fftcc csdr_amd_fftcc;
csdr_amd_fftcc *csdr_amd_fftcc_create(csdr_amd_ctx *ctx, int fft_size, int every_n_samples, int window, int max_frames);
void csdr_amd_fftcc_destroy(csdr_amd_fftcc *f);
int  csdr_amd_fftcc_process(csdr_amd_fftcc *f, const csdr_complexf *in, size_t n_in, csdr_complexf *out, size_t *consumed);

typedef struct csdr_amd_waterfall csdr_amd_waterfall;
enum { CSDR_AMD_WF_IN_CF32 = 0, CSDR_AMD_WF_IN_U8 = 1 };
enum { CSDR_AMD_WF_OUT_DB = 0, CSDR_AMD_WF_OUT_ADPCM = 1 };
csdr_amd_waterfall *csdr_amd_waterfall_create(csdr_amd_ctx *ctx, int fft_size, int every_n_samples, int window, int avgnumber,
                                              float add_db, int in_format, int out_format, int n_streams, size_t max_samples_per_call);
int  csdr_amd_waterfall_process(csdr_amd_waterfall *w, const void *in, size_t n_in, size_t in_pitch, void *out, size_t out_pitch, int *rows_out);
int  csdr_amd_waterfall_reset(csdr_amd_waterfall *w);
const char *csdr_amd_waterfall_kernel_name(const csdr_amd_waterfall *w);
int  csdr_amd_waterfall_force_generic(csdr_amd_waterfall *w, int on);
void csdr_amd_waterfall_destroy(csdr_amd_waterfall *w);
int  csdr_amd_logaveragepower_cf(csdr_amd_ctx *ctx, const csdr_complexf *in, float *out, int n_rows, int fft_size, int avgnumber, float add_db);
int  csdr_amd_fft_exchange_sides_ff(csdr_amd_ctx *ctx, const float *in, float *out, int n_rows, int fft_size);
int  csdr_amd_accumulate_power_cf(csdr_amd_ctx *ctx, const csdr_complexf *in, float *acc_io, size_t n);
int  csdr_amd_log_ff(csdr_amd_ctx *ctx, const float *in, float *out, size_t n, float add_db);

int csdr_amd_encode_ima_adpcm_i16_u8(csdr_amd_ctx *ctx, const int16_t *in, uint8_t *out, int n_streams, size_t n,
                                     size_t in_pitch, size_t out_pitch, int *state_io);
int csdr_amd_decode_ima_adpcm_u8_i16(csdr_amd_ctx *ctx, const uint8_t *in, int16_t *out, int n_streams, size_t n,
                                     size_t in_pitch, size_t out_pitch, int *state_io);
int csdr_amd_compress_fft_adpcm_f_u8(csdr_amd_ctx *ctx, const float *in, uint8_t *out, int n_blocks, int fft_size);

typedef struct csdr_amd_fftfilt csdr_amd_fftfilt;
csdr_amd_fftfilt *csdr_amd_fftfilt_create(csdr_amd_ctx *ctx, int fft_size, const csdr_complexf *host_taps,
                                          int taps_length, int n_streams, int max_blocks);
void csdr_amd_fftfilt_destroy(csdr_amd_fftfilt *f);
int  csdr_amd_fftfilt_set_taps(csdr_amd_fftfilt *f, const csdr_complexf *host_taps, int taps_length);
csdr_amd_fftfilt *csdr_amd_fftfilt_create_per_stream(csdr_amd_ctx *ctx, int fft_size, const csdr_complexf *host_taps,
                                                     int taps_length, int n_streams, int max_blocks);
int  csdr_amd_fftfilt_set_stream_taps(csdr_amd_fftfilt *f, int stream, const csdr_complexf *host_taps, int taps_length);
int  csdr_amd_fftfilt_per_stream(const csdr_amd_fftfilt *f);
int  csdr_amd_fftfilt_input_size(const csdr_amd_fftfilt *f);
const char *csdr_amd_fftfilt_kernel_name(const csdr_amd_fftfilt *f);
int  csdr_amd_fftfilt_window(const csdr_amd_fftfilt *f);
int  csdr_amd_fftfilt_reset(csdr_amd_fftfilt *f);
int  csdr_amd_fftfilt_process(csdr_amd_fftfilt *f, const csdr_complexf *in, csdr_complexf *out,
                              int n_blocks, size_t in_pitch, size_t out_pitch);

int csdr_amd_fft_c2c(csdr_amd_ctx *ctx, const csdr_complexf *in, csdr_complexf *out, int n, int forward);
int csdr_amd_bin_product(csdr_amd_ctx *ctx, const csdr_complexf *a, const csdr_complexf *b, csdr_complexf *out, size_t n);
int csdr_amd_scale_add(csdr_amd_ctx *ctx, csdr_complexf *io, size_t n, float scale, const csdr_complexf *add, size_t n_add);

typedef struct csdr_fastddc_s {
    int pre_decimation, post_decimation, taps_length, taps_min_length, overlap_length,
        fft_size, fft_inv_size, input_size, post_input_size;
    float pre_shift; int startbin, v, offsetbin; float post_shift; int output_scrape, scrap;
    struct { float sindelta, cosdelta, rate; } dsadata;
} csdr_fastddc_t;
int csdr_amd_fastddc_init(csdr_fastddc_t *ddc, float transition_bw, int decimation, float shift_rate);

typedef struct csdr_amd_fastddc_fwd csdr_amd_fastddc_fwd;
csdr_amd_fastddc_fwd *csdr_amd_fastddc_fwd_create(csdr_amd_ctx *ctx, const csdr_fastddc_t *ddc, int max_blocks);
void csdr_amd_fastddc_fwd_destroy(csdr_amd_fastddc_fwd *f);
int  csdr_amd_fastddc_fwd_process(csdr_amd_fastddc_fwd *f, const csdr_complexf *in, csdr_complexf *spectra, int n_blocks);

typedef struct csdr_amd_fastddc_inv csdr_amd_fastddc_inv;
csdr_amd_fastddc_inv *csdr_amd_fastddc_inv_create(csdr_amd_ctx *ctx, float transition_bw, int decimation,
                                                  const float *host_shift_rates, int n_channels, int window,
                                                  int max_blocks);
void csdr_amd_fastddc_inv_destroy(csdr_amd_fastddc_inv *f);
int  csdr_amd_fastddc_inv_set_rate(csdr_amd_fastddc_inv *f, int channel, float shift_rate);
int  csdr_amd_fastddc_inv_geometry(const csdr_amd_fastddc_inv *f, int channel, csdr_fastddc_t *ddc);
int  csdr_amd_fastddc_inv_max_output(const csdr_amd_fastddc_inv *f, int n_blocks);
int  csdr_amd_fastddc_inv_process(csdr_amd_fastddc_inv *f, const csdr_complexf *spectra, int n_blocks,
                                  csdr_complexf *out, size_t out_pitch, int *out_counts);
const char *csdr_amd_fastddc_inv_kernel_name(const csdr_amd_fastddc_inv *f);
const char *csdr_amd_fastddc_inv_kernels(const csdr_amd_fastddc_inv *f);
int  csdr_amd_fastddc_inv_set_profiling(csdr_amd_fastddc_inv *f, int on);
int  csdr_amd_fastddc_inv_kernel_time(csdr_amd_fastddc_inv *f, double *total_ms, long *launches);
int  csdr_amd_fastddc_inv_stage_time(csdr_amd_fastddc_inv *f, int stage, double *total_ms, long *launches);
typedef struct csdr_amd_fastddc_bank csdr_amd_fastddc_bank;
csdr_amd_fastddc_bank *csdr_amd_fastddc_bank_create(csdr_amd_ctx *ctx, float transition_bw, int decimation, const float *host_shift_rates, int n_channels,
                                                    int window, int max_blocks);
void csdr_amd_fastddc_bank_destroy(csdr_amd_fastddc_bank *b);
int  csdr_amd_fastddc_bank_set_rate(csdr_amd_fastddc_bank *b, int channel, float shift_rate);
int  csdr_amd_fastddc_bank_input_size(const csdr_amd_fastddc_bank *b);
int  csdr_amd_fastddc_bank_max_output(const csdr_amd_fastddc_bank *b, int n_blocks);
int  csdr_amd_fastddc_bank_process(csdr_amd_fastddc_bank *b, const csdr_complexf *in, int n_blocks, csdr_complexf *out, size_t out_pitch, int *out_counts);
int  csdr_amd_fastddc_bank_submit(csdr_amd_fastddc_bank *b, const csdr_complexf *in, int n_blocks);
int  csdr_amd_fastddc_bank_collect(csdr_amd_fastddc_bank *b, csdr_complexf *out, size_t out_pitch, int *out_counts);

typedef struct csdr_amd_comm csdr_amd_comm;
int  csdr_amd_comm_unique_id(char id128[128]);
csdr_amd_comm *csdr_amd_comm_create(csdr_amd_ctx *ctx, const char id128[128], int rank, int world);
void csdr_amd_comm_destroy(csdr_amd_comm *c);
int  csdr_amd_comm_rank(const csdr_amd_comm *c);
int  csdr_amd_comm_world(const csdr_amd_comm *c);
int  csdr_amd_comm_broadcast(csdr_amd_comm *c, void *dev_buf, size_t bytes, int root);
csdr_amd_comm *csdr_amd_comm_dup(csdr_amd_comm *c);
int  csdr_amd_comm_selftest(csdr_amd_comm *c, size_t n_floats, char *report, size_t report_cap);
typedef struct csdr_amd_loopback csdr_amd_loopback;
csdr_amd_loopback *csdr_amd_loopback_create(int world);
void csdr_amd_loopback_destroy(csdr_amd_loopback *g);
void csdr_amd_loopback_abort(csdr_amd_loopback *g);
csdr_amd_comm *csdr_amd_comm_create_loopback(csdr_amd_ctx *ctx, csdr_amd_loopback *g, int rank);
csdr_amd_comm *csdr_amd_comm_create_null(csdr_amd_ctx *ctx, int rank, int world);
csdr_amd_comm *csdr_amd_comm_create_ipc(csdr_amd_ctx *ctx, const char *path_prefix, int rank, int world);
int csdr_amd_debug_comm_exchange(csdr_amd_comm *c, const float *send_buf, float *recv_buf, size_t n, int peer, int n_sends);
enum { CSDR_AMD_SHARD_CHANNELS = 0, CSDR_AMD_SHARD_BLOCKS = 1 };
csdr_amd_fastddc_bank *csdr_amd_fastddc_bank_create_sharded(csdr_amd_ctx *ctx, float transition_bw, int decimation, const float *host_shift_rates_all, int n_channels_total,
                                                            int window, int max_blocks, csdr_amd_comm *comm);
csdr_amd_fastddc_bank *csdr_amd_fastddc_bank_create_sharded_by(csdr_amd_ctx *ctx, float transition_bw, int decimation, const float *host_shift_rates_all, int n_channels_total,
                                                               int window, int max_blocks, csdr_amd_comm *comm, int shard_mode);
int  csdr_amd_fastddc_bank_channel_slice(const csdr_amd_fastddc_bank *b, int *first, int *count);
int  csdr_amd_fastddc_bank_shard_mode(const csdr_amd_fastddc_bank *b);
int  csdr_amd_fastddc_bank_default_shard_mode(int world);
int  csdr_amd_fastddc_bank_local_blocks(const csdr_amd_fastddc_bank *b, int n_blocks, int *first, int *count);
int  csdr_amd_fastddc_bank_overlap(const csdr_amd_fastddc_bank *b);
int  csdr_amd_fastddc_bank_submit_local(csdr_amd_fastddc_bank *b, const csdr_complexf *in_run, int n_blocks);
int  csdr_amd_fastddc_bank_process_s16(csdr_amd_fastddc_bank *b, const int16_t *in_iq, int n_blocks, csdr_complexf *out, size_t out_pitch, int *out_counts);
int  csdr_amd_fastddc_bank_process_u8(csdr_amd_fastddc_bank *b, const uint8_t *in_iq, int n_blocks, csdr_complexf *out, size_t out_pitch, int *out_counts);
int  csdr_amd_fastddc_bank_submit_s16(csdr_amd_fastddc_bank *b, const int16_t *in_iq, int n_blocks);
int  csdr_amd_fastddc_bank_submit_u8(csdr_amd_fastddc_bank *b, const uint8_t *in_iq, int n_blocks);
int  csdr_amd_fastddc_bank_submit_local_s16(csdr_amd_fastddc_bank *b, const int16_t *in_run_iq, int n_blocks);
int  csdr_amd_fastddc_bank_submit_local_u8(csdr_amd_fastddc_bank *b, const uint8_t *in_run_iq, int n_blocks);
int  csdr_amd_fastddc_bank_finish(csdr_amd_fastddc_bank *b, int *out_counts);
int  csdr_amd_fastddc_bank_set_rate_global(csdr_amd_fastddc_bank *b, int channel, float shift_rate);
csdr_amd_fastddc_inv *csdr_amd_fastddc_bank_inverse(csdr_amd_fastddc_bank *b);

int  csdr_amd_fastddc_inv_block(csdr_amd_ctx *ctx, const csdr_complexf *d_spectrum, const csdr_complexf *d_taps_fft,
                                const csdr_fastddc_t *ddc, void *status_io, csdr_complexf *d_inv_in, csdr_complexf *d_td,
                                csdr_complexf *d_out);

typedef struct csdr_amd_wfm csdr_amd_wfm;
csdr_amd_wfm *csdr_amd_wfm_create(csdr_amd_ctx *ctx, int n_streams, float shift_rate, int decimation,
                                  const float *host_taps, int taps_length, int frac_rate,
                                  float tau, int audio_rate, size_t max_block_samples);
csdr_amd_wfm *csdr_amd_wfm_create_rates(csdr_amd_ctx *ctx, int n_streams, const float *shift_rates, int decimation,
                                        const float *host_taps, int taps_length, int frac_rate,
                                        float tau, int audio_rate, size_t max_block_samples);
int   csdr_amd_wfm_set_rate(csdr_amd_wfm *w, int stream, float shift_rate);
float csdr_amd_wfm_get_rate(const csdr_amd_wfm *w, int stream);
void csdr_amd_wfm_destroy(csdr_amd_wfm *w);
int  csdr_amd_wfm_reset(csdr_amd_wfm *w);
long csdr_amd_wfm_process(csdr_amd_wfm *w, const uint8_t *in, size_t in_pitch, size_t block_samples,
                          int16_t *audio_s16, float *audio_f, size_t out_pitch);
const char *csdr_amd_wfm_kernel_name(const csdr_amd_wfm *w);
int csdr_amd_wfm_fallback(const csdr_amd_wfm *w);
int csdr_amd_wfm_set_profiling(csdr_amd_wfm *w, int on);
int csdr_amd_wfm_kernel_time(csdr_amd_wfm *w, double *total_ms, long *launches);

typedef struct csdr_amd_wfm_ring csdr_amd_wfm_ring;
csdr_amd_wfm_ring *csdr_amd_wfm_ring_create(csdr_amd_ctx *ctx, int n_streams, float shift_rate, int decimation, const float *host_taps, int taps_length, int frac_rate,
                                            float tau, int audio_rate, size_t block_samples, int n_slots);
void csdr_amd_wfm_ring_destroy(csdr_amd_wfm_ring *r);
int  csdr_amd_wfm_ring_reset(csdr_amd_wfm_ring *r);
int  csdr_amd_wfm_ring_acquire(csdr_amd_wfm_ring *r, long long seq, double timeout_s);
uint8_t *csdr_amd_wfm_ring_input(csdr_amd_wfm_ring *r, long long seq, size_t *pitch_bytes);
long long csdr_amd_wfm_ring_submit(csdr_amd_wfm_ring *r);
long csdr_amd_wfm_ring_wait(csdr_amd_wfm_ring *r, long long seq, double timeout_s);
const int16_t *csdr_amd_wfm_ring_output(csdr_amd_wfm_ring *r, long long seq, size_t *pitch_samples);
int  csdr_amd_wfm_ring_set_rate(csdr_amd_wfm_ring *r, float shift_rate);
float csdr_amd_wfm_ring_get_rate(const csdr_amd_wfm_ring *r);
int  csdr_amd_wfm_ring_set_timeouts(csdr_amd_wfm_ring *r, double idle_us, double life_ms);
int  csdr_amd_wfm_ring_resident(csdr_amd_wfm_ring *r);
int  csdr_amd_wfm_ring_stop(csdr_amd_wfm_ring *r);
int  csdr_amd_wfm_ring_slots(const csdr_amd_wfm_ring *r);
int  csdr_amd_wfm_ring_grid(const csdr_amd_wfm_ring *r);
long csdr_amd_wfm_ring_launches(const csdr_amd_wfm_ring *r);
long long csdr_amd_wfm_ring_submitted(const csdr_amd_wfm_ring *r);
int  csdr_amd_wfm_ring_stats(csdr_amd_wfm_ring *r, double out[4]);
int  csdr_amd_wfm_ring_replay(csdr_amd_wfm_ring *r, long n_blocks, double *t_first_us, double *t_done_us);
int  csdr_amd_wfm_ring_block_times(csdr_amd_wfm_ring *r, long long seq, double *t_first_us, double *t_done_us);

typedef struct csdr_amd_ddc csdr_amd_ddc;
csdr_amd_ddc *csdr_amd_ddc_create(csdr_amd_ctx *ctx, int n_streams, float shift_rate, int decimation,
                                  const float *host_taps, int taps_length, size_t max_block_samples);
csdr_amd_ddc *csdr_amd_ddc_create_rates(csdr_amd_ctx *ctx, int n_streams, const float *shift_rates, int decimation,
                                        const float *host_taps, int taps_length, size_t max_block_samples);
int   csdr_amd_ddc_set_rate(csdr_amd_ddc *d, int stream, float shift_rate);
float csdr_amd_ddc_get_rate(const csdr_amd_ddc *d, int stream);
int   csdr_amd_ddc_fallback(const csdr_amd_ddc *d);
void csdr_amd_ddc_destroy(csdr_amd_ddc *d);
int  csdr_amd_ddc_reset(csdr_amd_ddc *d);
long csdr_amd_ddc_process(csdr_amd_ddc *d, const uint8_t *in, size_t in_pitch, size_t block_samples,
                          csdr_complexf *out, size_t out_pitch);
const char *csdr_amd_ddc_kernel_name(const csdr_amd_ddc *d);
int csdr_amd_ddc_set_profiling(csdr_amd_ddc *d, int on);
int csdr_amd_ddc_kernel_time(csdr_amd_ddc *d, double *total_ms, long *launches);
int csdr_amd_debug_ddc_mfma_tile(int D, int L, float shift_rate, const float *taps, long long n0, const uint8_t *window,
                                 const float *ctab3, float *out16);

typedef struct csdr_amd_nfm csdr_amd_nfm;
csdr_amd_nfm *csdr_amd_nfm_create(csdr_amd_ctx *ctx, int n_streams, float shift_rate, int decimation, const float *host_taps, int taps_length,
                                  int audio_rate, int agc_block, float agc_reference, float limit_max, size_t max_block_samples);
csdr_amd_nfm *csdr_amd_nfm_create_rates(csdr_amd_ctx *ctx, int n_streams, const float *shift_rates, int decimation, const float *host_taps, int taps_length,
                                        int audio_rate, int agc_block, float agc_reference, float limit_max, size_t max_block_samples);
int  csdr_amd_nfm_set_rate(csdr_amd_nfm *w, int stream, float shift_rate);
void csdr_amd_nfm_destroy(csdr_amd_nfm *w);
int  csdr_amd_nfm_reset(csdr_amd_nfm *w);
long csdr_amd_nfm_process(csdr_amd_nfm *w, const uint8_t *in, size_t in_pitch, size_t block_samples,
                          int16_t *audio_s16, float *audio_f, size_t out_pitch);
csdr_amd_ddc *csdr_amd_nfm_front_end(csdr_amd_nfm *w);

enum { CSDR_AMD_AMSSB_AM = 0, CSDR_AMD_AMSSB_SSB = 1 };
typedef struct csdr_amd_amssb_params {
    int mode, block;
    float reference, attack_rate, decay_rate, max_gain;
    short hang_time, attack_wait_time;
    float gain_filter_alpha, limit_max;
} csdr_amd_amssb_params;
typedef struct csdr_amd_amssb_chan { float last_dc, last_gain; } csdr_amd_amssb_chan;
typedef struct csdr_amd_amssb csdr_amd_amssb;
int  csdr_amd_amssb_params_default(csdr_amd_amssb_params *p, int mode);
csdr_amd_amssb *csdr_amd_amssb_create_cf32(csdr_amd_ctx *ctx, const csdr_amd_amssb_params *params, int n_channels, const csdr_complexf *taps, int taps_length,
                                           int fft_size, size_t max_samples_per_call);
csdr_amd_amssb *csdr_amd_amssb_create(csdr_amd_ctx *ctx, const csdr_amd_amssb_params *params, int n_channels, float shift_rate, int decimation,
                                      const float *ddc_taps, int ddc_taps_length, const csdr_complexf *taps, int taps_length, int fft_size,
                                      size_t max_samples_per_call);
csdr_amd_amssb *csdr_amd_amssb_create_rates(csdr_amd_ctx *ctx, const csdr_amd_amssb_params *params, int n_channels, const float *shift_rates, int decimation,
                                            const float *ddc_taps, int ddc_taps_length, const csdr_complexf *taps, int taps_length, int fft_size,
                                            size_t max_samples_per_call);
long long csdr_amd_amssb_process(csdr_amd_amssb *p, const void *in, size_t in_pitch, long long n_in, int16_t *audio_s16, float *pre_agc_f, size_t out_pitch);
long long csdr_amd_amssb_max_out(const csdr_amd_amssb *p, long long n_in);
int  csdr_amd_amssb_set_rate(csdr_amd_amssb *p, int channel, float shift_rate);
float csdr_amd_amssb_get_rate(const csdr_amd_amssb *p, int channel);
csdr_amd_ddc *csdr_amd_amssb_front_end(csdr_amd_amssb *p);
int  csdr_amd_amssb_set_passband(csdr_amd_amssb *p, int channel, float low, float high, int window);
int  csdr_amd_amssb_set_channel_taps(csdr_amd_amssb *p, int channel, const csdr_complexf *taps, int taps_length);
int  csdr_amd_amssb_get_passband(const csdr_amd_amssb *p, int channel, float *low, float *high);
int  csdr_amd_amssb_reset(csdr_amd_amssb *p);
int  csdr_amd_amssb_reset_channel(csdr_amd_amssb *p, int channel);
int  csdr_amd_amssb_get_channel(csdr_amd_amssb *p, int channel, csdr_amd_amssb_chan *out);
int  csdr_amd_amssb_set_channel(csdr_amd_amssb *p, int channel, const csdr_amd_amssb_chan *state);
int  csdr_amd_amssb_set_lanes(csdr_amd_amssb *p, int lanes);
int  csdr_amd_amssb_lanes(const csdr_amd_amssb *p);
int  csdr_amd_amssb_force_generic(csdr_amd_amssb *p, int on);
const char *csdr_amd_amssb_kernel_name(const csdr_amd_amssb *p);
void csdr_amd_amssb_destroy(csdr_amd_amssb *p);
long long csdr_amd_debug_amssb_walk(const csdr_amd_amssb_params *params, const csdr_complexf *in, int n_blocks, csdr_amd_amssb_chan *state_io, int16_t *s16_out,
                                    float *pre_agc_out);

int csdr_amd_debug_wfm_seq_tile(int D, int L, int F, float shift_rate, const float *taps, long long n0, const uint8_t *window,
                                const float *ctab2, float *out16);
void csdr_amd_debug_dft16(const float *in32, float *out32, int inverse);
int  csdr_amd_debug_fftfilt_lds(int n, const float *taps_iq, int taps_len, const float *x_iq, long m_new, float *y_iq);
void csdr_amd_debug_dft8(const float *in16, float *out16, int inverse);
int  csdr_amd_debug_ddc_chain(int mode, float rate2, int post_in, int post_dec, int n_blocks, int *remain_io, float *phase_io, float *phases_out, int *count_out);
int  csdr_amd_debug_ddc_fold_plan(int pre_decimation, int n_blocks, int *tiles, long *lds_bytes);
int csdr_amd_debug_nfm_deemph_tile(int audio_rate, float max_amp, const float *x, float *out16);
int csdr_amd_debug_waterfall_row(int fft_size, int every_n_samples, int window, int avgnumber, float add_db, int in_format, const void *in, long long n_in,
                                 float *db_row, float *power_row);
#ifdef __cplusplus
}
#endif
#endif
```

Baseline: 2.914 million.

## Run fastddc fold GEMM on bf16 MFMA with three-way split emulating f32

```diff
diff --git a/csdr_amd/__init__.py b/csdr_amd/__init__.py
--- a/csdr_amd/__init__.py
+++ b/csdr_amd/__init__.py
@@ -327,6 +327,8 @@
     L.csdr_amd_comm_create_ipc.restype = vp; L.csdr_amd_comm_create_ipc.argtypes = [vp, C.c_char_p, i, i]
     L.csdr_amd_fastddc_inv_kernel_name.restype = C.c_char_p; L.csdr_amd_fastddc_inv_kernel_name.argtypes = [vp]
     L.csdr_amd_fastddc_inv_kernels.restype = C.c_char_p; L.csdr_amd_fastddc_inv_kernels.argtypes = [vp]
+    if hasattr(L, "csdr_amd_fastddc_inv_fold_arith"):
+        L.csdr_amd_fastddc_inv_fold_arith.restype = C.c_char_p; L.csdr_amd_fastddc_inv_fold_arith.argtypes = [vp]
     L.csdr_amd_fastddc_inv_set_profiling.argtypes = [vp, i]
     L.csdr_amd_fastddc_inv_kernel_time.argtypes = [vp, C.POINTER(C.c_double), C.POINTER(C.c_long)]
     L.csdr_amd_fastddc_inv_stage_time.argtypes = [vp, i, C.POINTER(C.c_double), C.POINTER(C.c_long)]
@@ -1828,6 +1830,7 @@
 
     def _note_ddc_call(self, inv, counts):
         self.last_ddc_kernels = self.L.csdr_amd_fastddc_inv_kernels(inv).decode()
+        self.last_ddc_arith = self.L.csdr_amd_fastddc_inv_fold_arith(inv).decode() if hasattr(self.L, "csdr_amd_fastddc_inv_fold_arith") else "f32"
         self.ddc_kernels_seen.add(self.last_ddc_kernels)
         self.ddc_call_kernels.append(self.last_ddc_kernels); self.ddc_call_counts.append(counts.copy())
 
diff --git a/csdr_amd/csrc/fastddc.hpp b/csdr_amd/csrc/fastddc.hpp
--- a/csdr_amd/csrc/fastddc.hpp
+++ b/csdr_amd/csrc/fastddc.hpp
@@ -36,6 +36,7 @@
 int ddc_mfma_kernel_time(DdcMfma *m, double *total_ms, long *launches);
 int ddc_mfma_stage_time(DdcMfma *m, int stage, double *total_ms, long *launches);
 const char *ddc_mfma_kernel_name(const DdcMfma *m);
+const char *ddc_mfma_fold_arith(const DdcMfma *m);
 const char *ddc_mfma_kernels(const DdcMfma *m);
 
 }
diff --git a/csdr_amd/csrc/fastddc_mfma.hip b/csdr_amd/csrc/fastddc_mfma.hip
--- a/csdr_amd/csrc/fastddc_mfma.hip
+++ b/csdr_amd/csrc/fastddc_mfma.hip
@@ -13,6 +13,58 @@
 
 typedef float f32x16 __attribute__((ext_vector_type(16)));
 
+__host__ __device__ __forceinline__ uint32_t ddc_f32_bits(float x) { uint32_t u; memcpy(&u, &x, 4); return u; }
+__host__ __device__ __forceinline__ float ddc_bits_f32(uint32_t u) { float x; memcpy(&x, &u, 4); return x; }
+__host__ __device__ __forceinline__ uint32_t ddc_bf16_rne(float x)
+{
+    const uint32_t u = ddc_f32_bits(x);
+    if ((u & 0x7f800000u) == 0x7f800000u) return (u >> 16) | ((u & 0xffffu) ? 0x40u : 0u);
+    return (u + 0x7fffu + ((u >> 16) & 1u)) >> 16;
+}
+__host__ __device__ __forceinline__ uint32_t ddc_bf16_pair(float lo, float hi)
+{
+#if defined(__HIP_DEVICE_COMPILE__)
+    uint32_t r; asm("v_cvt_pk_bf16_f32 %0, %1, %2" : "=v"(r) : "v"(lo), "v"(hi)); return r;
+#else
+    return ddc_bf16_rne(lo) | (ddc_bf16_rne(hi) << 16);
+#endif
+}
+__host__ __device__ __forceinline__ void ddc_split3_pair(float x0, float x1, uint32_t &h, uint32_t &m, uint32_t &l)
+{
+    h = ddc_bf16_pair(x0, x1);
+    const float d0 = x0 - ddc_bits_f32(h << 16), d1 = x1 - ddc_bits_f32(h & 0xffff0000u);
+    m = ddc_bf16_pair(d0, d1);
+    const float e0 = d0 - ddc_bits_f32(m << 16), e1 = d1 - ddc_bits_f32(m & 0xffff0000u);
+    l = ddc_bf16_pair(e0, e1);
+}
+struct DdcBf16Planes { uint32_t t[3][4]; };
+constexpr int DDC_BF16_TERMS[6][2] = {{2, 0}, {0, 2}, {1, 1}, {1, 0}, {0, 1}, {0, 0}};
+__host__ __device__ __forceinline__ void ddc_bf16_operand(const float4 (&v)[4], DdcBf16Planes &re, DdcBf16Planes &im)
+{
+#pragma unroll
+    for (int j = 0; j < 4; j++) {
+        ddc_split3_pair(v[j].x, v[j].z, re.t[0][j], re.t[1][j], re.t[2][j]);
+        ddc_split3_pair(v[j].y, v[j].w, im.t[0][j], im.t[1][j], im.t[2][j]);
+    }
+}
+__host__ __device__ __forceinline__ DdcBf16Planes ddc_bf16_negate(const DdcBf16Planes &p)
+{
+    DdcBf16Planes n;
+#pragma unroll
+    for (int k = 0; k < 3; k++)
+#pragma unroll
+        for (int j = 0; j < 4; j++) n.t[k][j] = p.t[k][j] ^ 0x80008000u;
+    return n;
+}
+typedef __bf16 ddc_bf16x8 __attribute__((ext_vector_type(8)));
+typedef uint32_t ddc_u32x4 __attribute__((ext_vector_type(4)));
+__device__ __forceinline__ ddc_bf16x8 ddc_frag(const uint32_t (&w)[4]) { const ddc_u32x4 u = {w[0], w[1], w[2], w[3]}; return __builtin_bit_cast(ddc_bf16x8, u); }
+__device__ __forceinline__ void ddc_bf16_mac(f32x16 &acc, const DdcBf16Planes &a, const DdcBf16Planes &b)
+{
+#pragma unroll
+    for (int k = 0; k < 6; k++) acc = __builtin_amdgcn_mfma_f32_32x32x16_bf16(ddc_frag(a.t[DDC_BF16_TERMS[k][0]]), ddc_frag(b.t[DDC_BF16_TERMS[k][1]]), acc, 0, 0, 0);
+}
+
 struct DdcMfma {
     csdr_amd_ctx *ctx;
     Stream side;
@@ -23,13 +75,13 @@
     DevBuf<cf32> d_Xt[2]; DevBuf<float2> d_R[2]; DevBuf<int> d_blk_remain[2], d_blk_off[2], d_counts[2]; DevBuf<float> d_blk_phase[2];
     int pending_blocks[2]; int fill, drain;
     bool inline_set[2], chains_on_side[2];
-    bool gemm_three = false, gemm_narrow = false;
+    bool gemm_three = false, gemm_narrow = false, gemm_bf16 = false;
     const char *front[2] = {"", ""}, *front2[2] = {"", ""}; std::string kernels;
     bool y_holds[2] = {false, false};
     DevBuf<DdcChanState> d_state_spec; DdcChanState *last_state = nullptr; bool spec_valid = false, ahead_ok = false; int spec_set = 0, spec_blocks = 0;
     Event ev_ready[2], ev_free[2], ev_fork; bool free_recorded[2];
     DevBuf<cf32> d_Y, d_tail[2]; DevBuf<float2> d_twb; int flip, input_size, overlap;
-    struct Opt { bool fwd_off, riders_off, spec_off, pass2_own; } opt;
+    struct Opt { bool fwd_off, riders_off, spec_off, pass2_own, fold_f32; } opt;
     bool profiling = false; double prof_ms = 0; long prof_launches = 0; KernelTimer timer;
     bool profile_stages = false;
     struct StageProf { double ms = 0; long launches = 0; KernelTimer timer; } stage[2];
@@ -160,7 +212,7 @@
     }
 }
 
-template <int NBT, bool FWD>
+template <int NBT, bool FWD, bool BF16>
 __global__ __launch_bounds__(512, 2) void k_ddc_gemm3(const float *__restrict__ Ht, const float2 *__restrict__ Xt, float2 *__restrict__ Ct,
                                                        const ChanGeom *__restrict__ geom, int inv, int Cpad, int n_channels, int nbp, int nbl, int n_blocks, float scale,
                                                        const float2 *__restrict__ g_tw)
@@ -168,6 +220,7 @@
     extern __shared__ float4 xs_all[];
     constexpr int PRE = 128, G = PRE / 4, P4 = PRE / 2 + 1, ROWS = 32 * NBT, BUF = ROWS * P4, RPW = ROWS / 8;
     constexpr int AD = FWD ? 4 : 8;
+    constexpr int NP = BF16 ? 2 : 3;
     const int wave = __builtin_amdgcn_readfirstlane(threadIdx.x >> 6), lane = threadIdx.x & 63;
     const int c_base = blockIdx.y * 256 + wave * 32, b_base = blockIdx.z * ROWS;
     const int i = lane & 31, hi = lane >> 5;
@@ -177,7 +230,8 @@
     auto dma_rows = [&](int r, int buf) {
 #pragma unroll
         for (int k = 0; k < RPW; k++) {
-            const int row = wave * RPW + k, b = min(b_base + row, n_blocks - 1);
+            const int row = wave * RPW + k; int b = min(b_base + row, n_blocks - 1);
+            if constexpr (BF16) asm volatile("" : "+v"(b));
             const float2 *src = (FWD ? Xt + ((size_t)b * 512 + r) * PRE
                                      : Xt + (((size_t)(b / nbl) * inv + r) * nbl + (b % nbl)) * PRE) + 2 * lane;
             const uint32_t la = __builtin_amdgcn_readfirstlane((int)(lds_base + ((uint32_t)buf * BUF + (uint32_t)row * P4) * 16u));
@@ -220,7 +274,7 @@
     dma_rows(r, 0);
     asm volatile("s_waitcnt vmcnt(0)" ::: "memory");
     const int c_eff = min(c_base, Cpad - 32);
-    f32x16 acc[NBT][3];
+    f32x16 acc[NBT][NP];
     auto store_bins = [&](int rr) {
         if (!active) return;
         int mm[16];
@@ -233,12 +287,15 @@
         for (int e = 0; e < 16; e++) {
             const int c = c_base + (e & 3) + 8 * (e >> 2) + 4 * hi;
             if (c >= n_channels) continue;
-            float2 *dst = Ct + ((size_t)mm[e] * Cpad + c) * nbp + b_base + i;
+            float2 *dst = Ct + (size_t)(uint32_t)(mm[e] * Cpad + c) * (uint32_t)nbp + (uint32_t)(b_base + i);
 #pragma unroll
             for (int bt = 0; bt < NBT; bt++)
                 if (b_base + bt * 32 + i < n_blocks) {
-                    const float p1 = acc[bt][0][e], p2 = acc[bt][1][e], p3 = acc[bt][2][e];
-                    dst[bt * 32] = make_float2((p1 - p2) * scale, (p3 - p1 - p2) * scale);
+                    if constexpr (BF16) dst[bt * 32] = make_float2(acc[bt][0][e] * scale, acc[bt][1][e] * scale);
+                    else {
+                        const float p1 = acc[bt][0][e], p2 = acc[bt][1][e], p3 = acc[bt][NP - 1][e];
+                        dst[bt * 32] = make_float2((p1 - p2) * scale, (p3 - p1 - p2) * scale);
+                    }
                 }
         }
     };
@@ -257,10 +314,46 @@
 #pragma unroll
         for (int bt = 0; bt < NBT; bt++)
 #pragma unroll
-            for (int p = 0; p < 3; p++)
+            for (int p = 0; p < NP; p++)
 #pragma unroll
                 for (int e = 0; e < 16; e++) acc[bt][p][e] = 0.f;
         const float4 *xrow = xs_all + cur * BUF + i * P4 + hi;
+        static_assert(G % AD == 0 && G >= 2 * AD, "k loop");
+        if constexpr (BF16) {
+        float4 xn[4];
+#pragma unroll
+        for (int j = 0; j < 4; j++) xn[j] = xrow[2 * j];
+#define G3B_TAKE(J, GRP)                                                                                                   \
+        {                                                                                                                  \
+            constexpr int d_ = (GRP) % AD;                                                                                 \
+            if constexpr ((GRP) < G - AD) { G3_TAPS_READY(a[d_], AD - 1); av[J] = a[d_]; taps_fetch(a[d_], ap + (size_t)((GRP) + AD) * gstride); }      \
+            else { G3_TAPS_READY(a[d_], AD - 1 - ((GRP) - (G - AD))); av[J] = a[d_]; }                                     \
+        }
+#define DDC_STEP16(S)                                                                                                      \
+        {                                                                                                                  \
+            g3_v4f av[4];                                                                                                  \
+            G3B_TAKE(0, 4 * (S)) G3B_TAKE(1, 4 * (S) + 1) G3B_TAKE(2, 4 * (S) + 2) G3B_TAKE(3, 4 * (S) + 3)                \
+            if (4 * ((S) + 1) == AD && rn < inv) dma_rows(rn, cur ^ 1);             \
+            float4 af[4];                                                                                                  \
+            _Pragma("unroll") for (int j = 0; j < 4; j++) af[j] = make_float4(av[j].x, av[j].y, av[j].z, av[j].w);         \
+            DdcBf16Planes hr, hi_;                                                                                         \
+            ddc_bf16_operand(af, hr, hi_);                                                                                 \
+            const DdcBf16Planes hn = ddc_bf16_negate(hi_);                                                                 \
+            _Pragma("unroll") for (int bt = 0; bt < NBT; bt++) {                                                           \
+                float4 xc[4];                                                                                              \
+                const int btn = bt + 1 < NBT ? bt + 1 : 0, sn = bt + 1 < NBT ? (S) : min((S) + 1, G / 4 - 1);                \
+                _Pragma("unroll") for (int j = 0; j < 4; j++) { xc[j] = xn[j]; xn[j] = xrow[btn * 32 * P4 + 2 * (4 * sn + j)]; }      \
+                DdcBf16Planes xr, xi;                                                                                      \
+                ddc_bf16_operand(xc, xr, xi);                                                                              \
+                ddc_bf16_mac(acc[bt][0], hr, xr); ddc_bf16_mac(acc[bt][1], hr, xi);                                        \
+                ddc_bf16_mac(acc[bt][0], hn, xi); ddc_bf16_mac(acc[bt][1], hi_, xr);                                       \
+            }                                                                                                              \
+        }
+        static_assert(G == 32, "eight steps of sixteen q");
+        DDC_STEP16(0) DDC_STEP16(1) DDC_STEP16(2) DDC_STEP16(3) DDC_STEP16(4) DDC_STEP16(5) DDC_STEP16(6) DDC_STEP16(7)
+#undef DDC_STEP16
+#undef G3B_TAKE
+        } else {
         float4 xn[NBT];
 #pragma unroll
         for (int bt = 0; bt < NBT; bt++) xn[bt] = xrow[bt * 32 * P4];
@@ -280,7 +373,6 @@
                 acc[bt][2] = __builtin_amdgcn_mfma_f32_32x32x2f32(hs1, xs1, acc[bt][2], 0, 0, 0);                          \
             }                                                                                                              \
         }
-        static_assert(G % AD == 0 && G >= 2 * AD, "k loop");
 #pragma unroll
         for (int d = 0; d < AD; d++) { G3_TAPS_READY(a[d], AD - 1); const g3_v4f av = a[d]; taps_fetch(a[d], ap + (size_t)(AD + d) * gstride); DDC_STEP3(av, d); }
         if (rn < inv) dma_rows(rn, cur ^ 1);
@@ -294,6 +386,7 @@
         if constexpr (AD == 8) { G3_LAST(4) G3_LAST(5) G3_LAST(6) G3_LAST(7) }
 #undef G3_LAST
 #undef DDC_STEP3
+        }
         r_prev = r;
         if (rn >= inv) break;
         r = rn; cur ^= 1;
@@ -301,7 +394,7 @@
     store_bins(r_prev);
 }
 
-template <int NW>
+template <int NW, bool BF16>
 __global__ __launch_bounds__(64 * NW) void k_ddc_gemm3n(const float *__restrict__ Ht, const float2 *__restrict__ Xt, float2 *__restrict__ Ct,
                                                         const ChanGeom *__restrict__ geom, int inv, int Cpad, int n_channels, int nbp, int nbl, int n_blocks, float scale)
 {
@@ -333,12 +426,43 @@
     __builtin_amdgcn_fence(__ATOMIC_RELEASE, "workgroup", "local");
     if (NW > 1) __builtin_amdgcn_s_barrier();
     __builtin_amdgcn_fence(__ATOMIC_ACQUIRE, "workgroup", "local");
-    f32x16 acc[3];
-#pragma unroll
-    for (int p = 0; p < 3; p++)
+    constexpr int NP = BF16 ? 2 : 3;
+    f32x16 acc[NP];
+#pragma unroll
+    for (int p = 0; p < NP; p++)
 #pragma unroll
         for (int e = 0; e < 16; e++) acc[p][e] = 0.f;
     const float4 *xrow = xs_all + i * P4 + hi;
+    static_assert(G % AD == 0 && G >= 2 * AD, "k loop");
+    if constexpr (BF16) {
+    float4 xn[4];
+#pragma unroll
+    for (int j = 0; j < 4; j++) xn[j] = xrow[2 * j];
+#define G3B_TAKE(J, GRP)                                                                                                   \
+    {                                                                                                                      \
+        constexpr int d_ = (GRP) % AD;                                                                                     \
+        if constexpr ((GRP) < G - AD) { G3_TAPS_READY(a[d_], AD - 1); av[J] = a[d_]; taps_fetch(a[d_], ap + (size_t)((GRP) + AD) * gstride); }      \
+        else { G3_TAPS_READY(a[d_], AD - 1 - ((GRP) - (G - AD))); av[J] = a[d_]; }                                         \
+    }
+#define DDC_STEP16N(S)                                                                                                     \
+    {                                                                                                                      \
+        g3_v4f av[4];                                                                                                      \
+        G3B_TAKE(0, 4 * (S)) G3B_TAKE(1, 4 * (S) + 1) G3B_TAKE(2, 4 * (S) + 2) G3B_TAKE(3, 4 * (S) + 3)                    \
+        float4 af[4], xc[4];                                                                                               \
+        _Pragma("unroll") for (int j = 0; j < 4; j++) af[j] = make_float4(av[j].x, av[j].y, av[j].z, av[j].w);             \
+        _Pragma("unroll") for (int j = 0; j < 4; j++) { xc[j] = xn[j]; xn[j] = xrow[2 * (4 * min((S) + 1, G / 4 - 1) + j)]; }      \
+        DdcBf16Planes hr, hi_, xr, xi;                                                                                     \
+        ddc_bf16_operand(af, hr, hi_);                                                                                     \
+        ddc_bf16_operand(xc, xr, xi);                                                                                      \
+        const DdcBf16Planes hn = ddc_bf16_negate(hi_);                                                                     \
+        ddc_bf16_mac(acc[0], hr, xr); ddc_bf16_mac(acc[1], hr, xi);                                                        \
+        ddc_bf16_mac(acc[0], hn, xi); ddc_bf16_mac(acc[1], hi_, xr);                                                       \
+    }
+    static_assert(G == 32, "eight steps of sixteen q");
+    DDC_STEP16N(0) DDC_STEP16N(1) DDC_STEP16N(2) DDC_STEP16N(3) DDC_STEP16N(4) DDC_STEP16N(5) DDC_STEP16N(6) DDC_STEP16N(7)
+#undef DDC_STEP16N
+#undef G3B_TAKE
+    } else {
     float4 xn = xrow[0];
 #define DDC_STEP3N(AV, GG)                                                                                                 \
     {                                                                                                                      \
@@ -352,7 +476,6 @@
         acc[1] = __builtin_amdgcn_mfma_f32_32x32x2f32((AV).w, xv.w, acc[1], 0, 0, 0);                                      \
         acc[2] = __builtin_amdgcn_mfma_f32_32x32x2f32(hs1, xs1, acc[2], 0, 0, 0);                                          \
     }
-    static_assert(G % AD == 0 && G >= 2 * AD, "k loop");
 #pragma unroll
     for (int g = 0; g < G - AD; g += AD) {
 #pragma unroll
@@ -362,6 +485,7 @@
     G3N_LAST(0) G3N_LAST(1) G3N_LAST(2) G3N_LAST(3) G3N_LAST(4) G3N_LAST(5) G3N_LAST(6) G3N_LAST(7)
 #undef G3N_LAST
 #undef DDC_STEP3N
+    }
     if (!active) return;
     int mm[16];
 #pragma unroll
@@ -374,8 +498,12 @@
     for (int e = 0; e < 16; e++) {
         const int c = c_base + (e & 3) + 8 * (e >> 2) + 4 * hi;
         if (c >= n_channels) continue;
-        const float p1 = acc[0][e], p2 = acc[1][e], p3 = acc[2][e];
-        Ct[((size_t)mm[e] * Cpad + c) * nbp + b_base + i] = make_float2((p1 - p2) * scale, (p3 - p1 - p2) * scale);
+        float2 *dst = Ct + ((size_t)mm[e] * Cpad + c) * nbp + b_base + i;
+        if constexpr (BF16) *dst = make_float2(acc[0][e] * scale, acc[1][e] * scale);
+        else {
+            const float p1 = acc[0][e], p2 = acc[1][e], p3 = acc[NP - 1][e];
+            *dst = make_float2((p1 - p2) * scale, (p3 - p1 - p2) * scale);
+        }
     }
 }
 #undef G3_TAPS_READY
@@ -783,6 +911,7 @@
         o.fwd_off = getenv("CSDR_AMD_DDC_FWD_OFF") != nullptr;
         o.riders_off = getenv("CSDR_AMD_DDC_RIDERS_OFF") != nullptr; o.spec_off = getenv("CSDR_AMD_DDC_SPEC_OFF") != nullptr;
         o.pass2_own = getenv("CSDR_AMD_DDC_PASS2") != nullptr;
+        o.fold_f32 = getenv("CSDR_AMD_DDC_FOLD_F32") && atoi(getenv("CSDR_AMD_DDC_FOLD_F32")) != 0;
     }
     m->nbl = m->world > 1 ? (max_blocks + m->world - 1) / m->world : m->nbp;
     const size_t xt_elems = (size_t)m->world * inv * m->nbl * pre;
@@ -1025,6 +1154,7 @@
 }
 
 const char *ddc_mfma_kernel_name(const DdcMfma *m) { return m->gemm_three ? (m->gemm_narrow ? "k_ddc_gemm3n" : "k_ddc_gemm3") : "k_ddc_gemm"; }
+const char *ddc_mfma_fold_arith(const DdcMfma *m) { return m->gemm_three && m->gemm_bf16 ? "bf16x3" : "f32"; }
 const char *ddc_mfma_kernels(const DdcMfma *m) { return m->kernels.c_str(); }
 static void mfma_note_kernels(DdcMfma *m, int k, const char *fold, const char *inverse) { m->kernels.clear(); m->kernels.append(m->front[k]).append(m->front2[k]).append(fold).append("+").append(inverse); }
 int ddc_mfma_set_profiling(DdcMfma *m, int on)
@@ -1071,27 +1201,32 @@
         hipLaunchKernelGGL((k_ddc_gemm<NBTV, PV>), grid_use, dim3(512), lds_use, st, m->d_Ht.get(), reinterpret_cast<const float2 *>(m->d_Xt[k].get()),           \
                            reinterpret_cast<float2 *>(m->d_Ct.get()), d_geom, m->inv, m->pre, m->Cpad, m->C, m->nbp, m->nbl, n_blocks, scale); } while (0)
     const bool three = ddc_folds_with_gemm3(m, n_blocks);
-    m->gemm_three = three; m->gemm_narrow = false;
+    const bool bf = !m->opt.fold_f32;
+    m->gemm_three = three; m->gemm_narrow = false; m->gemm_bf16 = bf;
     const char *fold = "";
     if (three) {
         const bool fwd = m->y_holds[k];
         const float2 *src = fwd ? reinterpret_cast<const float2 *>(m->d_Y.get()) : reinterpret_cast<const float2 *>(m->d_Xt[k].get());
-#define DDC_GEMM3_LAUNCH(NBTV, FV) do { const int rc = lds_attr_once((const void *)k_ddc_gemm3<NBTV, FV>, lds_use); if (rc) return rc;                     \
-        hipLaunchKernelGGL((k_ddc_gemm3<NBTV, FV>), grid_use, dim3(512), lds_use, st, m->d_Ht.get(), src, reinterpret_cast<float2 *>(m->d_Ct.get()), d_geom, m->inv, m->Cpad, m->C,  \
+#define DDC_GEMM3_LAUNCH(NBTV, FV) do { if (bf) DDC_GEMM3_LAUNCH_(NBTV, FV, true); else DDC_GEMM3_LAUNCH_(NBTV, FV, false); } while (0)
+#define DDC_GEMM3_LAUNCH_(NBTV, FV, BV) do { const int rc = lds_attr_once((const void *)k_ddc_gemm3<NBTV, FV, BV>, lds_use); if (rc) return rc;                     \
+        hipLaunchKernelGGL((k_ddc_gemm3<NBTV, FV, BV>), grid_use, dim3(512), lds_use, st, m->d_Ht.get(), src, reinterpret_cast<float2 *>(m->d_Ct.get()), d_geom, m->inv, m->Cpad, m->C,  \
                            m->nbp, m->nbl, n_blocks, scale, m->d_tw.get()); } while (0)
         m->gemm_narrow = !fwd && ddc_fold_is_narrow(m, n_blocks);
         if (m->gemm_narrow) {
             const dim3 gn(m->inv, 1, cdiv(n_blocks, 32));
             const size_t ldsn = (size_t)32 * (m->pre / 2 + 1) * sizeof(float4);
-#define DDC_GEMM3N_LAUNCH(NWV) hipLaunchKernelGGL((k_ddc_gemm3n<NWV>), gn, dim3(64 * NWV), ldsn, st, m->d_Ht.get(), src, reinterpret_cast<float2 *>(m->d_Ct.get()), d_geom, m->inv, m->Cpad, m->C, \
+#define DDC_GEMM3N_LAUNCH(NWV) do { if (bf) DDC_GEMM3N_LAUNCH_(NWV, true); else DDC_GEMM3N_LAUNCH_(NWV, false); } while (0)
+#define DDC_GEMM3N_LAUNCH_(NWV, BV) hipLaunchKernelGGL((k_ddc_gemm3n<NWV, BV>), gn, dim3(64 * NWV), ldsn, st, m->d_Ht.get(), src, reinterpret_cast<float2 *>(m->d_Ct.get()), d_geom, m->inv, m->Cpad, m->C, \
                                                   m->nbp, m->nbl, n_blocks, scale)
             if (m->Cpad <= 32) DDC_GEMM3N_LAUNCH(1); else if (m->Cpad <= 64) DDC_GEMM3N_LAUNCH(2); else DDC_GEMM3N_LAUNCH(4);
             fold = m->Cpad <= 32 ? "k_ddc_gemm3n<1>" : m->Cpad <= 64 ? "k_ddc_gemm3n<2>" : "k_ddc_gemm3n<4>";
 #undef DDC_GEMM3N_LAUNCH
+#undef DDC_GEMM3N_LAUNCH_
         }
         else if (nbt == 2) { if (fwd) DDC_GEMM3_LAUNCH(2, true); else DDC_GEMM3_LAUNCH(2, false); }
         else          { if (fwd) DDC_GEMM3_LAUNCH(1, true); else DDC_GEMM3_LAUNCH(1, false); }
 #undef DDC_GEMM3_LAUNCH
+#undef DDC_GEMM3_LAUNCH_
         if (!m->gemm_narrow) fold = nbt == 2 ? (fwd ? "k_ddc_gemm3<2,true>" : "k_ddc_gemm3<2,false>") : (fwd ? "k_ddc_gemm3<1,true>" : "k_ddc_gemm3<1,false>");
     }
     else if (nbt == 2) { if (persist) DDC_GEMM_LAUNCH(2, true); else DDC_GEMM_LAUNCH(2, false); }
@@ -1167,3 +1302,61 @@
     if (inverse) dft8<true>(v); else dft8<false>(v);
     for (int k = 0; k < 8; k++) { out16[2 * k] = v[k].x; out16[2 * k + 1] = v[k].y; }
 }
+
+extern "C" void csdr_amd_debug_ddc_split3(const float *x, int n, unsigned short *h, unsigned short *m, unsigned short *l)
+{
+    for (int k = 0; k < n; k += 2) {
+        uint32_t hh, mm, ll;
+        csdr_amd::ddc_split3_pair(x[k], k + 1 < n ? x[k + 1] : 0.f, hh, mm, ll);
+        h[k] = (unsigned short)hh; m[k] = (unsigned short)mm; l[k] = (unsigned short)ll;
+        if (k + 1 < n) { h[k + 1] = (unsigned short)(hh >> 16); m[k + 1] = (unsigned short)(mm >> 16); l[k + 1] = (unsigned short)(ll >> 16); }
+    }
+}
+
+extern "C" int csdr_amd_debug_ddc_fold_tile_bf16(const float *H, const float *X, int pre, float *C)
+{
+    using namespace csdr_amd;
+    if (pre < 16 || pre % 16) return -1;
+    const int G = pre / 4;
+    std::vector<float4> Ht((size_t)G * 32 * 2), rows((size_t)32 * (pre / 2));
+    for (int c = 0; c < 32; c++)
+        for (int q = 0; q < pre; q++) {
+            float *ht = reinterpret_cast<float *>(Ht.data()) + (((size_t)(q >> 2) * 32 + c) * 8 + 2 * (q & 3));
+            ht[0] = H[((size_t)c * pre + q) * 2]; ht[1] = H[((size_t)c * pre + q) * 2 + 1];
+        }
+    memcpy(rows.data(), X, sizeof(float) * 2 * 32 * pre);
+    static const auto bf = [](uint32_t w, int e) { return ddc_bits_f32((e & 1 ? w >> 16 : w & 0xffffu) << 16); };
+    struct Lane { DdcBf16Planes hr, hi, hn, xr, xi; float acc[2][16]; };
+    std::vector<Lane> L(64);
+    for (auto &l : L) memset(l.acc, 0, sizeof l.acc);
+    const auto mac = [&](int p, DdcBf16Planes Lane::*a, DdcBf16Planes Lane::*b) {
+        for (int k = 0; k < 6; k++)
+            for (int l = 0; l < 64; l++)
+                for (int reg = 0; reg < 16; reg++) {
+                    const int row = (reg & 3) + 8 * (reg >> 2) + 4 * (l >> 5), col = l & 31;
+                    float sum = L[l].acc[p][reg];
+                    for (int kk = 0; kk < 16; kk++) {
+                        const uint32_t *aw = (L[row + 32 * (kk >> 3)].*a).t[DDC_BF16_TERMS[k][0]], *bw = (L[col + 32 * (kk >> 3)].*b).t[DDC_BF16_TERMS[k][1]];
+                        sum += bf(aw[(kk & 7) >> 1], kk) * bf(bw[(kk & 7) >> 1], kk);
+                    }
+                    L[l].acc[p][reg] = sum;
+                }
+    };
+    for (int s = 0; s < pre / 16; s++) {
+        for (int l = 0; l < 64; l++) {
+            const int i = l & 31, hi = l >> 5;
+            float4 af[4], xc[4];
+            for (int j = 0; j < 4; j++) { af[j] = Ht[((size_t)(4 * s + j) * 32 + i) * 2 + hi]; xc[j] = rows[(size_t)i * (pre / 2) + 2 * (4 * s + j) + hi]; }
+            ddc_bf16_operand(af, L[l].hr, L[l].hi); ddc_bf16_operand(xc, L[l].xr, L[l].xi);
+            L[l].hn = ddc_bf16_negate(L[l].hi);
+        }
+        mac(0, &Lane::hr, &Lane::xr); mac(1, &Lane::hr, &Lane::xi);
+        mac(0, &Lane::hn, &Lane::xi); mac(1, &Lane::hi, &Lane::xr);
+    }
+    for (int l = 0; l < 64; l++)
+        for (int reg = 0; reg < 16; reg++) {
+            const int c = (reg & 3) + 8 * (reg >> 2) + 4 * (l >> 5), b = l & 31;
+            C[((size_t)c * 32 + b) * 2] = L[l].acc[0][reg]; C[((size_t)c * 32 + b) * 2 + 1] = L[l].acc[1][reg];
+        }
+    return 0;
+}
diff --git a/csdr_amd/csrc/fftpath.hip b/csdr_amd/csrc/fftpath.hip
--- a/csdr_amd/csrc/fftpath.hip
+++ b/csdr_amd/csrc/fftpath.hip
@@ -617,6 +617,7 @@
 }
 
 const char *csdr_amd_fastddc_inv_kernel_name(const csdr_amd_fastddc_inv *f) { return f->mf ? ddc_mfma_kernel_name(f->mf.get()) : "k_ddc_fold_ct"; }
+const char *csdr_amd_fastddc_inv_fold_arith(const csdr_amd_fastddc_inv *f) { return f->mf ? ddc_mfma_fold_arith(f->mf.get()) : "f32"; }
 const char *csdr_amd_fastddc_inv_kernels(const csdr_amd_fastddc_inv *f) { return f->mf ? ddc_mfma_kernels(f->mf.get()) : f->kernels; }
 int csdr_amd_fastddc_inv_set_profiling(csdr_amd_fastddc_inv *f, int on) { return f->mf ? ddc_mfma_set_profiling(f->mf.get(), on) : 0; }
 int csdr_amd_fastddc_inv_kernel_time(csdr_amd_fastddc_inv *f, double *total_ms, long *launches)
diff --git a/include/csdr_amd.h b/include/csdr_amd.h
--- a/include/csdr_amd.h
+++ b/include/csdr_amd.h
@@ -362,6 +362,7 @@
                                   csdr_complexf *out, size_t out_pitch, int *out_counts);
 const char *csdr_amd_fastddc_inv_kernel_name(const csdr_amd_fastddc_inv *f);
 const char *csdr_amd_fastddc_inv_kernels(const csdr_amd_fastddc_inv *f);
+const char *csdr_amd_fastddc_inv_fold_arith(const csdr_amd_fastddc_inv *f);
 int  csdr_amd_fastddc_inv_set_profiling(csdr_amd_fastddc_inv *f, int on);
 int  csdr_amd_fastddc_inv_kernel_time(csdr_amd_fastddc_inv *f, double *total_ms, long *launches);
 int  csdr_amd_fastddc_inv_stage_time(csdr_amd_fastddc_inv *f, int stage, double *total_ms, long *launches);
@@ -534,6 +535,8 @@
 void csdr_amd_debug_dft8(const float *in16, float *out16, int inverse);
 int  csdr_amd_debug_ddc_chain(int mode, float rate2, int post_in, int post_dec, int n_blocks, int *remain_io, float *phase_io, float *phases_out, int *count_out);
 int  csdr_amd_debug_ddc_fold_plan(int pre_decimation, int n_blocks, int *tiles, long *lds_bytes);
+void csdr_amd_debug_ddc_split3(const float *x, int n, unsigned short *h, unsigned short *m, unsigned short *l);
+int  csdr_amd_debug_ddc_fold_tile_bf16(const float *H, const float *X, int pre, float *C);
 int csdr_amd_debug_nfm_deemph_tile(int audio_rate, float max_amp, const float *x, float *out16);
 int csdr_amd_debug_waterfall_row(int fft_size, int every_n_samples, int window, int avgnumber, float add_db, int in_format, const void *in, long long n_in,
                                  float *db_row, float *power_row);
```

Result: no change. 2.913 million (median of 2 runs) (-0.0%).
